# SoyeonHH/MMDA

Hardware: AMD Instinct MI355X
Metric: training samples/sec on MOSEI-shaped synthetic batch (higher is better)
Workload: dtype bf16; 1 GPU; MISA train step, MOSEI shapes B=32/GPU T=50 (d_t,d_v,d_a)=(300,35,74) hidden=128 V=20000, bf16 MFMA operands fp32 accumulate, dropout on, full lengths; global_batch=32, seq_len=50, parallelism=single, use_confidNet=False, rnncell=lstm, dp_global_stats=False

## Files before the change

### mmda_amd/csrc/fused_rows.h

```cpp
#pragma once
#include "../../include/mmda_hip.h"
#include "loss_terms.h"
#include <stdint.h>

struct FusedBwdC {
  int B, hs, ncls, nb;
  const float* tcp; const float* scores; const float* d_tcp; const float* d_scores; float* d_logits;
  float p_cls; uint64_t seed; int site_cls;
  const float* head_w;
  float* d_hfused;
  mmda_ln_bwd_args ln2;
  float* pg_parts;
  const float* d_recon; const float* rec_wT; float* rec_part;
};

struct FusedBwdA {
  int B, hs, nhead, nb;
  mmda_ln_bwd_args ln1;
  const float* ffn_parts; int n_parts; float* d_x1;
  const float* d_attn_out; const float* out_wT; float* d_ctx;
  const float* qkv; const float* probs; float* d_qkv; float p_tf; uint64_t seed; int site_attn;
  const float* in_wT;
  const float* d_recon;
  const float* rec_part;
  const float* rec_wT;
  const float* x6;
  float* d_x6;
  const float* priv_wT;
  const float* sh_wT;
  float* d_orig;
  mmda_ln_bwd_args lnp[3];
  float* pg_parts;
  unsigned long long* dbg;
  const unsigned* wait_flag; unsigned wait_value; unsigned* wait_err;
};

struct FusedFwdA {
  int B, hs, nhead, nb;
  const float* x6;
  const float* rec_w; const float* rec_b; float* recon;
  const float* in_w; const float* in_b; float* qkv;
  float* ctx; float* probs; float p_tf; uint64_t seed; int site_attn;
  const float* out_w; const float* out_b; float* attn_out;
  mmda_ln_args ln1;
  const float* orig; float* d_recon; float* d_orig; float recon_inv_n, recon_scale;
  int split_recon;
};
struct FusedFwdC {
  int B, hs, ncls, nb;
  mmda_ln_args ln2;
  const float* ffn_parts; int n_parts; const float* b2; float* f2;
  const float* hfused; const float* head_w; const float* head_b; float* logits;
  float threshold; float* tcp; float* scores; float* labels; float p_cls; uint64_t seed; int site_cls;
  const float* emo; float* d_scores;
  ClsTerm cls;
};
struct FusedFfnFwd {
  int M, hs, F, S;
  const float* x1; const float* w1; const float* b1; float* f1;
  float p; uint64_t seed; int site;
  const float* w2;
  float* parts;
};
struct FusedFfnBwd {
  int M, hs, F, S;
  const float* d_f2; const float* f1; float gate_scale;
  const float* l2_wT;
  float* d_f1;
  const float* l1_wT;
  float* parts;
};
int mmda_fused_ffn_fwd(const FusedFfnFwd* a, void* stream);
int mmda_fused_ffn_bwd(const FusedFfnBwd* a, void* stream);
int mmda_fused_fwd_a(const FusedFwdA* a, void* stream);
int mmda_fused_fwd_c(const FusedFwdC* a, void* stream);
int mmda_fused_bwd_c(const FusedBwdC* a, void* stream);
int mmda_fused_bwd_a(const FusedBwdA* a, void* stream);
constexpr int FUSED_PG_SLOTS = 5;
int mmda_fused_pg_finish(const float* pg_parts, int B, int hs, float* const* dgamma, float* const* dbeta, void* stream);
extern "C" int mmda_debug_set_fused_stamps(void* device_buffer);
```

### mmda_amd/csrc/fused_rows.hip

```cpp
#include "common.h"
#include "internal.h"
#include "rowlocal.h"
#include "fused_rows.h"

namespace {

typedef __attribute__((ext_vector_type(4))) float f4;
constexpr int FR_THREADS = 512;

struct MacRound { f4 a[8], b[8]; };
constexpr int WL_LD = 128 + 4;
struct WRows { f4 g[8]; };
__device__ __forceinline__ void wrows_load(WRows& W, const float* __restrict__ bblk, int ldb, int lane) {
#pragma unroll
  for (int j = 0; j < 8; ++j) W.g[j] = *reinterpret_cast<const f4*>(bblk + (int64_t)(2 * j + (lane >> 5)) * ldb + 4 * (lane & 31));
}
__device__ __forceinline__ void wrows_to_lds(const WRows& W, float* wl, int lane) {
#pragma unroll
  for (int j = 0; j < 8; ++j) *reinterpret_cast<f4*>(wl + (2 * j + (lane >> 5)) * WL_LD + 4 * (lane & 31)) = W.g[j];
}
__device__ __forceinline__ void mac_frags(MacRound& R, const float* arow , const float* wl, int lane) {
  const int r16 = lane & 15, g = lane >> 4;
  const f4 z = {0.f, 0.f, 0.f, 0.f};
#pragma unroll
  for (int c = 0; c < 8; ++c) {
    R.a[c] = arow ? *reinterpret_cast<const f4*>(arow + 16 * c + 4 * g) : z;
    R.b[c] = *reinterpret_cast<const f4*>(wl + r16 * WL_LD + 16 * c + 4 * g);
  }
}
__device__ __forceinline__ void mac_run(f32x4& acc, const MacRound& R) {
#pragma unroll
  for (int c = 0; c < 8; ++c)
#pragma unroll
    for (int s = 0; s < 4; ++s) acc = __builtin_amdgcn_mfma_f32_16x16x4f32(R.a[c][s], R.b[c][s], acc, 0, 0, 0);
}
template <int NR>
__device__ __forceinline__ void tile_mac_chain(f32x4& acc, const float* const (&ar)[NR], const float* const (&bblk)[NR], const int (&ldb)[NR],
                                               int lane, float* wl ) {
  WRows W;
  MacRound R;
  wrows_load(W, bblk[0], ldb[0], lane);
#pragma unroll
  for (int r = 0; r < NR; ++r) {
    wrows_to_lds(W, wl, lane);
    if (r + 1 < NR) wrows_load(W, bblk[r + 1], ldb[r + 1], lane);
    mac_frags(R, ar[r], wl, lane);
    mac_run(acc, R);
  }
}

__device__ __forceinline__ float sum_parts(const float* __restrict__ p, int n, int64_t stride) {
  float acc = 0.f;
  int q = 0;
  for (; q + 16 <= n; q += 16) {
    float v[16];
#pragma unroll
    for (int u = 0; u < 16; ++u) v[u] = p[(q + u) * stride];
#pragma unroll
    for (int u = 0; u < 16; ++u) acc += v[u];
  }
  for (; q < n; ++q) acc += p[q * stride];
  return acc;
}

template <typename RowOff, typename Finish>
__device__ __forceinline__ void sum_parts_rows(const float* __restrict__ parts, int n, int64_t stride, int groups, RowOff row_off, f4* lds,
                                               Finish finish) {
  const int n0 = (n + 1) >> 1;
  for (int it = threadIdx.x; it < 2 * groups; it += FR_THREADS) {
    const int gi = it % groups, half = it / groups;
    const float* p = parts + row_off(gi) + (int64_t)(half ? n0 : 0) * stride;
    const int cnt = half ? n - n0 : n0;
    f4 acc = {0.f, 0.f, 0.f, 0.f};
    int q = 0;
    for (; q + 16 <= cnt; q += 16) {
      f4 v[16];
#pragma unroll
      for (int u = 0; u < 16; ++u) v[u] = *reinterpret_cast<const f4*>(p + (q + u) * stride);
#pragma unroll
      for (int u = 0; u < 16; ++u) acc += v[u];
    }
    for (; q < cnt; ++q) acc += *reinterpret_cast<const f4*>(p + q * stride);
    lds[half * groups + gi] = acc;
  }
  __syncthreads();
  for (int gi = threadIdx.x; gi < groups; gi += FR_THREADS) finish(gi, lds[gi] + lds[groups + gi]);
  __syncthreads();
}

__device__ __forceinline__ void stage_sync() {
  __threadfence_block();
  __syncthreads();
}

constexpr int LDS_A_FLOATS = 12 * (384 + 4) + 18 * (128 + 4);
template <typename SrcOf>
__device__ __forceinline__ void stage_rows(float* lds, int nrows, int K, SrcOf src_of) {
  const int per_row = K >> 2;
  for (int e = threadIdx.x; e < nrows * per_row; e += FR_THREADS) {
    const int r = e / per_row, c = e % per_row;
    const float* src = src_of(r);
    const f4 z = {0.f, 0.f, 0.f, 0.f};
    *reinterpret_cast<f4*>(lds + r * (K + 4) + 4 * c) = src ? *reinterpret_cast<const f4*>(src + 4 * c) : z;
  }
  __syncthreads();
}

template <typename RowOf>
__device__ __forceinline__ void ln_bwd_rows(const mmda_ln_bwd_args& a, int nrows, RowOf row_of, float* red ,
                                            float* part) {
  const int lane = threadIdx.x & 63, wave = threadIdx.x >> 6;
  float dg[2] = {0.f, 0.f}, db[2] = {0.f, 0.f};
  for (int i = wave; i < nrows; i += FR_THREADS / 64) ln_bwd_row<2>(a, row_of(i), lane, dg, db);
  if (part == nullptr) return;
#pragma unroll
  for (int q = 0; q < 2; ++q) { red[(0 * 8 + wave) * 128 + q * 64 + lane] = dg[q]; red[(1 * 8 + wave) * 128 + q * 64 + lane] = db[q]; }
  __syncthreads();
  for (int i = threadIdx.x; i < 128; i += FR_THREADS) {
    float gsum = 0.f, bsum = 0.f;
#pragma unroll
    for (int w = 0; w < 8; ++w) { gsum += red[(0 * 8 + w) * 128 + i]; bsum += red[(1 * 8 + w) * 128 + i]; }
    part[i] = i < a.n ? gsum : 0.f;
    part[128 + i] = i < a.n ? bsum : 0.f;
  }
  __syncthreads();
}
__device__ __forceinline__ float* pg_slot(float* parts, int b, int k) { return parts ? parts + ((int64_t)b * FUSED_PG_SLOTS + k) * 256 : nullptr; }
__device__ __forceinline__ void pg_zero_rest(float* parts, int b0, int nb, int k) {
  if (!parts) return;
  for (int e = threadIdx.x; e < (nb - 1) * 256; e += FR_THREADS) pg_slot(parts, b0 + 1 + e / 256, k)[e % 256] = 0.f;
}

__device__ __forceinline__ void rec_part_rows(const FusedBwdC& P, int b0, int nb, float* lds_a, float* lds_w) {
  const int B = P.B, hs = P.hs;
  const int lane = threadIdx.x & 63, wave = threadIdx.x >> 6;
  const int r16 = lane & 15, g = lane >> 4;
  const int nmod = 3 * nb;
  const bool mok = r16 < nmod;
  const int mi = mok ? r16 / nb : 0;
  const int col = wave * 16 + r16;
  stage_rows(lds_a, nmod, hs, [&](int r) { return P.d_recon + ((int64_t)(r / nb) * B + b0 + (r % nb)) * hs; });
  f32x4 acc = {0.f, 0.f, 0.f, 0.f};
  const float* row = mok ? lds_a + r16 * (hs + 4) : nullptr;
  const float* const ar[3] = {(mok && mi == 0) ? row : nullptr, (mok && mi == 1) ? row : nullptr, (mok && mi == 2) ? row : nullptr};
  const float* rw = P.rec_wT + (int64_t)wave * 16 * hs;
  const float* const bb[3] = {rw, rw + (int64_t)hs * hs, rw + (int64_t)2 * hs * hs};
  const int ld[3] = {hs, hs, hs};
  tile_mac_chain<3>(acc, ar, bb, ld, lane, lds_w + wave * 16 * WL_LD);
#pragma unroll
  for (int i = 0; i < 4; ++i) {
    const int r = 4 * g + i;
    if (r < nmod) P.rec_part[((int64_t)(r / nb) * B + b0 + (r % nb)) * hs + col] = acc[i];
  }
}

__global__ __launch_bounds__(FR_THREADS) void fused_bwd_c_kernel(FusedBwdC P) {
  __shared__ float red[2 * 8 * 128];
  __shared__ __attribute__((aligned(16))) float lds_a[6 * (128 + 4)];
  __shared__ __attribute__((aligned(16))) float lds_w[8 * 16 * WL_LD];
  const int nblk = (P.B + P.nb - 1) / P.nb;
  if ((int)blockIdx.x >= nblk) {
    const int rb0 = ((int)blockIdx.x - nblk) * P.nb;
    rec_part_rows(P, rb0, min(P.nb, P.B - rb0), lds_a, lds_w);
    return;
  }
  const int b0 = (int)blockIdx.x * P.nb;
  const int nb = min(P.nb, P.B - b0);
  const int NC = 6 + P.ncls, B = P.B, hs = P.hs;
  for (int e = threadIdx.x; e < nb * NC; e += FR_THREADS) {
    const int b = b0 + e / NC, c = e % NC;
    P.d_logits[b * NC + c] = head_bwd_one(b, c, P.ncls, P.tcp, P.scores, P.d_tcp, P.d_scores, P.p_cls, P.seed, P.site_cls);
  }
  stage_sync();
  const int W6 = 6 * hs;
  for (int e = threadIdx.x; e < nb * W6; e += FR_THREADS) {
    const int b = b0 + e / W6, n = e % W6;
    float acc = 0.f;
    for (int c = 0; c < NC; ++c) acc += P.d_logits[b * NC + c] * P.head_w[(int64_t)c * W6 + n];
    P.d_hfused[(int64_t)b * W6 + n] = acc;
  }
  stage_sync();
  ln_bwd_rows(P.ln2, S6K * nb, [&](int i) { return (i / nb) * B + b0 + (i % nb); }, red, pg_slot(P.pg_parts, b0, 0));
  pg_zero_rest(P.pg_parts, b0, nb, 0);
}

__global__ __launch_bounds__(FR_THREADS) void fused_bwd_a_kernel(FusedBwdA P) {
  __shared__ float red[2 * 8 * 128];
  __shared__ __attribute__((aligned(16))) float lds_a[LDS_A_FLOATS];
  __shared__ __attribute__((aligned(16))) float lds_w[8 * 16 * WL_LD];
  const int b0 = (int)blockIdx.x * P.nb;
  const int nb = min(P.nb, P.B - b0);
  const int B = P.B, hs = P.hs;
  const int lane = threadIdx.x & 63, wave = threadIdx.x >> 6;
  const int r16 = lane & 15, g = lane >> 4;
  const int64_t BH = (int64_t)B * hs;
  int stamp_i = 0;
  auto stamp = [&]() { if (P.dbg && blockIdx.x == 0 && threadIdx.x == 0) P.dbg[stamp_i] = __builtin_readcyclecounter(); ++stamp_i; };
  stamp();
  flag_wait(P.wait_flag, P.wait_value, P.wait_err);
  if (P.ffn_parts) {
    const int64_t MH = (int64_t)S6K * B * hs;
    auto off = [&](int gi) { const int i = gi / (hs / 4); return ((int64_t)(i / nb) * B + b0 + (i % nb)) * hs + 4 * (gi % (hs / 4)); };
    sum_parts_rows(P.ffn_parts, P.n_parts, MH, S6K * nb * (hs / 4), off, reinterpret_cast<f4*>(lds_a), [&](int gi, f4 t) {
      f4* d = reinterpret_cast<f4*>(P.d_x1 + off(gi));
      *d = *d + t;
    });
    stage_sync();
  }
  ln_bwd_rows(P.ln1, S6K * nb, [&](int i) { return (i / nb) * B + b0 + (i % nb); }, red, pg_slot(P.pg_parts, b0, 1));
  pg_zero_rest(P.pg_parts, b0, nb, 1);
  stage_sync();
  stamp();
  const int ntok = S6K * nb;
  const bool rok = r16 < ntok;
  const int tj = rok ? r16 / nb : 0;
  const int col = wave * 16 + r16;
  {
    f32x4 acc = {0.f, 0.f, 0.f, 0.f};
    stage_rows(lds_a, ntok, hs, [&](int r) { return P.d_attn_out + ((int64_t)(r / nb) * B + b0 + (r % nb)) * hs; });
    const float* const ar[1] = {rok ? lds_a + r16 * (hs + 4) : nullptr};
    const float* const bb[1] = {P.out_wT + (int64_t)wave * 16 * hs};
    const int ld[1] = {hs};
    tile_mac_chain<1>(acc, ar, bb, ld, lane, lds_w + wave * 16 * WL_LD);
#pragma unroll
    for (int i = 0; i < 4; ++i) {
      const int r = 4 * g + i;
      if (r < ntok) P.d_ctx[((int64_t)(r / nb) * B + b0 + (r % nb)) * hs + col] = acc[i];
    }
  }
  stage_sync();
  stamp();
  for (int pr = wave; pr < nb * P.nhead; pr += FR_THREADS / 64)
    attn_bwd_hd64_one(P.qkv, P.probs, P.d_ctx, B, P.d_qkv, P.p_tf, P.seed, P.site_attn, P.nhead, (b0 + pr / P.nhead) * P.nhead + pr % P.nhead, lane);
  stage_sync();
  stamp();
  {
    f32x4 acc = {0.f, 0.f, 0.f, 0.f};
    float* lds_r = lds_a + 12 * (3 * hs + 4);
    stage_rows(lds_a, ntok, 3 * hs, [&](int r) { return P.d_qkv + ((int64_t)(r / nb) * B + b0 + (r % nb)) * 3 * hs; });
    const float* qrow = rok ? lds_a + r16 * (3 * hs + 4) : nullptr;
    const float* wrow = P.in_wT + (int64_t)wave * 16 * 3 * hs;
    if (P.rec_part) {
      const float* const ar[3] = {qrow, qrow ? qrow + 128 : nullptr, qrow ? qrow + 256 : nullptr};
      const float* const bb[3] = {wrow, wrow + 128, wrow + 256};
      const int ld[3] = {3 * hs, 3 * hs, 3 * hs};
      tile_mac_chain<3>(acc, ar, bb, ld, lane, lds_w + wave * 16 * WL_LD);
    } else {
      stage_rows(lds_r, ntok, hs, [&](int r) { return P.d_recon + ((int64_t)((r / nb) % 3) * B + b0 + (r % nb)) * hs; });
      const float* rec_row = rok ? lds_r + r16 * (hs + 4) : nullptr;
      const float* const ar[6] = {qrow, qrow ? qrow + 128 : nullptr, qrow ? qrow + 256 : nullptr, (rok && tj % 3 == 0) ? rec_row : nullptr,
                                  (rok && tj % 3 == 1) ? rec_row : nullptr, (rok && tj % 3 == 2) ? rec_row : nullptr};
      const float* recw = P.rec_wT + (int64_t)wave * 16 * hs;
      const float* const bb[6] = {wrow, wrow + 128, wrow + 256, recw, recw + (int64_t)hs * hs, recw + (int64_t)2 * hs * hs};
      const int ld[6] = {3 * hs, 3 * hs, 3 * hs, hs, hs, hs};
      tile_mac_chain<6>(acc, ar, bb, ld, lane, lds_w + wave * 16 * WL_LD);
    }
#pragma unroll
    for (int i = 0; i < 4; ++i) {
      const int r = 4 * g + i;
      if (r < ntok) {
        const int64_t o = ((int64_t)(r / nb) * B + b0 + (r % nb)) * hs + col;
        const float s = P.x6[o];
        float t = acc[i];
        if (P.rec_part) t += P.rec_part[((int64_t)((r / nb) % 3) * B + b0 + (r % nb)) * hs + col];
        P.d_x6[o] = (P.d_x6[o] + t) * (s * (1.f - s));
      }
    }
  }
  stage_sync();
  stamp();
  const int nmod = 3 * nb;
  const bool mok = r16 < nmod;
  const int mi = mok ? r16 / nb : 0;
  {
    f32x4 acc = {0.f, 0.f, 0.f, 0.f};
    stage_rows(lds_a, 2 * nmod, hs, [&](int r) { return P.d_x6 + ((int64_t)((r / nmod) * 3 + (r % nmod) / nb) * B + b0 + (r % nb)) * hs; });
    const float* prow = mok ? lds_a + r16 * (hs + 4) : nullptr;
    const float* const ar[4] = {mok ? lds_a + (nmod + r16) * (hs + 4) : nullptr, (mok && mi == 0) ? prow : nullptr,
                                (mok && mi == 1) ? prow : nullptr, (mok && mi == 2) ? prow : nullptr};
    const float* pw = P.priv_wT + (int64_t)wave * 16 * hs;
    const float* const bb[4] = {P.sh_wT + (int64_t)wave * 16 * hs, pw, pw + (int64_t)hs * hs, pw + (int64_t)2 * hs * hs};
    const int ld[4] = {hs, hs, hs, hs};
    tile_mac_chain<4>(acc, ar, bb, ld, lane, lds_w + wave * 16 * WL_LD);
#pragma unroll
    for (int i = 0; i < 4; ++i) {
      const int r = 4 * g + i;
      if (r < nmod) {
        const int64_t o = ((int64_t)(r / nb) * B + b0 + (r % nb)) * hs + col;
        P.d_orig[o] += acc[i];
      }
    }
  }
  stage_sync();
  stamp();
  for (int i = wave; i < 3 * nb; i += FR_THREADS / 64) {
    const mmda_ln_bwd_args& a = P.lnp[i / nb];
    float dg[2] = {0.f, 0.f}, db[2] = {0.f, 0.f};
    ln_bwd_row<2>(a, b0 + i % nb, lane, dg, db);
    float* part = pg_slot(P.pg_parts, b0 + i % nb, 2 + i / nb);
    if (part) {
#pragma unroll
      for (int q = 0; q < 2; ++q) {
        const int c = q * 64 + lane;
        part[c] = c < a.n ? dg[q] : 0.f;
        part[128 + c] = c < a.n ? db[q] : 0.f;
      }
    }
  }
  (void)BH;
  stamp();
}

__global__ __launch_bounds__(FR_THREADS) void fused_fwd_a_kernel(FusedFwdA P) {
  __shared__ __attribute__((aligned(16))) float lds_a[LDS_A_FLOATS];
  __shared__ __attribute__((aligned(16))) float lds_w[8 * 16 * WL_LD];
  const int nblk = (P.B + P.nb - 1) / P.nb;
  const bool do_recon = !P.split_recon || (int)blockIdx.x >= nblk;
  const bool do_chain = !P.split_recon || (int)blockIdx.x < nblk;
  const int b0 = ((int)blockIdx.x % nblk) * P.nb;
  const int nb = min(P.nb, P.B - b0);
  const int B = P.B, hs = P.hs;
  const int lane = threadIdx.x & 63, wave = threadIdx.x >> 6;
  const int r16 = lane & 15, g = lane >> 4;
  const int ntok = S6K * nb, nmod = 3 * nb;
  const bool rok = r16 < ntok;
  const bool mok = r16 < nmod;
  const int mi = mok ? r16 / nb : 0;
  const int col = wave * 16 + r16;
  stage_rows(lds_a, ntok, hs, [&](int r) { return P.x6 + ((int64_t)(r / nb) * B + b0 + (r % nb)) * hs; });
  if (do_recon) {
  for (int e = threadIdx.x; e < nmod * (hs / 4); e += FR_THREADS) {
    const int r = e / (hs / 4), c = e % (hs / 4);
    const f4 a = *reinterpret_cast<const f4*>(lds_a + r * (hs + 4) + 4 * c), b2 = *reinterpret_cast<const f4*>(lds_a + (nmod + r) * (hs + 4) + 4 * c);
    *reinterpret_cast<f4*>(lds_a + (12 + r) * (hs + 4) + 4 * c) = a + b2;
  }
  __syncthreads();
  {
    f32x4 acc = {0.f, 0.f, 0.f, 0.f};
    const float* srow = mok ? lds_a + (12 + r16) * (hs + 4) : nullptr;
    const float* const ar[3] = {(mok && mi == 0) ? srow : nullptr, (mok && mi == 1) ? srow : nullptr, (mok && mi == 2) ? srow : nullptr};
    const float* rw = P.rec_w + (int64_t)wave * 16 * hs;
    const float* const bb[3] = {rw, rw + (int64_t)hs * hs, rw + (int64_t)2 * hs * hs};
    const int ld[3] = {hs, hs, hs};
    tile_mac_chain<3>(acc, ar, bb, ld, lane, lds_w + wave * 16 * WL_LD);
#pragma unroll
    for (int i = 0; i < 4; ++i) {
      const int r = 4 * g + i;
      if (r < nmod) {
        const int64_t o = ((int64_t)(r / nb) * B + b0 + (r % nb)) * hs + col;
        const float rv = acc[i] + P.rec_b[(r / nb) * hs + col];
        P.recon[o] = rv;
        if (P.d_recon) {
          const float gr = recon_seed(rv - P.orig[o], P.recon_inv_n, P.recon_scale);
          P.d_recon[o] = gr;
          P.d_orig[o] = 0.f - gr;
        }
      }
    }
  }
  }
  if (!do_chain) return;
#pragma unroll 1
  for (int pass = 0; pass < 3; ++pass) {
    const int n = pass * 128 + col;
    f32x4 acc = {0.f, 0.f, 0.f, 0.f};
    const float* const ar[1] = {rok ? lds_a + r16 * (hs + 4) : nullptr};
    const float* const bb[1] = {P.in_w + (int64_t)(pass * 128 + wave * 16) * hs};
    const int ld[1] = {hs};
    tile_mac_chain<1>(acc, ar, bb, ld, lane, lds_w + wave * 16 * WL_LD);
    const float bias = P.in_b[n];
#pragma unroll
    for (int i = 0; i < 4; ++i) {
      const int r = 4 * g + i;
      if (r < ntok) P.qkv[((int64_t)(r / nb) * B + b0 + (r % nb)) * 3 * hs + n] = acc[i] + bias;
    }
  }
  stage_sync();
  for (int pr = wave; pr < nb * P.nhead; pr += FR_THREADS / 64)
    attn_fwd_hd64_one(P.qkv, B, P.ctx, P.probs, P.p_tf, P.seed, P.site_attn, P.nhead, (b0 + pr / P.nhead) * P.nhead + pr % P.nhead, lane);
  stage_sync();
  {
    f32x4 acc = {0.f, 0.f, 0.f, 0.f};
    stage_rows(lds_a, ntok, hs, [&](int r) { return P.ctx + ((int64_t)(r / nb) * B + b0 + (r % nb)) * hs; });
    const float* const ar[1] = {rok ? lds_a + r16 * (hs + 4) : nullptr};
    const float* const bb[1] = {P.out_w + (int64_t)wave * 16 * hs};
    const int ld[1] = {hs};
    tile_mac_chain<1>(acc, ar, bb, ld, lane, lds_w + wave * 16 * WL_LD);
    const float bias = P.out_b[col];
#pragma unroll
    for (int i = 0; i < 4; ++i) {
      const int r = 4 * g + i;
      if (r < ntok) P.attn_out[((int64_t)(r / nb) * B + b0 + (r % nb)) * hs + col] = acc[i] + bias;
    }
  }
  stage_sync();
  for (int i = wave; i < ntok; i += FR_THREADS / 64) ln_fwd_row<2>(P.ln1, (i / nb) * B + b0 + (i % nb), lane);
}

template <bool CLS_OPTS>
__global__ __launch_bounds__(FR_THREADS) void fused_fwd_c_kernel(FusedFwdC P) {
  __shared__ f4 sp[2 * 12 * 32];
  const int b0 = (int)blockIdx.x * P.nb;
  const int nb = min(P.nb, P.B - b0);
  const int B = P.B, hs = P.hs, NC = 6 + P.ncls, W6 = 6 * hs;
  const int lane = threadIdx.x & 63, wave = threadIdx.x >> 6;
  if (P.ffn_parts) {
    const int64_t MH = (int64_t)S6K * B * hs;
    auto off = [&](int gi) { const int i = gi / (hs / 4); return ((int64_t)(i / nb) * B + b0 + (i % nb)) * hs + 4 * (gi % (hs / 4)); };
    sum_parts_rows(P.ffn_parts, P.n_parts, MH, S6K * nb * (hs / 4), off, sp, [&](int gi, f4 t) {
      const float* b = P.b2 + 4 * (gi % (hs / 4));
      *reinterpret_cast<f4*>(P.f2 + off(gi)) = t + f4{b[0], b[1], b[2], b[3]};
    });
    stage_sync();
  }
  for (int i = wave; i < S6K * nb; i += FR_THREADS / 64) ln_fwd_row<2>(P.ln2, (i / nb) * B + b0 + (i % nb), lane);
  stage_sync();
  for (int e = wave; e < nb * NC; e += FR_THREADS / 64) {
    const int b = b0 + e / NC, c = e % NC;
    const float* x = P.hfused + (int64_t)b * W6;
    const float* w = P.head_w + (int64_t)c * W6;
    float acc = 0.f;
    for (int k = lane * 4; k < W6; k += 256) {
      const f4 xv = *reinterpret_cast<const f4*>(x + k), wv = *reinterpret_cast<const f4*>(w + k);
      acc += xv[0] * wv[0] + xv[1] * wv[1] + xv[2] * wv[2] + xv[3] * wv[3];
    }
    acc = wave_sum(acc);
    if (lane == 0) {
      const float z = acc + P.head_b[c];
      P.logits[b * NC + c] = z;
      head_fwd_one(z, b, c, P, [&](int k, float sc) {
        if (P.d_scores) {
          const float yv = P.emo[b * P.ncls + k];
          float v, d;
          if constexpr (CLS_OPTS) cls_term(P.cls, sc, yv, k, v, d);
          else bce_plain(sc, yv, 1.f, v, d);
          P.d_scores[b * P.ncls + k] = d / B;
        }
      });
    }
  }
}

constexpr int FFN_RB = 48, FFN_S = 32;
constexpr int FFN_LDS_X = FFN_RB * (128 + 4), FFN_LDS_H = FFN_RB * (FFN_S + 4);

struct FfnGeom { int rb0, nrows, j; };

template <typename Epi1, typename Store2>
__device__ __forceinline__ void ffn_two_products(const float* xs, float* hs_, const float* __restrict__ b1rows ,
                                                 int ldb1, const float* __restrict__ b2rows , int ldb2,
                                                 Epi1 epi1, Store2 store2) {
  const int lane = threadIdx.x & 63, wave = threadIdx.x >> 6;
  const int r16 = lane & 15, g = lane >> 4;
  {
    const int ct = wave >> 2;
    f4 bw[8];
    const float* brow = b1rows + (int64_t)(ct * 16 + r16) * ldb1;
#pragma unroll
    for (int c = 0; c < 8; ++c) bw[c] = *reinterpret_cast<const f4*>(brow + 16 * c + 4 * g);
#pragma unroll
    for (int q = 0; q < (FFN_RB / 16 + 3) / 4; ++q) {
      const int rt = (wave & 3) + 4 * q;
      if (rt >= FFN_RB / 16) break;
      const float* arow = xs + (rt * 16 + r16) * (128 + 4);
      f32x4 acc = {0.f, 0.f, 0.f, 0.f};
#pragma unroll
      for (int c = 0; c < 8; ++c) {
        const f4 a = *reinterpret_cast<const f4*>(arow + 16 * c + 4 * g);
#pragma unroll
        for (int s = 0; s < 4; ++s) acc = __builtin_amdgcn_mfma_f32_16x16x4f32(a[s], bw[c][s], acc, 0, 0, 0);
      }
#pragma unroll
      for (int i = 0; i < 4; ++i) {
        const int row = rt * 16 + 4 * g + i, unit = ct * 16 + r16;
        hs_[row * (FFN_S + 4) + unit] = epi1(row, unit, acc[i]);
      }
    }
  }
  __syncthreads();
  {
    f4 bw[2];
    const float* brow = b2rows + (int64_t)(wave * 16 + r16) * ldb2;
#pragma unroll
    for (int c = 0; c < 2; ++c) bw[c] = *reinterpret_cast<const f4*>(brow + 16 * c + 4 * g);
#pragma unroll
    for (int rt = 0; rt < FFN_RB / 16; ++rt) {
      const float* arow = hs_ + (rt * 16 + r16) * (FFN_S + 4);
      f32x4 acc = {0.f, 0.f, 0.f, 0.f};
#pragma unroll
      for (int c = 0; c < 2; ++c) {
        const f4 a = *reinterpret_cast<const f4*>(arow + 16 * c + 4 * g);
#pragma unroll
        for (int s = 0; s < 4; ++s) acc = __builtin_amdgcn_mfma_f32_16x16x4f32(a[s], bw[c][s], acc, 0, 0, 0);
      }
#pragma unroll
      for (int i = 0; i < 4; ++i) store2(rt * 16 + 4 * g + i, wave * 16 + r16, acc[i]);
    }
  }
}

__device__ __forceinline__ void ffn_stage_x(float* xs, const float* __restrict__ X, int rb0, int M) {
  constexpr int PER = FFN_RB * 32 / FR_THREADS;
  f4 v[PER];
#pragma unroll
  for (int u = 0; u < PER; ++u) {
    const int e = threadIdx.x + u * FR_THREADS, r = e >> 5, c = e & 31;
    v[u] = *reinterpret_cast<const f4*>(X + (int64_t)min(rb0 + r, M - 1) * 128 + 4 * c);
  }
#pragma unroll
  for (int u = 0; u < PER; ++u) {
    const int e = threadIdx.x + u * FR_THREADS, r = e >> 5, c = e & 31;
    const f4 z = {0.f, 0.f, 0.f, 0.f};
    *reinterpret_cast<f4*>(xs + r * (128 + 4) + 4 * c) = (rb0 + r < M) ? v[u] : z;
  }
  __syncthreads();
}

__global__ __launch_bounds__(FR_THREADS) void fused_ffn_fwd_kernel(FusedFfnFwd P) {
  extern __shared__ __attribute__((aligned(16))) float ffn_lds[];
  float* xs = ffn_lds; float* hs_ = ffn_lds + FFN_LDS_X;
  const int nsl = P.F / FFN_S;
  const int j = (int)blockIdx.x % nsl, rb0 = ((int)blockIdx.x / nsl) * FFN_RB;
  ffn_stage_x(xs, P.x1, rb0, P.M);
  float* part = P.parts + (int64_t)j * P.M * P.hs;
  ffn_two_products(xs, hs_, P.w1 + (int64_t)j * FFN_S * P.hs, P.hs, P.w2 + (int64_t)j * FFN_S, P.F,
    [&](int row, int unit, float v) {
      const int m = rb0 + row, n = j * FFN_S + unit;
      v += P.b1[n];
      v = fmaxf(v, 0.f);
      if (P.p > 0.f) v *= drop_mul(P.p, P.seed, P.site, (uint64_t)m * P.F + n);
      if (m < P.M) P.f1[(int64_t)m * P.F + n] = v; else v = 0.f;
      return v;
    },
    [&](int row, int col, float v) { if (rb0 + row < P.M) part[(int64_t)(rb0 + row) * P.hs + col] = v; });
}

__global__ __launch_bounds__(FR_THREADS) void fused_ffn_bwd_kernel(FusedFfnBwd P) {
  extern __shared__ __attribute__((aligned(16))) float ffn_lds[];
  float* xs = ffn_lds; float* hs_ = ffn_lds + FFN_LDS_X;
  const int nsl = P.F / FFN_S;
  const int j = (int)blockIdx.x % nsl, rb0 = ((int)blockIdx.x / nsl) * FFN_RB;
  ffn_stage_x(xs, P.d_f2, rb0, P.M);
  float* part = P.parts + (int64_t)j * P.M * P.hs;
  ffn_two_products(xs, hs_, P.l2_wT + (int64_t)j * FFN_S * P.hs, P.hs, P.l1_wT + (int64_t)j * FFN_S, P.F,
    [&](int row, int unit, float v) {
      const int m = rb0 + row, n = j * FFN_S + unit;
      if (m >= P.M) return 0.f;
      v *= (P.f1[(int64_t)m * P.F + n] > 0.f) ? P.gate_scale : 0.f;
      P.d_f1[(int64_t)m * P.F + n] = v;
      return v;
    },
    [&](int row, int col, float v) { if (rb0 + row < P.M) part[(int64_t)(rb0 + row) * P.hs + col] = v; });
}

}

int mmda_fused_ffn_fwd(const FusedFfnFwd* a, void* stream) {
  if (!a || a->M <= 0 || a->hs != 128 || a->S != FFN_S || a->F <= 0 || (a->F % FFN_S)) return MMDA_EINVAL;
  const int lds = (FFN_LDS_X + FFN_LDS_H) * 4;
  static bool attr = false;
  if (!attr) { (void)hipFuncSetAttribute(reinterpret_cast<const void*>(fused_ffn_fwd_kernel), hipFuncAttributeMaxDynamicSharedMemorySize, lds); attr = true; }
  hipLaunchKernelGGL(fused_ffn_fwd_kernel, dim3((a->F / FFN_S) * ceil_div(a->M, FFN_RB)), dim3(FR_THREADS), lds, (hipStream_t)stream, *a);
  MMDA_CHECK_LAUNCH("mmda_fused_ffn_fwd");
  return MMDA_OK;
}

int mmda_fused_ffn_bwd(const FusedFfnBwd* a, void* stream) {
  if (!a || a->M <= 0 || a->hs != 128 || a->S != FFN_S || a->F <= 0 || (a->F % FFN_S)) return MMDA_EINVAL;
  const int lds = (FFN_LDS_X + FFN_LDS_H) * 4;
  static bool attr = false;
  if (!attr) { (void)hipFuncSetAttribute(reinterpret_cast<const void*>(fused_ffn_bwd_kernel), hipFuncAttributeMaxDynamicSharedMemorySize, lds); attr = true; }
  hipLaunchKernelGGL(fused_ffn_bwd_kernel, dim3((a->F / FFN_S) * ceil_div(a->M, FFN_RB)), dim3(FR_THREADS), lds, (hipStream_t)stream, *a);
  MMDA_CHECK_LAUNCH("mmda_fused_ffn_bwd");
  return MMDA_OK;
}

int mmda_fused_fwd_a(const FusedFwdA* a, void* stream) {
  if (!a || a->B <= 0 || a->nb <= 0 || a->nb > 2 || a->hs != 128 || a->nhead != 2 || a->ln1.n != 128) return MMDA_EINVAL;
  if (a->d_recon && (!a->orig || !a->d_orig)) return MMDA_EINVAL;
  static const int split_on = mmda_env_int("MMDA_FUSED_SPLIT", 1);
  FusedFwdA f = *a;
  const int nblk = ceil_div(a->B, a->nb);
  f.split_recon = (split_on && nblk <= 64) ? 1 : 0;
  hipLaunchKernelGGL(fused_fwd_a_kernel, dim3(f.split_recon ? 2 * nblk : nblk), dim3(FR_THREADS), 0, (hipStream_t)stream, f);
  MMDA_CHECK_LAUNCH("mmda_fused_fwd_a");
  return MMDA_OK;
}

int mmda_fused_fwd_c(const FusedFwdC* a, void* stream) {
  if (!a || a->B <= 0 || a->nb <= 0 || a->nb > 2 || a->hs != 128 || a->ln2.n != 128 || (a->d_scores && !a->emo)) return MMDA_EINVAL;
  const bool opts = a->d_scores && !cls_plain(a->cls);
  hipLaunchKernelGGL(opts ? fused_fwd_c_kernel<true> : fused_fwd_c_kernel<false>, dim3(ceil_div(a->B, a->nb)), dim3(FR_THREADS), 0,
                     (hipStream_t)stream, *a);
  MMDA_CHECK_LAUNCH("mmda_fused_fwd_c");
  return MMDA_OK;
}

struct FusedPgOut { float* dgamma[FUSED_PG_SLOTS]; float* dbeta[FUSED_PG_SLOTS]; };
__global__ __launch_bounds__(256) void fused_pg_finish_kernel(const float* __restrict__ parts, int B, int hs, FusedPgOut out) {
  __shared__ float sub[256];
  const int e = blockIdx.x * 16 + (threadIdx.x >> 4);
  const int j = threadIdx.x & 15;
  const bool ok = e < FUSED_PG_SLOTS * 256;
  const int k = ok ? e / 256 : 0, which = (e % 256) / 128, c = e % 128;
  const float* p = parts + (int64_t)k * 256 + which * 128 + c;
  float acc = 0.f;
  if (ok) {
    const int64_t st = (int64_t)FUSED_PG_SLOTS * 256;
    int b = j;
    for (; b + 7 * 16 < B; b += 8 * 16) {
      float v[8];
#pragma unroll
      for (int u = 0; u < 8; ++u) v[u] = p[(b + 16 * u) * st];
#pragma unroll
      for (int u = 0; u < 8; ++u) acc += v[u];
    }
    for (; b < B; b += 16) acc += p[b * st];
  }
  sub[threadIdx.x] = acc;
  __syncthreads();
  float* dst = which ? out.dbeta[k] : out.dgamma[k];
  if (ok && j == 0 && dst && c < hs) {
    float t = 0.f;
#pragma unroll
    for (int u = 0; u < 16; ++u) t += sub[(threadIdx.x & ~15) + u];
    dst[c] += t;
  }
}

int mmda_fused_pg_finish(const float* pg_parts, int B, int hs, float* const* dgamma, float* const* dbeta, void* stream) {
  if (!pg_parts || B <= 0 || hs != 128 || !dgamma || !dbeta) return MMDA_EINVAL;
  FusedPgOut out;
  for (int k = 0; k < FUSED_PG_SLOTS; ++k) { out.dgamma[k] = dgamma[k]; out.dbeta[k] = dbeta[k]; }
  hipLaunchKernelGGL(fused_pg_finish_kernel, dim3(FUSED_PG_SLOTS * 256 / 16), dim3(256), 0, (hipStream_t)stream, pg_parts, B, hs, out);
  MMDA_CHECK_LAUNCH("mmda_fused_pg_finish");
  return MMDA_OK;
}

int mmda_fused_bwd_c(const FusedBwdC* a, void* stream) {
  if (!a || a->B <= 0 || a->nb <= 0 || a->hs != 128 || a->ln2.n != 128) return MMDA_EINVAL;
  if ((a->ln2.dgamma || a->ln2.dbeta) && !a->pg_parts) return MMDA_EINVAL;
  if (a->rec_part && (!a->d_recon || !a->rec_wT || a->nb > 2)) return MMDA_EINVAL;
  hipLaunchKernelGGL(fused_bwd_c_kernel, dim3(ceil_div(a->B, a->nb) * (a->rec_part ? 2 : 1)), dim3(FR_THREADS), 0, (hipStream_t)stream, *a);
  MMDA_CHECK_LAUNCH("mmda_fused_bwd_c");
  return MMDA_OK;
}

static unsigned long long* g_fr_dbg = nullptr;
extern "C" int mmda_debug_set_fused_stamps(void* device_buffer) { g_fr_dbg = (unsigned long long*)device_buffer; return MMDA_OK; }

int mmda_fused_bwd_a(const FusedBwdA* a, void* stream) {
  if (!a || a->B <= 0 || a->nb <= 0 || a->nb > 2 || a->hs != 128 || a->nhead != 2) return MMDA_EINVAL;
  if ((a->ln1.dgamma || a->ln1.dbeta || a->lnp[0].dgamma || a->lnp[0].dbeta) && !a->pg_parts) return MMDA_EINVAL;
  FusedBwdA P = *a;
  P.dbg = g_fr_dbg;
  hipLaunchKernelGGL(fused_bwd_a_kernel, dim3(ceil_div(a->B, a->nb)), dim3(FR_THREADS), 0, (hipStream_t)stream, P);
  MMDA_CHECK_LAUNCH("mmda_fused_bwd_a");
  return MMDA_OK;
}
```

### mmda_amd/csrc/misa.hip

```cpp
#include "common.h"
#include "fused_rows.h"
#include "internal.h"
#include <algorithm>

#include <cstring>
#include <map>
#include <string>
#include <vector>

namespace {

struct ParamInfo { std::string name; int64_t off; int rows, cols; };

struct RnnP {
  int D, H;
  int64_t w_ih, w_hh[2], b_ih, b_hh;
  int ldD, ldG, ldH;
};
struct ModP {
  int D, H;
  RnnP rnn[2];
  int64_t ln_w, ln_b;
  int64_t pw, pb, plw, plb;
};
struct ParamTable {
  std::vector<ParamInfo> params;
  std::map<std::string, int> index;
  int64_t dense = 0, flat = 0;
  int64_t rnn2_begin = 0, rnn1_begin = 0;
  ModP mod[3];
  int64_t priv_w, priv_b, sh_w, sh_b, rec_w, rec_b, d1_w = -1, d1_b = -1, d2_w = -1, d2_b = -1, sp_w, sp_b;
  int64_t head_w, head_b, embed;
  int64_t in_w, in_b, out_w, out_b, l1_w, l1_b, l2_w, l2_b, n1_w, n1_b, n2_w, n2_b;
  int64_t prelu_a = -1;
};

struct RnnW {
  int64_t pack_f[2], pack_b[2], pack_c[2];
  int64_t wb, wbT;
  int64_t xb, xbT;
  int64_t dgb, dgbT;
  int64_t hbT;
  int64_t hbp[2];
  int64_t pw_ih = -1, pw_hh[2] = {-1, -1}, pb_ih = -1, pb_hh = -1, gw_ih = -1, gw_hh[2] = {-1, -1}, gb = -1;
};
struct ModW {
  RnnW rnn[2];
  int64_t x, gates[2], c[2], hseq[2], normed, ln_mean, ln_rstd, utt, d_utt, d_hseq1, d_normed, d_x, xchg, xchg_floats;
};
struct Workspace {
  int B = 0, T = 0, ldR = 0;
  int64_t floats = 0;
  ModW mod[3];
  int64_t pub_begin = 0, pub_end = 0;
  int64_t zero_begin = 0, zero_end = 0;
  int64_t zero_cls = 0, zero_recon = 0;
  int64_t gpad_begin = 0, gpad_end = 0;
  int64_t z, pmean, prstd, orig, x6, rsum, recon, dom_z, dom_h, dom, qkv, probs, ctx, attn_out, ln1_mean, ln1_rstd, x1, f1, f2,
      ln2_mean, ln2_rstd, hfused, logits, tcp, scores, labels, losses, diff_work, ffn_parts, pg_parts, ln_parts;
  int64_t x1q, x1s, w1q, w1s, f1q, f1s, w2q, w2s;
  int64_t head_wT, l2_wT, l1_wT, out_wT, in_wT, rec_wT, priv_wT, sh_wT, d1_wT = -1, d2_wT = -1, pwT[3];
  int64_t d_scores, d_tcp, d_x6, d_orig, d_recon, d_dom, d_logits, d_hfused, d_x1, d_f2, d_f1, d_attn_out, d_ctx, d_qkv, d_z,
      d_dom_h, d_dom_z;
  int64_t gnorm = -1, gnorm_parts = -1;
  int64_t esort = -1;
  int64_t rec_part = -1;
};

struct StepPlan {
  bool inf = false;
  bool enc_cut = false;
  bool enc_nostash = false;
  bool enc_cached = false;
  bool bfg = false;
  int gm = 0;
  bool kdg = false;
  bool tn_wgrad = false;
  bool want_b = false, want_c = false;
  bool want_wT = false, wT_merge = false;
  bool skinny = false;
  bool row_fuse = false;
  bool ffn_fuse_fwd = false, ffn_fuse_bwd = false;
  bool seed_recon = false, seed_cls = false;
  bool fj_on = false, fj_fwd = false, fj_device = false;
  bool zg_here = false;
  bool rec_hoisted = false;
  bool sort_early = false;
  int embed_update = 0;
  bool embed_deferred = false;
  bool embed_bg = false, embed_bg_late = false; int embed_bg_wgs = 0, embed_bg_lds = 0;
};

enum { EU_DENSE = 0, EU_SPARSE = 1, EU_FROZEN = 2 };

enum { SITE_ATTN = 1, SITE_DROP1 = 2, SITE_FFN = 3, SITE_DROP2 = 4, SITE_CLS = 5, SITE_DISC = 6,
       SITE_RRELU = 7 , SITE_RRELU_DISC = 10 };
constexpr int FFN = 2048, NHEAD = 2, S6 = 6;

struct OptStep { float lr, clip, grad_scale; int step; const float* acc; bool norm; };
struct PendingRows {
  const int64_t* ids = nullptr; const int32_t* lengths = nullptr; bool on = false;
  void set(const int64_t* i, const int32_t* l) { ids = i; lengths = l; on = true; }
  PendingRows take() { const PendingRows r = *this; *this = PendingRows{}; return r; }
};
struct RowList { int64_t* ids; float* rows; int64_t used, capacity; };

int64_t add_param(ParamTable& t, const std::string& name, int rows, int cols) {
  ParamInfo p{name, t.flat, rows, cols};
  t.index[name] = (int)t.params.size();
  t.params.push_back(p);
  t.flat += (int64_t)rows * (cols > 0 ? cols : 1);
  return p.off;
}

ParamTable build_params(const mmda_misa_config& c) {
  ParamTable t{};
  const int dims[3] = {c.d_t, c.d_v, c.d_a};
  const char* mn[3] = {"t", "v", "a"};
  const int hs = c.hidden;
  for (int i = 0; i < 3; ++i) { ModP& md = t.mod[i]; md.D = md.H = dims[i]; }
  for (int i = 0; i < 3; ++i) {
    ModP& md = t.mod[i];
    std::string p = std::string("project_") + mn[i] + ".project_" + mn[i];
    md.pw = add_param(t, p + ".weight", hs, 4 * md.H);
    md.pb = add_param(t, p + ".bias", hs, 0);
    md.plw = add_param(t, p + "_layer_norm.weight", hs, 0);
    md.plb = add_param(t, p + "_layer_norm.bias", hs, 0);
  }
  t.priv_w = add_param(t, "private_t.private_t_1.weight", hs, hs);
  add_param(t, "private_v.private_v_1.weight", hs, hs);
  add_param(t, "private_a.private_a_3.weight", hs, hs);
  t.priv_b = add_param(t, "private_t.private_t_1.bias", hs, 0);
  add_param(t, "private_v.private_v_1.bias", hs, 0);
  add_param(t, "private_a.private_a_3.bias", hs, 0);
  t.sh_w = add_param(t, "shared.shared_1.weight", hs, hs);
  t.sh_b = add_param(t, "shared.shared_1.bias", hs, 0);
  t.rec_w = add_param(t, "recon_t.recon_t_1.weight", hs, hs);
  add_param(t, "recon_v.recon_v_1.weight", hs, hs);
  add_param(t, "recon_a.recon_a_1.weight", hs, hs);
  t.rec_b = add_param(t, "recon_t.recon_t_1.bias", hs, 0);
  add_param(t, "recon_v.recon_v_1.bias", hs, 0);
  add_param(t, "recon_a.recon_a_1.bias", hs, 0);
  if (!c.use_cmd_sim) {
    t.d1_w = add_param(t, "discriminator.discriminator_layer_1.weight", hs, hs);
    t.d1_b = add_param(t, "discriminator.discriminator_layer_1.bias", hs, 0);
    t.d2_w = add_param(t, "discriminator.discriminator_layer_2.weight", 3, hs);
    t.d2_b = add_param(t, "discriminator.discriminator_layer_2.bias", 3, 0);
  }
  t.sp_w = add_param(t, "sp_discriminator.sp_discriminator_layer_1.weight", 4, hs);
  t.sp_b = add_param(t, "sp_discriminator.sp_discriminator_layer_1.bias", 4, 0);
  t.head_w = add_param(t, "confidence.confidence_layer_1.weight", 6, 6 * hs);
  add_param(t, "classifier.classifier_layer.weight", c.ncls, 6 * hs);
  t.head_b = add_param(t, "confidence.confidence_layer_1.bias", 6, 0);
  add_param(t, "classifier.classifier_layer.bias", c.ncls, 0);
  for (int i = 0; i < 3; ++i) {
    t.mod[i].ln_w = add_param(t, std::string(mn[i]) + "layer_norm.weight", 2 * t.mod[i].H, 0);
    t.mod[i].ln_b = add_param(t, std::string(mn[i]) + "layer_norm.bias", 2 * t.mod[i].H, 0);
  }
  const std::string te = "transformer_encoder.layers.0.";
  t.in_w = add_param(t, te + "self_attn.in_proj_weight", 3 * hs, hs);
  t.in_b = add_param(t, te + "self_attn.in_proj_bias", 3 * hs, 0);
  t.out_w = add_param(t, te + "self_attn.out_proj.weight", hs, hs);
  t.out_b = add_param(t, te + "self_attn.out_proj.bias", hs, 0);
  t.l1_w = add_param(t, te + "linear1.weight", FFN, hs);
  t.l1_b = add_param(t, te + "linear1.bias", FFN, 0);
  t.l2_w = add_param(t, te + "linear2.weight", hs, FFN);
  t.l2_b = add_param(t, te + "linear2.bias", hs, 0);
  t.n1_w = add_param(t, te + "norm1.weight", hs, 0);
  t.n1_b = add_param(t, te + "norm1.bias", hs, 0);
  t.n2_w = add_param(t, te + "norm2.weight", hs, 0);
  t.n2_b = add_param(t, te + "norm2.bias", hs, 0);
  if (c.act == MMDA_ACT_PRELU) t.prelu_a = add_param(t, "activation.weight", 1, 0);
  for (int l = 1; l >= 0; --l) {
    t.flat = (t.flat + 3) & ~(int64_t)3;
    (l == 1 ? t.rnn2_begin : t.rnn1_begin) = t.flat;
    for (int i = 0; i < 3; ++i) {
      ModP& md = t.mod[i];
      RnnP& r = md.rnn[l];
      r.H = md.H; r.D = l == 0 ? md.D : 2 * md.H;
      r.ldD = round_up(r.D, 8); r.ldG = round_up(8 * r.H, 8); r.ldH = round_up(r.H, 8);
      const int ng = c.rnncell == MMDA_CELL_GRU ? 3 : 4;
      std::string pre = std::string(mn[i]) + "rnn" + (l == 0 ? "1" : "2") + ".";
      r.w_ih = add_param(t, pre + "weight_ih_l0", ng * r.H, r.D);
      add_param(t, pre + "weight_ih_l0_reverse", ng * r.H, r.D);
      r.w_hh[0] = add_param(t, pre + "weight_hh_l0", ng * r.H, r.H);
      r.w_hh[1] = add_param(t, pre + "weight_hh_l0_reverse", ng * r.H, r.H);
      r.b_ih = add_param(t, pre + "bias_ih_l0", ng * r.H, 0);
      add_param(t, pre + "bias_ih_l0_reverse", ng * r.H, 0);
      r.b_hh = add_param(t, pre + "bias_hh_l0", ng * r.H, 0);
      add_param(t, pre + "bias_hh_l0_reverse", ng * r.H, 0);
    }
  }
  t.flat = (t.flat + 3) & ~(int64_t)3;
  t.dense = t.flat;
  t.embed = add_param(t, "embed.weight", c.vocab, c.d_t);
  t.flat = (t.flat + 3) & ~(int64_t)3;
  return t;
}

Workspace carve(const mmda_misa_config& c, const ParamTable& par, int B, int T) {
  const int hs = c.hidden, NC = 6 + c.ncls;
  const int64_t R = (int64_t)T * B;
  int64_t cur = 0;
  auto take = [&cur](int64_t n) { int64_t o = cur; cur += (n + 3) & ~(int64_t)3; return o; };
  Workspace w{};
  w.B = B; w.T = T; w.ldR = round_up(B * T, 8);
  for (int i = 0; i < 3; ++i) {
    const ModP& md = par.mod[i]; ModW& mw = w.mod[i];
    mw.xchg_floats = (mmda_lstm_xchg_bytes(md.H, B) + 3) / 4;
    mw.xchg = mw.xchg_floats > 0 ? take(mw.xchg_floats) : -1;
  }
  for (int i = 0; i < 3; ++i) {
    const ModP& md = par.mod[i]; ModW& mw = w.mod[i];
    for (int l = 0; l < 2; ++l) {
      const RnnP& r = md.rnn[l]; RnnW& rw = mw.rnn[l];
      for (int d = 0; d < 2; ++d) {
        rw.pack_f[d] = take(mmda_lstm_packed_bytes(MMDA_F32, r.H, 0) / 4);
        rw.pack_b[d] = take(mmda_lstm_packed_bytes(MMDA_F32, r.H, 1) / 4);
        rw.pack_c[d] = take(mmda_lstm_packed_bytes(MMDA_BF16, r.H, 2) / 4);
      }
    }
    for (int l = 0; l < 2; ++l) {
      const RnnP& r = md.rnn[l]; RnnW& rw = mw.rnn[l];
      rw.wb = take((int64_t)8 * r.H * r.ldD / 2); rw.wbT = take((int64_t)r.D * r.ldG / 2);
      rw.xb = take(R * r.ldD / 2); rw.xbT = take((int64_t)r.D * w.ldR / 2);
      rw.dgb = take(R * r.ldG / 2); rw.dgbT = take((int64_t)8 * r.H * w.ldR / 2);
      rw.hbT = take((int64_t)2 * r.H * w.ldR / 2);
      for (int d = 0; d < 2; ++d) rw.hbp[d] = take(R * r.ldH / 2);
    }
    if (c.rnncell == MMDA_CELL_GRU) {
      for (int l = 0; l < 2; ++l) {
        const RnnP& r = md.rnn[l]; RnnW& rw = mw.rnn[l];
        rw.pw_ih = take((int64_t)8 * r.H * r.D); rw.pw_hh[0] = take((int64_t)4 * r.H * r.H); rw.pw_hh[1] = take((int64_t)4 * r.H * r.H);
        rw.pb_ih = take(8 * r.H); rw.pb_hh = take(8 * r.H);
      }
    }
    mw.x = (i == 0) ? take(R * md.D) : -1;
    for (int l = 0; l < 2; ++l) {
      mw.gates[l] = take(R * 8 * md.H);
      mw.c[l] = take((int64_t)T * round_up(B, 4) * 2 * md.H);
      mw.hseq[l] = take(R * 2 * md.H);
    }
    mw.normed = take(R * 2 * md.H);
    mw.ln_mean = take(R);
    mw.ln_rstd = take(R);
    mw.utt = take((int64_t)B * 4 * md.H);
    mw.d_utt = take((int64_t)B * 4 * md.H);
    mw.d_hseq1 = take(R * 2 * md.H);
    mw.d_normed = take(R * 2 * md.H);
    mw.d_x = (i == 0) ? take(R * md.D) : -1;
  }
  const int64_t BH = (int64_t)B * hs;
  w.z = take(3 * BH); w.pmean = take(3 * B); w.prstd = take(3 * B);
  w.pub_begin = cur;
  w.orig = take(3 * BH); w.x6 = take(6 * BH); w.recon = take(3 * BH); w.dom = take((int64_t)3 * B * 3);
  w.tcp = take((int64_t)B * 6); w.scores = take((int64_t)B * c.ncls); w.labels = take((int64_t)B * c.ncls);
  w.pub_end = cur;
  w.rsum = take(3 * BH); w.dom_z = take(3 * BH); w.dom_h = take(3 * BH);
  w.qkv = take(6 * BH * 3); w.probs = take((int64_t)B * NHEAD * S6 * S6); w.ctx = take(6 * BH);
  w.attn_out = take(6 * BH); w.ln1_mean = take(6 * B); w.ln1_rstd = take(6 * B); w.x1 = take(6 * BH);
  w.f1 = take((int64_t)6 * B * FFN); w.f2 = take(6 * BH); w.ln2_mean = take(6 * B); w.ln2_rstd = take(6 * B);
  w.hfused = take(6 * BH); w.logits = take((int64_t)B * NC);
  w.x1q = take(6 * BH / 4); w.x1s = take(6 * BH / 128 + 4); w.w1q = take((int64_t)FFN * hs / 4); w.w1s = take((int64_t)FFN * hs / 128 + 4);
  w.f1q = take((int64_t)6 * B * FFN / 4); w.f1s = take((int64_t)6 * B * FFN / 128 + 4);
  w.w2q = take((int64_t)hs * FFN / 4); w.w2s = take((int64_t)hs * FFN / 128 + 4);
  w.diff_work = take(mmda_loss_diff_work_floats(B, hs));
  w.ffn_parts = take((int64_t)(FFN / 32) * 6 * BH);
  w.ln_parts = take((int64_t)512 * 2 * 2 * (par.mod[0].H + par.mod[1].H + par.mod[2].H));
  w.rec_part = take(3 * BH);
  w.esort = take(2 * (int64_t)B * T + 64);
  w.pg_parts = take((int64_t)B * FUSED_PG_SLOTS * 2 * 128);
  w.head_wT = take((int64_t)6 * hs * NC); w.l2_wT = take((int64_t)FFN * hs); w.l1_wT = take((int64_t)hs * FFN);
  w.out_wT = take((int64_t)hs * hs); w.in_wT = take((int64_t)hs * 3 * hs); w.rec_wT = take((int64_t)3 * hs * hs);
  w.priv_wT = take((int64_t)3 * hs * hs); w.sh_wT = take((int64_t)hs * hs);
  if (!c.use_cmd_sim) { w.d1_wT = take((int64_t)hs * hs); w.d2_wT = take((int64_t)hs * 3); }
  for (int i = 0; i < 3; ++i) w.pwT[i] = take((int64_t)4 * par.mod[i].H * hs);
  w.gpad_begin = cur;
  if (c.rnncell == MMDA_CELL_GRU) {
    for (int i = 0; i < 3; ++i)
      for (int l = 0; l < 2; ++l) {
        const RnnP& r = par.mod[i].rnn[l]; RnnW& rw = w.mod[i].rnn[l];
        rw.gw_ih = take((int64_t)8 * r.H * r.D); rw.gw_hh[0] = take((int64_t)4 * r.H * r.H); rw.gw_hh[1] = take((int64_t)4 * r.H * r.H);
        rw.gb = take(8 * r.H);
      }
  }
  w.gpad_end = cur;
  w.zero_begin = cur;
  w.losses = take(8);
  w.d_tcp = take((int64_t)B * 6); w.d_x6 = take(6 * BH); w.d_dom = take((int64_t)3 * B * 3);
  w.zero_cls = cur;
  w.d_scores = take((int64_t)B * c.ncls);
  w.zero_recon = cur;
  w.d_orig = take(3 * BH); w.d_recon = take(3 * BH);
  w.zero_end = cur;
  w.d_logits = take((int64_t)B * NC); w.d_hfused = take(6 * BH); w.d_x1 = take(6 * BH); w.d_f2 = take(6 * BH);
  w.d_f1 = take((int64_t)6 * B * FFN); w.d_attn_out = take(6 * BH); w.d_ctx = take(6 * BH);
  w.d_qkv = take(6 * BH * 3); w.d_z = take(3 * BH); w.d_dom_h = take(3 * BH); w.d_dom_z = take(3 * BH);
  w.gnorm = take(4); w.gnorm_parts = take(2 * mmda_grad_norm_partials(INT64_MAX));
  w.floats = cur;
  return w;
}

struct TensorName { const char* name; int64_t (*off)(const Workspace&); };
#define TENSOR(name, expr) {name, [](const Workspace& w) -> int64_t { return w.expr; }}
const TensorName kTensorNames[] = {
    TENSOR("scores", scores), TENSOR("labels", labels), TENSOR("tcp", tcp), TENSOR("logits", logits), TENSOR("hfused", hfused),
    TENSOR("x6", x6), TENSOR("orig", orig), TENSOR("recon", recon), TENSOR("dom", dom), TENSOR("losses", losses),
    TENSOR("grad_norm", gnorm), TENSOR("utt_t", mod[0].utt), TENSOR("utt_v", mod[1].utt), TENSOR("utt_a", mod[2].utt),
    TENSOR("d_scores", d_scores), TENSOR("d_tcp", d_tcp), TENSOR("d_x6", d_x6), TENSOR("d_orig", d_orig), TENSOR("d_recon", d_recon),
    TENSOR("d_dom", d_dom), TENSOR("pub_begin", pub_begin), TENSOR("pub_end", pub_end), TENSOR("zero_begin", zero_begin),
    TENSOR("zero_end", zero_end), TENSOR("hseq1_t", mod[0].hseq[0]), TENSOR("hseq1_v", mod[1].hseq[0]), TENSOR("hseq1_a", mod[2].hseq[0]),
    TENSOR("d_x_t", mod[0].d_x),
    TENSOR("xchg_t", mod[0].xchg), TENSOR("xchg_v", mod[1].xchg), TENSOR("xchg_a", mod[2].xchg)};
#undef TENSOR

}

struct mmda_misa {
  explicit mmda_misa(const mmda_misa_config& c) : cfg(c), par(build_params(c)) {}
  mmda_misa(const mmda_misa&) = delete;
  mmda_misa_config cfg;
  const ParamTable par;
  const Workspace& lay = lay_;
  void rebind(const Workspace& v) { lay_ = v; }
  float *P = nullptr, *G = nullptr, *M1 = nullptr, *V1 = nullptr;
  float* ws = nullptr;
  float* xchg_ws = nullptr; int xchg_B = 0; int abort_sticky = 0;
  mmda_adam_opts adam = {0.9f, 0.999f, 1e-8f, 0.f, 0, nullptr};
  float clip_norm = 0.f;
  mmda_cls_opts cls_opts = {}; int cls_on = 0;
  const mmda_cls_opts* cls() const { return cls_on ? &cls_opts : nullptr; }
  int fusion_fp8 = 0;
  int embed_update = EU_DENSE;
  std::vector<mmda_run> runs;
  int prefix_frozen = 0;
  int embed_flag = 1;
  int enc_frozen = 0;
  int cut_keep_stash = 0;
  int32_t* df_row_step = nullptr; float* df_ring = nullptr; int df_window = 0;
  int use_side = 1;
  int use_cluster = 1;
  int use_bf16_gemm = 1;
  int inference = 0;
  int ext_batch_losses = 0;
  int ev_stride = 1;
  int ev_rotate = 0;
  hipStream_t side = nullptr;
  hipEvent_t ev_fork = nullptr, ev_join = nullptr, ev_pack = nullptr;
  hipEvent_t ev_early = nullptr;
  hipStream_t bg = nullptr; hipEvent_t ev_bg_fork = nullptr, ev_bg_done = nullptr;
  unsigned* row_stamp = nullptr; unsigned bg_epoch = 0u;
  int bg_on = -1, bg_wgs = 0;
  const OptStep* bg_step = nullptr;
  int bg_pending = 0, bg_active = 0;
  unsigned* jflags = nullptr;
  mmda_run* runs_dev = nullptr; int runs_dev_cap = 0; int runs_dirty = 1;
  std::vector<hipEvent_t> ev;
  StepPlan plan;
  int64_t early_floats = 0; int early_valid = 0;
  int64_t adam_early_done = 0;
  int wT_valid = 0;
  int wT_pending = 0;
  int enc_cached = 0;
  PendingRows eu;
  int df_seq = 0, df_flushed = 0;
  int training = 0; uint64_t seed = 0;
  unsigned epoch = 1;
  int side_pending = 0;
  int zero_grad_pending = 0;
  int eager_losses = 0, eager_done = 0;
  const float* emo_eager = nullptr;
  const float* misc_deferred = nullptr;
  unsigned jval[2] = {0u, 0u};
  int esort_valid = 0; unsigned esort_val = 0u;
  int fj1 = 0, fj2 = 0, fj1_armed = 0;
  int ev_steps = 0, ev_fwd = 0, ev_bwd = 0;
  int ev_seen_f = 0, ev_seen_b = 0;
  std::vector<char> ev_done;

 private:
  Workspace lay_{};
};

namespace {

struct Ctx {
  mmda_misa* m; void* s; int rc = 0;
  bool grouping = false; std::vector<mmda_gemm_args> pending;
  bool absent_next = false; std::vector<mmda_gemm_args> absent;
  bool deferring = false; std::vector<mmda_gemm_args> deferred;
};

void group_begin(Ctx& c) { c.grouping = true; c.pending.clear(); c.absent.clear(); }
void group_end(Ctx& c) {
  c.grouping = false;
  if (!c.rc && !c.pending.empty())
    c.rc = mmda_gemm_grouped_sized(c.pending.data(), (int)c.pending.size(), c.absent.data(), (int)c.absent.size(), c.s);
  c.pending.clear(); c.absent.clear();
}

void gemm(Ctx& c, int mode, int tA, int tB, int M, int N, int K, const float* A, int lda, const float* Bp, int ldb, float* C,
          int ldc, const float* bias = nullptr, const float* bias2 = nullptr, int acc = 0, int act = 0, int batch = 1,
          int64_t sA = 0, int64_t sB = 0, int64_t sC = 0, int64_t sBias = 0, mmda_gemm_args* extra = nullptr) {
  if (c.rc) return;
  mmda_gemm_args g = {};
  if (extra) g = *extra;
  g.mode = mode; g.transA = tA; g.transB = tB; g.M = M; g.N = N; g.K = K; g.batch = batch;
  g.A = A; g.lda = lda; g.strideA = sA; g.B = Bp; g.ldb = ldb; g.strideB = sB; g.C = C; g.ldc = ldc; g.strideC = sC;
  g.bias = bias; g.bias2 = bias2; g.strideBias = sBias; g.accumulate = acc; g.act = act;
  if (c.absent_next) { c.absent_next = false; if (c.grouping) c.absent.push_back(g); return; }
  if (c.deferring && tA && acc) c.deferred.push_back(g);
  else if (c.grouping) c.pending.push_back(g);
  else c.rc = mmda_gemm(&g, c.s);
}

int side_fork(mmda_misa* m, void* main_stream, void** out);
int side_launch(mmda_misa* m, std::vector<mmda_gemm_args>& list, void* main_stream);
int side_join(mmda_misa* m, void* main_stream);
void lin_fwd(Ctx& c, int mode, int M, int N, int K, const float* x, const float* W, const float* b, float* y, int act = 0) {
  gemm(c, mode, 0, 1, M, N, K, x, K, W, K, y, N, b, nullptr, 0, act);
}
void lin_dx(Ctx& c, int mode, int M, int N, int K, const float* dy, const float* W, float* dx, int acc) {
  gemm(c, mode, 0, 0, M, K, N, dy, N, W, K, dx, K, nullptr, nullptr, acc);
}
void lin_dw(Ctx& c, int mode, int M, int N, int K, const float* dy, const float* x, float* dW, float* db) {
  mmda_gemm_args e = {};
  e.bias_grad = db;
  gemm(c, mode, 1, 0, N, K, M, dy, N, x, K, dW, K, nullptr, nullptr, 1, 0, 1, 0, 0, 0, 0, &e);
}

constexpr int SKINNY_MAX_B = 256;
mmda_skinny_args sk_nt(int M, int N, int K, const float* x, int ldx, const float* W, const float* b, float* y, int ldy, int act = 0) {
  mmda_skinny_args g = {};
  g.M = M; g.N = N; g.K = K; g.transB = 1; g.A = x; g.lda = ldx; g.B = W; g.ldb = K; g.C = y; g.ldc = ldy; g.bias = b; g.act = act;
  return g;
}
mmda_skinny_args sk_nn(int M, int N, int K, const float* dy, int lddy, const float* W, float* dx, int lddx, int acc) {
  mmda_skinny_args g = {};
  g.M = M; g.N = K; g.K = N; g.transB = 0; g.A = dy; g.lda = lddy; g.B = W; g.ldb = K; g.C = dx; g.ldc = lddx; g.accumulate = acc;
  return g;
}
mmda_skinny_args sk_dx(int M, int N, int K, const float* dy, int lddy, const float* WT, float* dx, int lddx, int acc) {
  mmda_skinny_args g = {};
  g.M = M; g.N = K; g.K = N; g.transB = 1; g.A = dy; g.lda = lddy; g.B = WT; g.ldb = N; g.C = dx; g.ldc = lddx; g.accumulate = acc;
  return g;
}
mmda_skinny_args sk_dxw(bool wt, int M, int N, int K, const float* dy, int lddy, const float* WT, const float* W, float* dx, int lddx,
                        int acc) {
  return wt ? sk_dx(M, N, K, dy, lddy, WT, dx, lddx, acc) : sk_nn(M, N, K, dy, lddy, W, dx, lddx, acc);
}
void sk_launch(Ctx& c, const mmda_skinny_args* p, int n) {
  if (!c.rc) c.rc = mmda_gemm_skinny(p, n, c.s);
}


void ev_rec(mmda_misa* m, int step, int slot, int which, void* stream) {
  if (m->ev.empty() || step >= m->ev_steps) return;
  if ((slot < 2 ? m->ev_seen_f : m->ev_seen_b) % m->ev_stride) return;
  if (m->ev_rotate && slot != (step & 3)) return;
  (void)hipEventRecord(m->ev[(step * 4 + slot) * 2 + which], (hipStream_t)stream);
  if (which == 1 && (size_t)(step * 4 + slot) < m->ev_done.size()) m->ev_done[step * 4 + slot] = 1;
}

unsigned fork_event_flags() {
  static const int sysfence = mmda_env_int("MMDA_EVENT_SYSFENCE", 0);
  return hipEventDisableTiming | (sysfence ? 0u : hipEventDisableSystemFence);
}
int side_fork(mmda_misa* m, void* main_stream, void** out) {
  *out = main_stream;
  if (!m->use_side) return MMDA_OK;
  if (!m->side) {
    if (hipStreamCreateWithFlags(&m->side, hipStreamNonBlocking) != hipSuccess) return MMDA_ELAUNCH;
    const unsigned evf = fork_event_flags();
    if (hipEventCreateWithFlags(&m->ev_fork, evf) != hipSuccess) return MMDA_ELAUNCH;
    if (hipEventCreateWithFlags(&m->ev_join, evf) != hipSuccess) return MMDA_ELAUNCH;
    if (hipEventCreateWithFlags(&m->ev_pack, evf) != hipSuccess) return MMDA_ELAUNCH;
    if (hipMalloc(reinterpret_cast<void**>(&m->jflags), 64) != hipSuccess) { m->jflags = nullptr; return MMDA_ELAUNCH; }
    if (hipMemset(m->jflags, 0, 64) != hipSuccess) return MMDA_ELAUNCH;
  }
  if (hipEventRecord(m->ev_fork, (hipStream_t)main_stream) != hipSuccess) return MMDA_ELAUNCH;
  if (hipStreamWaitEvent(m->side, m->ev_fork, 0) != hipSuccess) return MMDA_ELAUNCH;
  m->side_pending = 1;
  *out = m->side;
  return MMDA_OK;
}
int side_launch(mmda_misa* m, std::vector<mmda_gemm_args>& list, void* main_stream) {
  if (list.empty()) return MMDA_OK;
  void* ss = nullptr;
  int rc = side_fork(m, main_stream, &ss);
  if (!rc) rc = mmda_gemm_grouped(list.data(), (int)list.size(), ss);
  list.clear();
  return rc;
}
__global__ void flag_wait_kernel(const unsigned* flag, unsigned value, unsigned* err) { flag_wait(flag, value, err); }
__global__ void flag_set_kernel(unsigned* flag, unsigned value) {
  __hip_atomic_store(flag, value, __ATOMIC_RELEASE, __HIP_MEMORY_SCOPE_AGENT);
}
int side_flag_signal(mmda_misa* m, int idx, bool by_kernel = false) {
  if (!m->side || !m->jflags) return MMDA_EINVAL;
  ++m->jval[idx];
  if (!by_kernel) {
    hipLaunchKernelGGL(flag_set_kernel, dim3(1), dim3(1), 0, m->side, m->jflags + idx, m->jval[idx]);
    MMDA_CHECK_LAUNCH("side_flag_signal");
  }
  if (hipEventRecord(m->ev_join, m->side) != hipSuccess) return MMDA_ELAUNCH;
  m->side_pending = 0;
  return MMDA_OK;
}
int flag_join_fallback(mmda_misa* m, void* main_stream) {
  if (hipStreamWaitEvent((hipStream_t)main_stream, m->ev_join, 0) != hipSuccess) return MMDA_ELAUNCH;
  return MMDA_OK;
}
int side_join(mmda_misa* m, void* main_stream) {
  if (!m->side_pending) return MMDA_OK;
  if (hipEventRecord(m->ev_join, m->side) != hipSuccess) return MMDA_ELAUNCH;
  if (hipStreamWaitEvent((hipStream_t)main_stream, m->ev_join, 0) != hipSuccess) return MMDA_ELAUNCH;
  m->side_pending = 0;
  return MMDA_OK;
}

int bg_begin(mmda_misa* m, const int64_t* ids, int n, void* main_stream, RowStamp* st) {
  const size_t bytes = sizeof(unsigned) * (size_t)m->cfg.vocab;
  if (!m->bg) {
    int least = 0, greatest = 0;
    if (hipDeviceGetStreamPriorityRange(&least, &greatest) != hipSuccess) return MMDA_ELAUNCH;
    if (hipStreamCreateWithPriority(&m->bg, hipStreamNonBlocking, least) != hipSuccess) { m->bg = nullptr; return MMDA_ELAUNCH; }
    if (hipEventCreateWithFlags(&m->ev_bg_fork, fork_event_flags()) != hipSuccess) return MMDA_ELAUNCH;
    if (hipEventCreateWithFlags(&m->ev_bg_done, fork_event_flags()) != hipSuccess) return MMDA_ELAUNCH;
  }
  if (!m->row_stamp) {
    if (hipMalloc(reinterpret_cast<void**>(&m->row_stamp), bytes) != hipSuccess) { m->row_stamp = nullptr; return MMDA_ELAUNCH; }
    if (hipMemset(m->row_stamp, 0, bytes) != hipSuccess) return MMDA_ELAUNCH;
    m->bg_epoch = 0u;
  }
  if (!m->ev_bg_fork || !m->ev_bg_done) return MMDA_ELAUNCH;
  if (++m->bg_epoch == 0u) {
    if (hipMemsetAsync(m->row_stamp, 0, bytes, (hipStream_t)main_stream) != hipSuccess) return MMDA_ELAUNCH;
    m->bg_epoch = 1u;
  }
  *st = RowStamp{m->row_stamp, m->bg_epoch, m->cfg.vocab, ids, n};
  return MMDA_OK;
}
TableRows bg_table(const mmda_misa* m) { return TableRows{m->row_stamp, m->bg_epoch, m->cfg.vocab, m->cfg.d_t}; }
AdamHyper bg_hyper(const mmda_misa* m, const OptStep& o) {
  return AdamHyper{o.lr, m->adam.beta1, m->adam.beta2, m->adam.eps, o.clip, o.grad_scale, o.step, m->adam.weight_decay, m->adam.decoupled, nullptr};
}
int bg_launch(mmda_misa* m, void* main_stream) {
  if (!m->bg_step || !m->bg || !m->row_stamp) return MMDA_EINVAL;
  if (hipEventRecord(m->ev_bg_fork, (hipStream_t)main_stream) != hipSuccess) return MMDA_ELAUNCH;
  if (hipStreamWaitEvent(m->bg, m->ev_bg_fork, 0) != hipSuccess) return MMDA_ELAUNCH;
  const int64_t e = m->par.embed;
  const int rc = mmda_adam_background_launch(m->P + e, m->M1 + e, m->V1 + e, bg_table(m), bg_hyper(m, *m->bg_step), m->plan.embed_bg_wgs,
                                             m->plan.embed_bg_lds, m->bg);
  if (rc) return rc;
  m->bg_pending = 1; m->bg_active = 1;
  if (hipEventRecord(m->ev_bg_done, m->bg) != hipSuccess) return MMDA_ELAUNCH;
  return MMDA_OK;
}
int bg_join(mmda_misa* m, void* stream) {
  if (!m->bg_pending) return MMDA_OK;
  if (hipStreamWaitEvent((hipStream_t)stream, m->ev_bg_done, 0) != hipSuccess) return MMDA_ELAUNCH;
  m->bg_pending = 0;
  return MMDA_OK;
}

#define WS(off) (m->ws + (off))
#define PP(off) (m->P + (off))
#define GG(off) (m->G + (off))

inline bool is_gru(const mmda_misa* m) { return m->cfg.rnncell == MMDA_CELL_GRU; }
inline float* rW_ih(mmda_misa* m, int i, int l) { return is_gru(m) ? WS(m->lay.mod[i].rnn[l].pw_ih) : PP(m->par.mod[i].rnn[l].w_ih); }
inline float* rW_hh(mmda_misa* m, int i, int l, int d) { return is_gru(m) ? WS(m->lay.mod[i].rnn[l].pw_hh[d]) : PP(m->par.mod[i].rnn[l].w_hh[d]); }
inline float* rB_ih(mmda_misa* m, int i, int l) { return is_gru(m) ? WS(m->lay.mod[i].rnn[l].pb_ih) : PP(m->par.mod[i].rnn[l].b_ih); }
inline float* rB_hh(mmda_misa* m, int i, int l) { return is_gru(m) ? WS(m->lay.mod[i].rnn[l].pb_hh) : PP(m->par.mod[i].rnn[l].b_hh); }
inline float* gW_ih(mmda_misa* m, int i, int l) { return is_gru(m) ? WS(m->lay.mod[i].rnn[l].gw_ih) : GG(m->par.mod[i].rnn[l].w_ih); }
inline float* gW_hh(mmda_misa* m, int i, int l, int d) { return is_gru(m) ? WS(m->lay.mod[i].rnn[l].gw_hh[d]) : GG(m->par.mod[i].rnn[l].w_hh[d]); }
inline float* gB_ih(mmda_misa* m, int i, int l) { return is_gru(m) ? WS(m->lay.mod[i].rnn[l].gb) : GG(m->par.mod[i].rnn[l].b_ih); }
inline float* gB_hh(mmda_misa* m, int i, int l) { return is_gru(m) ? nullptr : GG(m->par.mod[i].rnn[l].b_hh); }

int gru_jobs(mmda_misa* m, float* base, bool grads, mmda_gru_pad_job* j) {
  int n = 0;
  for (int i = 0; i < 3; ++i)
    for (int l = 0; l < 2; ++l, ++n) {
      const RnnP& r = m->par.mod[i].rnn[l]; const RnnW& rw = m->lay.mod[i].rnn[l];
      j[n] = mmda_gru_pad_job{};
      j[n].H = r.H; j[n].D = r.D;
      for (int d = 0; d < 2; ++d) {
        j[n].w_ih[d] = base + r.w_ih + (int64_t)d * 3 * r.H * r.D; j[n].w_hh[d] = base + r.w_hh[d];
        j[n].b_ih[d] = base + r.b_ih + (int64_t)d * 3 * r.H; j[n].b_hh[d] = base + r.b_hh + (int64_t)d * 3 * r.H;
        j[n].pw_hh[d] = grads ? WS(rw.gw_hh[d]) : WS(rw.pw_hh[d]);
      }
      j[n].pw_ih = grads ? WS(rw.gw_ih) : WS(rw.pw_ih);
      j[n].pb_ih = grads ? WS(rw.gb) : WS(rw.pb_ih);
      j[n].pb_hh = grads ? nullptr : WS(rw.pb_hh);
    }
  return n;
}

mmda_act_params act_params(mmda_misa* m, int training, uint64_t seed, int site, bool grads) {
  mmda_act_params p = {};
  if (m->cfg.act == MMDA_ACT_PRELU) { p.slope = m->P + m->par.prelu_a; p.dslope = grads ? m->G + m->par.prelu_a : nullptr; }
  if (m->cfg.act == MMDA_ACT_RRELU) { p.lo = 1.0f / 8.0f; p.hi = 1.0f / 3.0f; p.rand = training ? 1 : 0; p.seed = seed; p.site = site; }
  return p;
}

int check_ready(const mmda_misa* m) {
  if (!m || !m->P || !m->ws) return MMDA_EINVAL;
  return MMDA_OK;
}

mmda_lstm_desc lstm_desc(mmda_misa* m, int i, int l, bool bwd, int gate_minor, bool with_c) {
  const ModW& mw = m->lay.mod[i]; const RnnW& rw = mw.rnn[l];
  const int64_t* wp = bwd ? rw.pack_b : rw.pack_f;
  mmda_lstm_desc d = {};
  d.H = m->par.mod[i].rnn[l].H; d.gates = WS(mw.gates[l]); d.cstash = WS(mw.c[l]); d.hseq = WS(mw.hseq[l]);
  d.wpack[0] = WS(wp[0]); d.wpack[1] = WS(wp[1]);
  if (with_c) { d.wpack_c[0] = WS(rw.pack_c[0]); d.wpack_c[1] = WS(rw.pack_c[1]); }
  d.utt = WS(bwd ? mw.d_utt : mw.utt); d.layer = l; d.d_hseq = bwd && l == 0 ? WS(mw.d_hseq1) : nullptr;
  d.xchg = (m->use_cluster && mw.xchg >= 0) ? (void*)WS(mw.xchg) : nullptr; d.epoch_base = m->epoch;
  d.gate_minor = gate_minor; d.cell = m->cfg.rnncell;
  return d;
}

int64_t grad_floats(const mmda_misa* m) { return m->embed_update == EU_DENSE && !m->df_row_step ? m->par.flat : m->par.embed; }

bool masked(const mmda_misa* m) { return m->prefix_frozen || (!m->embed_flag && grad_floats(m) == m->par.flat); }
bool encoder_cut(const mmda_misa* m) {
  return m->enc_frozen && (m->embed_update == EU_FROZEN || (m->embed_update == EU_DENSE && !m->df_row_step && !m->embed_flag));
}
void runs_slice(const mmda_misa* m, int64_t lo, int64_t hi, int* r0, int* n, int64_t* items) {
  const int nr = (int)m->runs.size() - 1;
  int a = 0;
  while (a < nr && m->runs[a].begin < lo) ++a;
  int b = a;
  while (b < nr && m->runs[b].begin < hi) ++b;
  *r0 = a; *n = b - a; *items = m->runs[b].first - m->runs[a].first;
}
int runs_ready(mmda_misa* m, void* stream) {
  if (!m->runs_dirty && m->runs_dev) return MMDA_OK;
  const int need = (int)m->runs.size();
  if (hipStreamSynchronize((hipStream_t)stream) != hipSuccess) return MMDA_ELAUNCH;
  if (m->side && hipStreamSynchronize(m->side) != hipSuccess) return MMDA_ELAUNCH;
  if (need > m->runs_dev_cap) {
    if (m->runs_dev) (void)hipFree(m->runs_dev);
    m->runs_dev = nullptr; m->runs_dev_cap = 0;
    const int cap = (int)m->par.params.size() + 1;
    if (hipMalloc(reinterpret_cast<void**>(&m->runs_dev), sizeof(mmda_run) * cap) != hipSuccess) { m->runs_dev = nullptr; return MMDA_ELAUNCH; }
    m->runs_dev_cap = cap;
  }
  if (hipMemcpy(m->runs_dev, m->runs.data(), sizeof(mmda_run) * need, hipMemcpyHostToDevice) != hipSuccess) return MMDA_ELAUNCH;
  m->runs_dirty = 0;
  return MMDA_OK;
}
constexpr mmda_adam_opts kAdamDefaults = {0.9f, 0.999f, 1e-8f, 0.f, 0, nullptr};
int bucket_adam(mmda_misa* m, int64_t lo, int64_t hi, const float* acc, float lr, float clip, float grad_scale, int step, const FlagWait& w,
                void* stream, const float* scale_dev = nullptr) {
  const AdamHyper h{lr, m->adam.beta1, m->adam.beta2, m->adam.eps, clip, grad_scale, step, m->adam.weight_decay, m->adam.decoupled, scale_dev};
  if (!masked(m)) return mmda_adam_launch(m->P + lo, acc ? acc + lo : nullptr, m->G + lo, m->M1 + lo, m->V1 + lo, hi - lo, nullptr, h, w, stream);
  int r0 = 0, n = 0; int64_t items = 0;
  runs_slice(m, lo, hi, &r0, &n, &items);
  if (n > 0 && (m->runs_dirty || !m->runs_dev)) return MMDA_EINVAL;
  const RunTable t{n > 0 ? m->runs_dev + r0 : nullptr, n, items};
  return mmda_adam_launch(m->P, acc, m->G, m->M1, m->V1, 0, &t, h, w, stream);
}
int bucket_norm(mmda_misa* m, const float* acc, float grad_scale, void* stream) {
  if (!m->ws || m->lay.gnorm < 0) return MMDA_EINVAL;
  double* parts = reinterpret_cast<double*>(m->ws + m->lay.gnorm_parts);
  const int64_t cap = mmda_grad_norm_partials(INT64_MAX);
  const int64_t hi = grad_floats(m);
  if (!masked(m)) return mmda_grad_norm_launch(m->G, acc, hi, nullptr, m->clip_norm, grad_scale, parts, cap, m->ws + m->lay.gnorm, stream);
  int r0 = 0, n = 0; int64_t items = 0;
  runs_slice(m, 0, hi, &r0, &n, &items);
  if (n > 0 && (m->runs_dirty || !m->runs_dev)) return MMDA_EINVAL;
  const RunTable t{n > 0 ? m->runs_dev + r0 : nullptr, n, items};
  return mmda_grad_norm_launch(m->G, acc, 0, &t, m->clip_norm, grad_scale, parts, cap, m->ws + m->lay.gnorm, stream);
}
bool adam_settings_refused(const mmda_misa* m) {
  if (m->adam.weight_decay > 0.f && m->df_row_step) return true;
  if (m->clip_norm > 0.f && (m->embed_update == EU_SPARSE || m->df_row_step)) return true;
  return false;
}
int apply_trainable(mmda_misa* m, const unsigned char* flags) {
  const int np = (int)m->par.params.size();
  std::vector<int64_t> begin, len;
  int prefix_frozen = 0, embed_flag = 1, enc_frozen = 1;
  for (int i = 0; i < np; ++i) {
    const ParamInfo& p = m->par.params[i];
    const bool on = !flags || flags[i] != 0;
    const std::string top = p.name.substr(0, p.name.find('.'));
    if (p.off == m->par.embed) embed_flag = on ? 1 : 0;
    else if (!on) prefix_frozen = 1;
    if (on && ((p.off >= m->par.rnn2_begin && p.off < m->par.embed) || top == "tlayer_norm" || top == "vlayer_norm" || top == "alayer_norm")) enc_frozen = 0;
    if (!on) continue;
    begin.push_back(p.off);
    len.push_back((i + 1 < np ? m->par.params[i + 1].off : m->par.flat) - p.off);
  }
  const int64_t cuts[3] = {m->par.rnn2_begin, m->par.rnn1_begin, m->par.embed};
  std::vector<mmda_run> runs(begin.size() + 1);
  int n = 0;
  const int64_t items = mmda_runs_build_cut(begin.data(), len.data(), (int)begin.size(), m->par.flat, cuts, 3, runs.data(), &n);
  if (items < 0) return MMDA_EINVAL;
  runs.resize(n + 1);
  runs[n] = mmda_run{m->par.flat, 0, items};
  m->runs.swap(runs);
  m->prefix_frozen = prefix_frozen; m->embed_flag = embed_flag; m->enc_frozen = enc_frozen;
  m->runs_dirty = 1;
  return MMDA_OK;
}

constexpr int FJ_DEVICE_MAX_B = 64;
constexpr int kEmbedBgDefault = 1, kEmbedBgWorkgroups = 32, kEmbedBgLds = 1024, kEmbedBgMaxB = 32;

StepPlan plan_step(mmda_misa* m) {
  static const int tn_on = mmda_env_int("MMDA_GEMM_TN", 1);
  static const int wt_merge = mmda_env_int("MMDA_WT_MERGE", 1);
  static const int row_fuse_on = mmda_env_int("MMDA_ROW_FUSE", 1);
  static const int ffn_fuse_on = mmda_env_int("MMDA_FFN_FUSE", 1);
  static const int loss_seeds_on = mmda_env_int("MMDA_LOSS_SEEDS", 1);
  static const int flag_join_on = mmda_env_int("MMDA_FLAG_JOIN", 1);
  static const int zg_side = mmda_env_int("MMDA_ZERO_GRAD_SIDE", -1);
  static const int fsplit = mmda_env_int("MMDA_FUSED_SPLIT", 1);
  static const int sort_early = mmda_env_int("MMDA_SORT_EARLY", 1);
  static const int bg_on = mmda_env_int("MMDA_EMBED_BG", kEmbedBgDefault);
  static const int bg_wgs = mmda_env_int("MMDA_EMBED_BG_WGS", 0);
  static const int bg_late = mmda_env_int("MMDA_EMBED_BG_LATE", 0);
  static const int bg_lds = mmda_env_int("MMDA_EMBED_BG_LDS", kEmbedBgLds);
  const mmda_misa_config& c = m->cfg;
  const int B = m->lay.B, T = m->lay.T, mode = c.mode;
  StepPlan P;
  auto probe_resident = [&](int gate_minor, int backward) -> bool {
    if (T <= 0 || mode != MMDA_BF16) return false;
    mmda_lstm_desc probe[3];
    for (int i = 0; i < 3; ++i) probe[i] = lstm_desc(m, i, 0, false, gate_minor, true);
    if (backward == 2) return mmda_lstm_bwd_emits_dg_bf16(mode, 3, probe, B, T) != 0;
    return mmda_lstm_resident_applicable(mode, 3, probe, B, T, backward) != 0;
  };
  P.inf = m->inference != 0;
  P.enc_cut = !P.inf && encoder_cut(m);
  P.enc_nostash = P.inf || (P.enc_cut && !m->cut_keep_stash);
  P.enc_cached = m->enc_cached != 0;
  P.bfg = mode == MMDA_BF16 && m->use_bf16_gemm;
  if (P.bfg && (B % 8) == 0 && T > 0) P.gm = probe_resident(1, 0) && probe_resident(1, 1);
  P.kdg = !P.enc_nostash && P.bfg && P.gm && probe_resident(1, 2);
  P.tn_wgrad = P.kdg && tn_on;
  P.want_c = !P.enc_nostash && m->use_cluster && mode == MMDA_BF16;
  P.want_b = !P.enc_nostash && !(P.want_c && probe_resident(0, 1));
  P.skinny = B <= SKINNY_MAX_B;
  P.want_wT = P.skinny && !P.inf;
  P.wT_merge = P.bfg && P.want_wT && wt_merge;
  P.row_fuse = P.skinny && row_fuse_on && c.use_cmd_sim && c.hidden == 128 && NHEAD == 2;
  P.ffn_fuse_fwd = P.row_fuse && ffn_fuse_on && !m->fusion_fp8 && (FFN % 32) == 0;
  P.ffn_fuse_bwd = P.row_fuse && ffn_fuse_on && (FFN % 32) == 0;
  P.seed_recon = loss_seeds_on && P.row_fuse && m->eager_losses && m->emo_eager;
  P.seed_cls = P.seed_recon && !c.use_confidNet;
  P.fj_on = flag_join_on && m->use_side && m->eager_losses;
  P.fj_fwd = P.fj_on && P.seed_recon && P.seed_cls;
  P.fj_device = P.fj_fwd && B <= FJ_DEVICE_MAX_B;
  P.zg_here = zg_side >= 0 ? zg_side != 0 : P.fj_device;
  P.rec_hoisted = fsplit && m->lay.rec_part >= 0 && B <= 64;
  P.embed_update = m->embed_update;
  P.embed_deferred = m->embed_update == EU_DENSE && m->df_row_step != nullptr;
  P.sort_early = sort_early && T > 0 && m->lay.esort >= 0 && mmda_embed_scatter_sorts(T * B) && P.embed_update != EU_FROZEN && !P.enc_cut;
  const int bg_switch = m->bg_on >= 0 ? (m->bg_on ? 2 : 0) : bg_on;
  const int64_t tab = (int64_t)c.vocab * c.d_t;
  P.embed_bg = bg_switch != 0 && (bg_switch >= 2 || B <= kEmbedBgMaxB) && m->bg_step && !P.enc_cached && !P.enc_cut && P.embed_update == EU_DENSE &&
               !P.embed_deferred && !masked(m) && T > 0 && m->M1 && m->V1 && tab > 0 && (tab & 3) == 0 && tab < ((int64_t)1 << 31);
  P.embed_bg_late = bg_late != 0;
  P.embed_bg_lds = std::max(0, std::min(65536, bg_lds));
  P.embed_bg_wgs = std::min(4096, m->bg_wgs > 0 ? m->bg_wgs : bg_wgs > 0 ? bg_wgs : kEmbedBgWorkgroups);
  return P;
}

}

extern "C" int mmda_misa_create(const mmda_misa_config* cfg, mmda_misa** out) {
  if (!cfg || !out) return MMDA_EINVAL;
  if (cfg->vocab <= 0 || cfg->d_t <= 0 || cfg->d_v <= 0 || cfg->d_a <= 0 || cfg->hidden <= 0 || cfg->ncls <= 0) return MMDA_EINVAL;
  if (cfg->d_t > 512 || cfg->d_v > 512 || cfg->d_a > 512 || cfg->hidden % NHEAD || cfg->hidden > 1024) return MMDA_EINVAL;
  if (cfg->mode != MMDA_F32 && cfg->mode != MMDA_BF16) return MMDA_EINVAL;
  if (cfg->rnncell != MMDA_CELL_LSTM && cfg->rnncell != MMDA_CELL_GRU) return MMDA_EINVAL;
  mmda_misa* m = new mmda_misa(*cfg);
  if (apply_trainable(m, nullptr)) { delete m; return MMDA_EINVAL; }
  *out = m;
  return MMDA_OK;
}
extern "C" void mmda_misa_destroy(mmda_misa* m) {
  if (!m) return;
  if (m->ev_fork) (void)hipEventDestroy(m->ev_fork);
  if (m->ev_join) (void)hipEventDestroy(m->ev_join);
  if (m->ev_pack) (void)hipEventDestroy(m->ev_pack);
  if (m->ev_early) (void)hipEventDestroy(m->ev_early);
  if (m->bg) { (void)hipStreamSynchronize(m->bg); (void)hipStreamDestroy(m->bg); }
  if (m->ev_bg_fork) (void)hipEventDestroy(m->ev_bg_fork);
  if (m->ev_bg_done) (void)hipEventDestroy(m->ev_bg_done);
  if (m->row_stamp) (void)hipFree(m->row_stamp);
  if (m->side) (void)hipStreamDestroy(m->side);
  if (m->jflags) (void)hipFree(m->jflags);
  if (m->runs_dev) (void)hipFree(m->runs_dev);
  for (hipEvent_t e : m->ev) (void)hipEventDestroy(e);
  delete m;
}
extern "C" int mmda_misa_num_params(const mmda_misa* m) { return m ? (int)m->par.params.size() : MMDA_EINVAL; }
extern "C" int mmda_misa_param_info(const mmda_misa* m, int i, const char** name, int64_t* offset, int* rows, int* cols) {
  if (!m || i < 0 || i >= (int)m->par.params.size()) return MMDA_EINVAL;
  const ParamInfo& p = m->par.params[i];
  if (name) *name = p.name.c_str();
  if (offset) *offset = p.off;
  if (rows) *rows = p.rows;
  if (cols) *cols = p.cols;
  return MMDA_OK;
}
extern "C" int64_t mmda_misa_flat_floats(const mmda_misa* m) { return m ? m->par.flat : MMDA_EINVAL; }
extern "C" int64_t mmda_misa_dense_floats(const mmda_misa* m) { return m ? m->par.dense : MMDA_EINVAL; }
extern "C" int mmda_misa_bind(mmda_misa* m, float* params, float* grads, float* adam_m, float* adam_v) {
  if (!m || !params) return MMDA_EINVAL;
  if (((uintptr_t)params | (uintptr_t)grads | (uintptr_t)adam_m | (uintptr_t)adam_v) & 15) return MMDA_EINVAL;
  m->P = params; m->G = grads; m->M1 = adam_m; m->V1 = adam_v;
  return MMDA_OK;
}
extern "C" int64_t mmda_misa_workspace_floats(const mmda_misa* m, int B, int T) {
  if (!m || B <= 0 || T <= 0) return MMDA_EINVAL;
  return carve(m->cfg, m->par, B, T).floats;
}
namespace {
int harvest_abort(mmda_misa* m) {
  if (!m->ws || !m->xchg_ws || m->xchg_ws != m->ws) return MMDA_OK;
  for (int i = 0; i < 3; ++i) {
    if (m->lay.mod[i].xchg < 0) continue;
    unsigned w = 0;
    if (hipMemcpy(&w, m->ws + m->lay.mod[i].xchg, sizeof(w), hipMemcpyDeviceToHost) != hipSuccess) return MMDA_ELAUNCH;
    if (w) m->abort_sticky = 1;
  }
  return MMDA_OK;
}
}

extern "C" int mmda_misa_set_workspace_async(mmda_misa* m, float* ws, int64_t floats, int B, int T, void* stream) {
  if (!m || !ws || B <= 0 || T <= 0 || ((uintptr_t)ws & 15)) return MMDA_EINVAL;
  const Workspace w = carve(m->cfg, m->par, B, T);
  if (floats < w.floats) return MMDA_EINVAL;
  const bool keep = m->xchg_ws == ws && m->xchg_B == B;
  if (!keep && m->xchg_ws == ws) { int rc = harvest_abort(m); if (rc) return rc; }
  m->rebind(w);
  m->ws = ws;
  hipStream_t s = (hipStream_t)stream;
  if (!keep) {
    for (int i = 0; i < 3; ++i)
      if (w.mod[i].xchg >= 0 && hipMemsetAsync(ws + w.mod[i].xchg, 0, sizeof(float) * w.mod[i].xchg_floats, s) != hipSuccess) return MMDA_ELAUNCH;
    m->xchg_ws = ws; m->xchg_B = B;
  }
  if (w.gpad_end > w.gpad_begin && hipMemsetAsync(ws + w.gpad_begin, 0, sizeof(float) * (w.gpad_end - w.gpad_begin), s) != hipSuccess)
    return MMDA_ELAUNCH;
  return MMDA_OK;
}
extern "C" int mmda_misa_set_workspace(mmda_misa* m, float* ws, int64_t floats, int B, int T) {
  return mmda_misa_set_workspace_async(m, ws, floats, B, T, nullptr);
}
extern "C" int64_t mmda_misa_tensor_offset(const mmda_misa* m, const char* name) {
  if (!m || !name || !m->ws) return -1;
  for (const TensorName& t : kTensorNames)
    if (!strcmp(t.name, name)) return t.off(m->lay);
  return -1;
}
extern "C" int mmda_misa_set_mode(mmda_misa* m, int mode) {
  if (!m || (mode != MMDA_F32 && mode != MMDA_BF16)) return MMDA_EINVAL;
  m->cfg.mode = mode;
  return MMDA_OK;
}
extern "C" int mmda_misa_set_overlap(mmda_misa* m, int side_stream) {
  if (!m) return MMDA_EINVAL;
  m->use_side = side_stream ? 1 : 0;
  return MMDA_OK;
}
extern "C" int mmda_misa_set_recurrence(mmda_misa* m, int resident_weights) {
  if (!m) return MMDA_EINVAL;
  m->use_cluster = resident_weights ? 1 : 0;
  return MMDA_OK;
}
extern "C" int mmda_misa_set_gemm_operands(mmda_misa* m, int bf16_copies) {
  if (!m) return MMDA_EINVAL;
  m->use_bf16_gemm = bf16_copies ? 1 : 0;
  return MMDA_OK;
}
extern "C" int64_t mmda_misa_early_grad_floats(const mmda_misa* m) {
  return (m && m->early_valid) ? m->early_floats : 0;
}
extern "C" int mmda_misa_wait_early_grads(mmda_misa* m, void* stream) {
  if (!m || !m->early_valid || !m->ev_early) return MMDA_EINVAL;
  if (hipStreamWaitEvent((hipStream_t)stream, m->ev_early, 0) != hipSuccess) return MMDA_ELAUNCH;
  return MMDA_OK;
}
extern "C" int mmda_misa_set_external_batch_losses(mmda_misa* m, int on) {
  if (!m) return MMDA_EINVAL;
  m->ext_batch_losses = on ? 1 : 0;
  return MMDA_OK;
}
extern "C" int mmda_misa_set_inference(mmda_misa* m, int forward_only) {
  if (!m) return MMDA_EINVAL;
  m->inference = forward_only ? 1 : 0;
  return MMDA_OK;
}
extern "C" int mmda_misa_cluster_status(const mmda_misa* m, int* aborted_host) {
  if (!m || !m->ws || !aborted_host) return MMDA_EINVAL;
  *aborted_host = m->abort_sticky;
  if (m->jflags) {
    unsigned w = 0;
    if (hipMemcpy(&w, m->jflags + 2, sizeof(w), hipMemcpyDeviceToHost) != hipSuccess) return MMDA_ELAUNCH;
    if (w) *aborted_host |= 2;
  }
  for (int i = 0; i < 3; ++i) {
    if (m->lay.mod[i].xchg < 0) continue;
    unsigned w = 0;
    if (hipMemcpy(&w, m->ws + m->lay.mod[i].xchg, sizeof(w), hipMemcpyDeviceToHost) != hipSuccess) return MMDA_ELAUNCH;
    if (w) *aborted_host = 1;
  }
  return MMDA_OK;
}

namespace {
void weight_transpose_jobs(mmda_misa* m, std::vector<mmda_transpose_job>& tj) {
  const mmda_misa_config& c = m->cfg;
  const ParamTable& p = m->par; const Workspace& w = m->lay;
  const int hs_ = c.hidden, NC_ = 6 + c.ncls;
  auto T_ = [&](int64_t src, int rows, int cols, int64_t dst) { tj.push_back(mmda_transpose_job{PP(src), rows, cols, cols, WS(dst), rows}); };
  T_(p.head_w, NC_, 6 * hs_, w.head_wT); T_(p.l2_w, hs_, FFN, w.l2_wT); T_(p.l1_w, FFN, hs_, w.l1_wT);
  T_(p.out_w, hs_, hs_, w.out_wT); T_(p.in_w, 3 * hs_, hs_, w.in_wT); T_(p.sh_w, hs_, hs_, w.sh_wT);
  for (int i = 0; i < 3; ++i) {
    T_(p.rec_w + (int64_t)i * hs_ * hs_, hs_, hs_, w.rec_wT + (int64_t)i * hs_ * hs_);
    T_(p.priv_w + (int64_t)i * hs_ * hs_, hs_, hs_, w.priv_wT + (int64_t)i * hs_ * hs_);
    T_(p.mod[i].pw, hs_, 4 * p.mod[i].H, w.pwT[i]);
  }
  if (!c.use_cmd_sim) { T_(p.d1_w, hs_, hs_, w.d1_wT); T_(p.d2_w, 3, hs_, w.d2_wT); }
}
int weight_transposes(mmda_misa* m, void* ss) {
  std::vector<mmda_transpose_job> tj;
  weight_transpose_jobs(m, tj);
  const int rc = mmda_transpose_f32(tj.data(), (int)tj.size(), ss);
  m->wT_valid = rc ? 0 : 1;
  m->wT_pending = 0;
  return rc;
}

int backward_only_jobs(mmda_misa* m, mmda_convert_job* cj) {
  const ParamTable& p = m->par; const Workspace& w = m->lay;
  const int R = w.B * w.T;
  int n = 0;
  for (int i = 0; i < 3; ++i) {
    const ModP& md = p.mod[i]; const ModW& mw = w.mod[i];
    for (int l = 0; l < 2; ++l) {
      const RnnP& r = md.rnn[l]; const RnnW& rw = mw.rnn[l];
      if (m->plan.tn_wgrad) {
        for (int d = 0; d < 2; ++d)
          cj[n++] = mmda_convert_job{WS(mw.hseq[l]) + d * md.H, 2 * md.H, R, md.H, nullptr, WS(rw.hbp[d]), r.ldH, nullptr, 0};
      } else {
        cj[n++] = mmda_convert_job{WS(mw.hseq[l]), 2 * md.H, R, 2 * md.H, nullptr, nullptr, 0, WS(rw.hbT), w.ldR};
      }
    }
    if (!m->plan.tn_wgrad) cj[n++] = mmda_convert_job{WS(mw.normed), 2 * md.H, R, 2 * md.H, nullptr, nullptr, 0, WS(mw.rnn[1].xbT), w.ldR};
  }
  return n;
}

int eager_side_losses(mmda_misa* m, void* stream) {
  if (!m->eager_losses) return MMDA_OK;
  const mmda_misa_config& c = m->cfg; const Workspace& w = m->lay;
  const int B = w.B, hs = c.hidden;
  const int64_t BH = (int64_t)B * hs;
  void* ss = nullptr;
  int rc = side_fork(m, stream, &ss);
  if (!rc && m->wT_pending) rc = weight_transposes(m, B >= 128 ? stream : ss);
  const StepPlan& P = m->plan;
  const int64_t zend = P.seed_cls ? w.zero_cls : P.seed_recon ? w.zero_recon : w.zero_end;
  if (!rc && P.zg_here && m->zero_grad_pending) {
    rc = mmda_zero2(WS(w.zero_begin), zend - w.zero_begin, m->G, grad_floats(m), ss);
    m->zero_grad_pending = 0;
  } else if (!rc) {
    if (hipMemsetAsync(WS(w.zero_begin), 0, sizeof(float) * (zend - w.zero_begin), (hipStream_t)ss) != hipSuccess) rc = MMDA_ELAUNCH;
  }
  float* L = WS(w.losses);
  if (!rc) rc = mmda_loss_diff(WS(w.x6), BH, B, hs, c.diff_weight, L + 1, WS(w.d_x6), WS(w.diff_work), ss);
  m->fj1_armed = (!rc && c.use_cmd_sim && P.fj_fwd && m->jflags && mmda_loss_cmd_sets_flag(B, hs)) ? 1 : 0;
  if (!rc && c.use_cmd_sim) {
    static const int sim_pairs[6] = {0, 1, 0, 2, 2, 1};
    rc = mmda_loss_cmd_pairs_tail(WS(w.x6 + 3 * BH), BH, 3, 3, sim_pairs, 5, B, hs, c.sim_weight, 1.0f / 3.0f, L + 2, WS(w.d_x6 + 3 * BH), ss,
                                  m->fj1_armed ? m->jflags + 0 : nullptr, m->jval[0] + 1);
  }
  if (!rc && m->zero_grad_pending) { rc = mmda_misa_zero_grad(m, stream); m->zero_grad_pending = 0; }
  m->eager_done = 1;
  return rc;
}
}

namespace {
int ffn_fp8(mmda_misa* m, float p_tf, uint64_t seed, void* stream) {
  const mmda_misa_config& c = m->cfg; const ParamTable& p = m->par; const Workspace& w = m->lay;
  const int hs = c.hidden, R6 = 6 * w.B;
  if ((hs % 128) != 0) return MMDA_EINVAL;
  auto U8 = [&](int64_t off) { return reinterpret_cast<unsigned char*>(m->ws + off); };
  mmda_mx8_quant_job q[3] = {
      {m->ws + w.x1, hs, R6, hs, U8(w.x1q), U8(w.x1s)},
      {m->P + p.l1_w, hs, FFN, hs, U8(w.w1q), U8(w.w1s)},
      {m->P + p.l2_w, FFN, hs, FFN, U8(w.w2q), U8(w.w2s)}};
  int rc = mmda_mx8_quant(q, 3, stream);
  if (rc) return rc;
  mmda_mx8_args g = {};
  g.M = R6; g.N = FFN; g.K = hs; g.Aq = U8(w.x1q); g.As = U8(w.x1s); g.Bq = U8(w.w1q); g.Bs = U8(w.w1s);
  g.C = m->ws + w.f1; g.ldc = FFN; g.bias = m->P + p.l1_b; g.act = MMDA_ACT_RELU; g.drop_p = p_tf; g.drop_seed = seed; g.drop_site = SITE_FFN;
  rc = mmda_gemm_mx8(&g, stream);
  if (rc) return rc;
  mmda_mx8_quant_job qf = {m->ws + w.f1, FFN, R6, FFN, U8(w.f1q), U8(w.f1s)};
  rc = mmda_mx8_quant(&qf, 1, stream);
  if (rc) return rc;
  mmda_mx8_args h = {};
  h.M = R6; h.N = hs; h.K = FFN; h.Aq = U8(w.f1q); h.As = U8(w.f1s); h.Bq = U8(w.w2q); h.Bs = U8(w.w2s);
  h.C = m->ws + w.f2; h.ldc = hs; h.bias = m->P + p.l2_b;
  return mmda_gemm_mx8(&h, stream);
}
}

extern "C" int mmda_misa_set_adam(mmda_misa* m, const mmda_adam_opts* opts, float clip_norm) {
  if (!m || !(clip_norm >= 0.f)) return MMDA_EINVAL;
  const mmda_adam_opts o = opts ? *opts : kAdamDefaults;
  if (!mmda_adam_opts_valid(&o)) return MMDA_EINVAL;
  const bool moved = o.beta1 != m->adam.beta1 || o.beta2 != m->adam.beta2 || o.eps != m->adam.eps;
  if (moved && m->df_row_step && m->df_flushed != m->df_seq) return MMDA_EINVAL;
  m->adam = o; m->adam.scale_dev = nullptr;
  m->clip_norm = clip_norm;
  return MMDA_OK;
}

extern "C" int mmda_misa_set_cls_loss(mmda_misa* m, const mmda_cls_opts* opts) {
  if (!m || !mmda_cls_opts_valid(opts, m->cfg.ncls)) return MMDA_EINVAL;
  m->cls_on = opts && !(opts->n_weights == 0 && opts->focal_gamma == 0.f);
  m->cls_opts = m->cls_on ? *opts : mmda_cls_opts{};
  return MMDA_OK;
}

extern "C" int mmda_misa_set_embed_update(mmda_misa* m, int mode) {
  if (!m) return MMDA_EINVAL;
  if (mode != EU_DENSE && mode != EU_SPARSE && mode != EU_FROZEN) return MMDA_EINVAL;
  if (mode != EU_DENSE) { m->df_row_step = nullptr; m->df_ring = nullptr; m->df_window = 0; }
  m->embed_update = mode;
  m->eu.take();
  return MMDA_OK;
}

extern "C" int mmda_misa_set_embed_deferred(mmda_misa* m, int32_t* row_step, float* step_scalars, int window, void* stream) {
  if (!m) return MMDA_EINVAL;
  if (!row_step && !step_scalars) {
    m->df_row_step = nullptr; m->df_ring = nullptr; m->df_window = 0; m->eu.take();
    return MMDA_OK;
  }
  if (!row_step || !step_scalars || window < 1 || m->embed_update != EU_DENSE) return MMDA_EINVAL;
  const int rc = mmda_embed_deferred_reset(row_step, m->cfg.vocab, stream);
  if (rc) return rc;
  m->df_row_step = row_step; m->df_ring = step_scalars; m->df_window = window; m->eu.take();
  m->df_seq = m->df_flushed = 0;
  return MMDA_OK;
}

extern "C" int mmda_misa_set_embed_background(mmda_misa* m, int on, int workgroups) {
  if (!m || (on != 0 && on != 1) || workgroups < 0 || workgroups > 4096) return MMDA_EINVAL;
  m->bg_on = on; m->bg_wgs = workgroups;
  return MMDA_OK;
}
extern "C" int mmda_misa_embed_background_active(const mmda_misa* m) { return m ? m->bg_active : MMDA_EINVAL; }

extern "C" int mmda_misa_embed_flush(mmda_misa* m, void* stream) {
  if (!m) return MMDA_EINVAL;
  if (!m->df_row_step) return MMDA_OK;
  if (!m->P || !m->M1 || !m->V1) return MMDA_EINVAL;
  if (m->df_flushed == m->df_seq) return MMDA_OK;
  const int rc = mmda_embed_rows_flush(PP(m->par.embed), m->M1 + m->par.embed, m->V1 + m->par.embed, m->df_row_step, m->df_ring, m->df_window,
                                       m->cfg.d_t, m->cfg.vocab, m->adam.beta1, m->adam.beta2, m->adam.eps, m->df_seq, stream);
  if (!rc) m->df_flushed = m->df_seq;
  return rc;
}

namespace {
int deferred_apply(mmda_misa* m, const int64_t* ids, const unsigned* sorted, const int32_t* lengths, float lr, float beta1, float beta2,
                   float eps, float clip, float grad_scale, int step, bool catch_up, void* stream) {
  if (!m->df_row_step || !m->P || !m->M1 || !m->V1 || !m->ws || m->lay.T <= 0 || !ids) return MMDA_EINVAL;
  if (m->df_seq == INT32_MAX) return MMDA_EINVAL;
  const int seq = m->df_seq + 1;
  const int rc = mmda_embed_dense_adam_apply(PP(m->par.embed), m->M1 + m->par.embed, m->V1 + m->par.embed, m->df_row_step, m->df_ring, m->df_window, ids,
                                             sorted, m->lay.B * m->lay.T, m->cfg.d_t, WS(m->lay.mod[0].d_x), lengths, m->lay.B, m->cfg.vocab, lr, beta1,
                                             beta2, eps, clip, grad_scale, seq, step, catch_up, stream);
  if (rc) return rc;
  if (seq % m->df_window == 0) m->df_flushed = seq - 1;
  m->df_seq = seq;
  return MMDA_OK;
}
}

extern "C" int mmda_misa_embed_deferred_step(mmda_misa* m, float lr, float beta1, float beta2, float eps, float clip, float grad_scale,
                                             int step, void* stream) {
  if (!m || !m->df_row_step || m->embed_update != EU_DENSE || !m->eu.on || step < 1) return MMDA_EINVAL;
  const PendingRows r = m->eu.take();
  return deferred_apply(m, r.ids, nullptr, r.lengths, lr, beta1, beta2, eps, clip, grad_scale, step, true, stream);
}

extern "C" int mmda_misa_set_fusion_fp8(mmda_misa* m, int on) {
  if (!m) return MMDA_EINVAL;
  if (on && (m->cfg.hidden % 128) != 0) return MMDA_EINVAL;
  m->fusion_fp8 = on ? 1 : 0;
  return MMDA_OK;
}

extern "C" int mmda_misa_set_trainable(mmda_misa* m, const unsigned char* flags, int n_params) {
  if (!m || !flags || n_params != (int)m->par.params.size()) return MMDA_EINVAL;
  return apply_trainable(m, flags);
}
extern "C" int mmda_misa_trainable_info(const mmda_misa* m, mmda_run* runs, int capacity, int* n_runs, int64_t* trainable_floats,
                                        int* encoder_cut_on) {
  if (!m || capacity < 0 || (capacity > 0 && !runs)) return MMDA_EINVAL;
  int n = 0; int64_t floats = 0, end = -1, items = 0;
  mmda_run last = {0, 0, 0};
  for (size_t i = 0; i + 1 < m->runs.size(); ++i) {
    const mmda_run& r = m->runs[i];
    floats += r.len;
    if (n > 0 && r.begin == end) {
      last.len += r.len;
    } else {
      if (n > 0) items += ((last.begin + last.len - 1) >> 2) - (last.begin >> 2) + 1;
      last = mmda_run{r.begin, r.len, items};
      ++n;
    }
    if (n <= capacity) runs[n - 1] = last;
    end = r.begin + r.len;
  }
  if (n_runs) *n_runs = n;
  if (trainable_floats) *trainable_floats = floats;
  if (encoder_cut_on) *encoder_cut_on = encoder_cut(m) ? 1 : 0;
  return MMDA_OK;
}
extern "C" int mmda_misa_set_cut_forward(mmda_misa* m, int keep_stash) {
  if (!m) return MMDA_EINVAL;
  m->cut_keep_stash = keep_stash ? 1 : 0;
  return MMDA_OK;
}

namespace {
struct Pass : Ctx {
  const StepPlan& P;
  const mmda_misa_config& c;
  const ParamTable& p; const Workspace& w;
  const int B, T, R, hs, NC, mode;
  static constexpr int fmode = MMDA_F32;
  const int64_t BH; const float p_tf, p_cls; const uint64_t seed;
  const OptStep* early = nullptr;
  Pass(mmda_misa* m_, void* s_)
      : Ctx{m_, s_}, P(m_->plan), c(m_->cfg), p(m_->par), w(m_->lay), B(w.B), T(w.T), R(w.T * w.B), hs(c.hidden), NC(6 + c.ncls), mode(c.mode),
        BH((int64_t)B * hs), p_tf(m_->training ? c.fusion_dropout : 0.f), p_cls(m_->training ? c.dropout : 0.f), seed(m_->seed) {}
  mmda_ln_args proj_ln_fwd(int i), norm1_fwd(), norm2_fwd();
  mmda_ln_bwd_args proj_ln_bwd(int i), norm1_bwd(), norm2_bwd();
  void fwd_operands(const int64_t* t_ids, const float* const* xin);
  void fwd_encoder_layer(int l, const float* const* xin, const int32_t* lengths);
  void fwd_fusion_skinny(), fwd_fusion_tiled();
  void bwd_fusion_fused(), bwd_fusion_skinny(), bwd_fusion_tiled(), skinny_ffn_dx(bool wt), skinny_proj_dx(bool wt);
  void fusion_wgrads(), bwd_side_chain(bool pg_pending, const int64_t* t_ids, const int32_t* lengths);
  void bwd_encoder_layer(int l, const float* const* xin, const int64_t* t_ids, const int32_t* lengths);
  void bwd_text_rows(const int64_t* t_ids, const int32_t* lengths);
  const unsigned* take_sorted();
};

mmda_ln_args Pass::proj_ln_fwd(int i) {
  mmda_ln_args ln = {};
  ln.rows = B; ln.n = hs; ln.x = WS(w.z + i * BH); ln.gamma = PP(p.mod[i].plw); ln.beta = PP(p.mod[i].plb);
  ln.y = WS(w.orig + i * BH); ln.mean = WS(w.pmean + i * B); ln.rstd = WS(w.prstd + i * B); ln.act = c.act;
  ln.eps = 1e-5f; ln.actp = act_params(m, m->training, seed, SITE_RRELU + i, false);
  return ln;
}
mmda_ln_args Pass::norm1_fwd() {
  mmda_ln_args ln = {};
  ln.rows = 6 * B; ln.n = hs; ln.x = WS(w.x6); ln.res = WS(w.attn_out); ln.gamma = PP(p.n1_w); ln.beta = PP(p.n1_b);
  ln.y = WS(w.x1); ln.mean = WS(w.ln1_mean); ln.rstd = WS(w.ln1_rstd); ln.drop_p = p_tf; ln.drop_seed = seed;
  ln.drop_site = SITE_DROP1; ln.eps = 1e-5f;
  return ln;
}
mmda_ln_args Pass::norm2_fwd() {
  mmda_ln_args ln = {};
  ln.rows = 6 * B; ln.n = hs; ln.x = WS(w.x1); ln.res = WS(w.f2); ln.gamma = PP(p.n2_w); ln.beta = PP(p.n2_b);
  ln.y = WS(w.hfused); ln.mean = WS(w.ln2_mean); ln.rstd = WS(w.ln2_rstd); ln.drop_p = p_tf; ln.drop_seed = seed;
  ln.drop_site = SITE_DROP2; ln.permute_S = S6; ln.permute_B = B; ln.eps = 1e-5f;
  return ln;
}
mmda_ln_bwd_args Pass::proj_ln_bwd(int i) {
  mmda_ln_bwd_args l = {};
  l.rows = B; l.n = hs; l.dy = WS(w.d_orig + i * BH); l.x = WS(w.z + i * BH); l.gamma = PP(p.mod[i].plw);
  l.mean = WS(w.pmean + i * B); l.rstd = WS(w.prstd + i * B); l.d_x = WS(w.d_z + i * BH);
  l.dgamma = GG(p.mod[i].plw); l.dbeta = GG(p.mod[i].plb); l.act = c.act;
  l.actp = act_params(m, m->training, seed, SITE_RRELU + i, true);
  return l;
}
mmda_ln_bwd_args Pass::norm1_bwd() {
  mmda_ln_bwd_args l = {};
  l.rows = 6 * B; l.n = hs; l.dy = WS(w.d_x1); l.x = WS(w.x6); l.res = WS(w.attn_out); l.gamma = PP(p.n1_w);
  l.mean = WS(w.ln1_mean); l.rstd = WS(w.ln1_rstd); l.d_x = WS(w.d_x6); l.accumulate_dx = 1; l.d_res = WS(w.d_attn_out);
  l.dgamma = GG(p.n1_w); l.dbeta = GG(p.n1_b); l.drop_p = p_tf; l.drop_seed = seed; l.drop_site = SITE_DROP1;
  return l;
}
mmda_ln_bwd_args Pass::norm2_bwd() {
  mmda_ln_bwd_args l = {};
  l.rows = 6 * B; l.n = hs; l.dy = WS(w.d_hfused); l.x = WS(w.x1); l.res = WS(w.f2); l.gamma = PP(p.n2_w);
  l.mean = WS(w.ln2_mean); l.rstd = WS(w.ln2_rstd); l.d_x = WS(w.d_x1); l.d_res = WS(w.d_f2);
  l.dgamma = GG(p.n2_w); l.dbeta = GG(p.n2_b); l.drop_p = p_tf; l.drop_seed = seed; l.drop_site = SITE_DROP2;
  l.permute_S = S6; l.permute_B = B;
  return l;
}

void Pass::fwd_operands(const int64_t* t_ids, const float* const* xin) {
  auto first_jobs = [&](bool transposed, mmda_convert_job* cj) -> int {
    int n = 0;
    for (int i = 0; i < 3; ++i) {
      for (int l = 0; l < 2; ++l) {
        const RnnP& r = p.mod[i].rnn[l]; const RnnW& rw = w.mod[i].rnn[l];
        cj[n++] = mmda_convert_job{rW_ih(m, i, l), r.D, 8 * r.H, r.D, nullptr, WS(rw.wb), r.ldD,
                                   transposed ? WS(rw.wbT) : nullptr, transposed ? r.ldG : 0, P.gm ? r.H : 0};
      }
      const RnnP& r0 = p.mod[i].rnn[0]; const RnnW& rw0 = w.mod[i].rnn[0];
      const float* src = i == 0 ? PP(p.embed) : xin[i];
      const bool xt = transposed && !P.tn_wgrad;
      cj[n++] = mmda_convert_job{src, r0.D, R, r0.D, i == 0 ? t_ids : nullptr, WS(rw0.xb), r0.ldD, xt ? WS(rw0.xbT) : nullptr, xt ? w.ldR : 0};
    }
    return n;
  };
  m->wT_pending = 0;
  int Hs[12]; const float* Wp[12]; void* Fp[12]; void* Bp[12]; void* Cp[12];
  int k = 0;
  for (int i = 0; i < 3; ++i)
    for (int l = 0; l < 2; ++l)
      for (int d = 0; d < 2; ++d, ++k) {
        const RnnP& r = p.mod[i].rnn[l]; const RnnW& rw = w.mod[i].rnn[l];
        Hs[k] = r.H; Wp[k] = rW_hh(m, i, l, d); Fp[k] = WS(rw.pack_f[d]); Bp[k] = P.want_b ? WS(rw.pack_b[d]) : nullptr; Cp[k] = WS(rw.pack_c[d]);
      }
  m->wT_valid = 0;
  if (P.bfg) {
    mmda_convert_job cj[9];
    const int nj = first_jobs(!P.enc_nostash, cj);
    std::vector<mmda_transpose_job> tj;
    if (P.wT_merge) weight_transpose_jobs(m, tj);
    if (tj.size() > 20) tj.clear();
    RowStamp st;
    if (P.embed_bg) rc = bg_begin(m, t_ids, R, s, &st);
    if (!rc) rc = mmda_lstm_pack_convert_transpose_stamped(12, Hs, Wp, Fp, Bp, P.want_c ? Cp : nullptr, cj, nj, tj.data(), (int)tj.size(),
                                                           P.embed_bg ? &st : nullptr, s);
    m->wT_pending = (P.want_wT && tj.empty()) ? 1 : 0;
    if (!tj.empty()) m->wT_valid = rc ? 0 : 1;
  } else {
    void* ss = nullptr;
    rc = side_fork(m, s, &ss);
    if (!rc) rc = mmda_lstm_pack_whh_multi(mode, 12, Hs, Wp, Fp, Bp, P.want_c ? Cp : nullptr, ss);
    if (!rc && ss != s && hipEventRecord(m->ev_pack, (hipStream_t)ss) != hipSuccess) rc = MMDA_ELAUNCH;
    if (!rc && P.want_wT) rc = weight_transposes(m, ss);
    RowStamp st;
    if (!rc && P.embed_bg) rc = bg_begin(m, t_ids, R, s, &st);
    if (!rc) rc = mmda_embed_gather_stamped(PP(p.embed), t_ids, R, m->cfg.d_t, WS(w.mod[0].x), P.embed_bg ? &st : nullptr, s);
  }
  if (!rc && P.embed_bg && !P.embed_bg_late) rc = bg_launch(m, s);
}

void Pass::fwd_encoder_layer(int l, const float* const* xin, const int32_t* lengths) {
  mmda_lstm_desc desc[3];
  mmda_gemm_bf16_args bg[3];
  group_begin(*this);
  for (int i = 0; i < 3; ++i) {
    const RnnP& r = p.mod[i].rnn[l]; const ModW& mw = w.mod[i]; const RnnW& rw = mw.rnn[l];
    const float* in = l == 0 ? xin[i] : WS(mw.normed);
    if (P.bfg) {
      bg[i] = mmda_gemm_bf16_args{};
      bg[i].M = R; bg[i].N = 8 * r.H; bg[i].K = r.D; bg[i].A = WS(rw.xb); bg[i].lda = r.ldD; bg[i].B = WS(rw.wb); bg[i].ldb = r.ldD;
      bg[i].C = WS(mw.gates[l]); bg[i].ldc = 8 * r.H; bg[i].bias = rB_ih(m, i, l); bg[i].bias2 = rB_hh(m, i, l);
      bg[i].perm_n_H = P.gm ? r.H : 0;
    } else {
      gemm(*this, mode, 0, 1, R, 8 * r.H, r.D, in, r.D, rW_ih(m, i, l), r.D, WS(mw.gates[l]), 8 * r.H, rB_ih(m, i, l), rB_hh(m, i, l));
    }
    desc[i] = lstm_desc(m, i, l, false, P.gm, false);
    desc[i].forward_only = P.enc_nostash;
  }
  if (P.bfg && !rc) rc = mmda_gemm_bf16_grouped(bg, 3, s);
  m->epoch += (unsigned)T + 2u;
  group_end(*this);
  if (!rc && l == 0 && m->side_pending && m->use_side) {
    if (hipStreamWaitEvent((hipStream_t)s, m->ev_pack, 0) != hipSuccess) rc = MMDA_ELAUNCH;
  }
  if (rc) return;
  ev_rec(m, m->ev_fwd, l, 0, s);
  rc = mmda_lstm_fwd(mode, 3, desc, B, T, lengths, s);
  ev_rec(m, m->ev_fwd, l, 1, s);
  if (rc) return;
  if (l == 0 && P.embed_bg && P.embed_bg_late) { rc = bg_launch(m, s); if (rc) return; }
  if (l == 0) {
    mmda_ln_args ln[3];
    for (int i = 0; i < 3; ++i) {
      const ModP& md = p.mod[i]; const ModW& mw = w.mod[i];
      ln[i] = mmda_ln_args{};
      ln[i].rows = R; ln[i].n = 2 * md.H; ln[i].x = WS(mw.hseq[0]); ln[i].gamma = PP(md.ln_w); ln[i].beta = PP(md.ln_b);
      ln[i].y = WS(mw.normed); ln[i].mean = WS(mw.ln_mean); ln[i].rstd = WS(mw.ln_rstd); ln[i].eps = 1e-5f;
    }
    if (P.bfg)
      for (int i = 0; i < 3; ++i) { ln[i].y_bf16 = WS(w.mod[i].rnn[1].xb); ln[i].ld_bf16 = p.mod[i].rnn[1].ldD; }
    if (P.bfg && (P.enc_nostash || P.tn_wgrad))
      for (int i = 0; i < 3; ++i) ln[i].y = nullptr;
    rc = mmda_layernorm_fwd_multi(ln, 3, s);
  } else if (!m->eager_losses && ((P.bfg && !P.enc_nostash) || m->zero_grad_pending || m->wT_pending)) {
    void* ss = nullptr;
    rc = side_fork(m, s, &ss);
    if (!rc && m->wT_pending) rc = weight_transposes(m, ss);
    if (!rc && m->zero_grad_pending && !m->eager_losses) { rc = mmda_misa_zero_grad(m, ss); m->zero_grad_pending = 0; }
  }
}

void Pass::fwd_fusion_skinny() {
  mmda_skinny_args g[8];
  mmda_ln_args ln[3];
  for (int i = 0; i < 3; ++i) {
    const ModP& md = p.mod[i]; const ModW& mw = w.mod[i];
    g[i] = sk_nt(B, hs, 4 * md.H, WS(mw.utt), 4 * md.H, PP(md.pw), PP(md.pb), WS(w.z + i * BH), hs);
    ln[i] = proj_ln_fwd(i);
  }
  sk_launch(*this, g, 3);
  if (!rc) rc = mmda_layernorm_fwd_multi(ln, 3, s);
  for (int i = 0; i < 3; ++i)
    g[i] = sk_nt(B, hs, hs, WS(w.orig + i * BH), hs, PP(p.priv_w + (int64_t)i * hs * hs), PP(p.priv_b + i * hs), WS(w.x6 + i * BH), hs,
                 MMDA_ACT_SIGMOID);
  g[3] = sk_nt(3 * B, hs, hs, WS(w.orig), hs, PP(p.sh_w), PP(p.sh_b), WS(w.x6 + 3 * BH), hs, MMDA_ACT_SIGMOID);
  sk_launch(*this, g, 4);
  if (!rc) rc = eager_side_losses(m, s);
  const mmda_ln_args l1 = norm1_fwd();
  if (P.row_fuse) {
    if (!rc) {
      FusedFwdA f = {};
      f.B = B; f.hs = hs; f.nhead = NHEAD; f.nb = 1; f.x6 = WS(w.x6);
      f.rec_w = PP(p.rec_w); f.rec_b = PP(p.rec_b); f.recon = WS(w.recon);
      f.in_w = PP(p.in_w); f.in_b = PP(p.in_b); f.qkv = WS(w.qkv);
      f.ctx = WS(w.ctx); f.probs = WS(w.probs); f.p_tf = p_tf; f.seed = seed; f.site_attn = SITE_ATTN;
      f.out_w = PP(p.out_w); f.out_b = PP(p.out_b); f.attn_out = WS(w.attn_out); f.ln1 = l1;
      if (P.seed_recon) {
        f.orig = WS(w.orig); f.d_recon = WS(w.d_recon); f.d_orig = WS(w.d_orig);
        f.recon_inv_n = 1.0f / (float)(3 * BH); f.recon_scale = c.recon_weight;
      }
      rc = mmda_fused_fwd_a(&f, s);
    }
  } else {
    int n = 0;
    for (int i = 0; i < 3; ++i) {
      g[n] = sk_nt(B, hs, hs, WS(w.x6 + i * BH), hs, PP(p.rec_w + (int64_t)i * hs * hs), PP(p.rec_b + i * hs), WS(w.recon + i * BH), hs);
      g[n++].A2 = WS(w.x6 + (3 + i) * BH);
    }
    g[n++] = sk_nt(6 * B, 3 * hs, hs, WS(w.x6), hs, PP(p.in_w), PP(p.in_b), WS(w.qkv), 3 * hs);
    if (!c.use_cmd_sim) g[n++] = sk_nt(3 * B, hs, hs, WS(w.x6 + 3 * BH), hs, PP(p.d1_w), PP(p.d1_b), WS(w.dom_z), hs);
    sk_launch(*this, g, n);
    if (!c.use_cmd_sim && !rc) {
      const mmda_act_params ap = act_params(m, m->training, seed, SITE_RRELU_DISC, false);
      rc = mmda_act_dropout_fwd_p(WS(w.dom_z), WS(w.dom_h), 3 * BH, c.act, &ap, p_cls, seed, SITE_DISC, s);
    }
    if (!rc) rc = mmda_attn_fwd(WS(w.qkv), S6, B, hs, NHEAD, WS(w.ctx), WS(w.probs), p_tf, seed, SITE_ATTN, s);
    n = 0;
    g[n++] = sk_nt(6 * B, hs, hs, WS(w.ctx), hs, PP(p.out_w), PP(p.out_b), WS(w.attn_out), hs);
    if (!c.use_cmd_sim) g[n++] = sk_nt(3 * B, 3, hs, WS(w.dom_h), hs, PP(p.d2_w), PP(p.d2_b), WS(w.dom), 3);
    sk_launch(*this, g, n);
    if (!rc) rc = mmda_layernorm_fwd(&l1, s);
  }
  if (m->fusion_fp8) {
    if (!rc) rc = ffn_fp8(m, p_tf, seed, s);
  } else if (P.ffn_fuse_fwd) {
    if (!rc) {
      FusedFfnFwd f = {};
      f.M = 6 * B; f.hs = hs; f.F = FFN; f.S = 32; f.x1 = WS(w.x1); f.w1 = PP(p.l1_w); f.b1 = PP(p.l1_b); f.f1 = WS(w.f1);
      f.p = p_tf; f.seed = seed; f.site = SITE_FFN; f.w2 = PP(p.l2_w); f.parts = WS(w.ffn_parts);
      rc = mmda_fused_ffn_fwd(&f, s);
    }
  } else {
    g[0] = sk_nt(6 * B, FFN, hs, WS(w.x1), hs, PP(p.l1_w), PP(p.l1_b), WS(w.f1), FFN, MMDA_ACT_RELU);
    g[0].drop_p = p_tf; g[0].drop_seed = seed; g[0].drop_site = SITE_FFN;
    sk_launch(*this, g, 1);
    g[0] = sk_nt(6 * B, hs, FFN, WS(w.f1), FFN, PP(p.l2_w), PP(p.l2_b), WS(w.f2), hs);
    sk_launch(*this, g, 1);
  }
  const mmda_ln_args l2 = norm2_fwd();
  if (P.row_fuse) {
    if (!rc) {
      FusedFwdC f = {};
      f.B = B; f.hs = hs; f.ncls = c.ncls; f.nb = 1; f.ln2 = l2;
      if (P.ffn_fuse_fwd) { f.ffn_parts = WS(w.ffn_parts); f.n_parts = FFN / 32; f.b2 = PP(p.l2_b); f.f2 = WS(w.f2); }
      f.hfused = WS(w.hfused); f.head_w = PP(p.head_w); f.head_b = PP(p.head_b); f.logits = WS(w.logits);
      f.threshold = c.threshold; f.tcp = WS(w.tcp); f.scores = WS(w.scores); f.labels = WS(w.labels);
      f.p_cls = p_cls; f.seed = seed; f.site_cls = SITE_CLS;
      if (P.seed_cls) { f.emo = m->emo_eager; f.d_scores = WS(w.d_scores); f.cls = cls_term_of(m->cls()); }
      rc = mmda_fused_fwd_c(&f, s);
    }
  } else {
    if (!rc) rc = mmda_layernorm_fwd(&l2, s);
    g[0] = sk_nt(B, NC, 6 * hs, WS(w.hfused), 6 * hs, PP(p.head_w), PP(p.head_b), WS(w.logits), NC);
    sk_launch(*this, g, 1);
    if (!rc)
      rc = mmda_heads_fwd(WS(w.logits), B, c.ncls, c.threshold, WS(w.tcp), WS(w.scores), WS(w.labels), p_cls, seed, SITE_CLS,
                            s);
  }
}

void Pass::fwd_fusion_tiled() {
  for (int i = 0; i < 3 && !rc; ++i) {
    const ModP& md = p.mod[i]; const ModW& mw = w.mod[i];
    lin_fwd(*this, fmode, B, hs, 4 * md.H, WS(mw.utt), PP(md.pw), PP(md.pb), WS(w.z + i * BH));
    if (rc) break;
    const mmda_ln_args ln = proj_ln_fwd(i);
    rc = mmda_layernorm_fwd(&ln, s);
  }
  gemm(*this, fmode, 0, 1, B, hs, hs, WS(w.orig), hs, PP(p.priv_w), hs, WS(w.x6), hs, PP(p.priv_b), nullptr, 0, MMDA_ACT_SIGMOID, 3,
       BH, (int64_t)hs * hs, BH, hs);
  gemm(*this, fmode, 0, 1, 3 * B, hs, hs, WS(w.orig), hs, PP(p.sh_w), hs, WS(w.x6 + 3 * BH), hs, PP(p.sh_b), nullptr, 0,
       MMDA_ACT_SIGMOID);
  if (!rc) rc = eager_side_losses(m, s);
  if (!rc) rc = mmda_add(WS(w.x6), WS(w.x6 + 3 * BH), WS(w.rsum), 3 * BH, s);
  gemm(*this, fmode, 0, 1, B, hs, hs, WS(w.rsum), hs, PP(p.rec_w), hs, WS(w.recon), hs, PP(p.rec_b), nullptr, 0, 0, 3, BH,
       (int64_t)hs * hs, BH, hs);
  if (!c.use_cmd_sim) {
    lin_fwd(*this, fmode, 3 * B, hs, hs, WS(w.x6 + 3 * BH), PP(p.d1_w), PP(p.d1_b), WS(w.dom_z));
    if (!rc) {
      const mmda_act_params ap = act_params(m, m->training, seed, SITE_RRELU_DISC, false);
      rc = mmda_act_dropout_fwd_p(WS(w.dom_z), WS(w.dom_h), 3 * BH, c.act, &ap, p_cls, seed, SITE_DISC, s);
    }
    lin_fwd(*this, fmode, 3 * B, 3, hs, WS(w.dom_h), PP(p.d2_w), PP(p.d2_b), WS(w.dom));
  }
  lin_fwd(*this, fmode, 6 * B, 3 * hs, hs, WS(w.x6), PP(p.in_w), PP(p.in_b), WS(w.qkv));
  if (!rc) rc = mmda_attn_fwd(WS(w.qkv), S6, B, hs, NHEAD, WS(w.ctx), WS(w.probs), p_tf, seed, SITE_ATTN, s);
  lin_fwd(*this, fmode, 6 * B, hs, hs, WS(w.ctx), PP(p.out_w), PP(p.out_b), WS(w.attn_out));
  const mmda_ln_args l1 = norm1_fwd(), l2 = norm2_fwd();
  if (!rc) rc = mmda_layernorm_fwd(&l1, s);
  if (m->fusion_fp8) {
    if (!rc) rc = ffn_fp8(m, p_tf, seed, s);
  } else {
    mmda_gemm_args e = {};
    e.drop_p = p_tf; e.drop_seed = seed; e.drop_site = SITE_FFN;
    gemm(*this, fmode, 0, 1, 6 * B, FFN, hs, WS(w.x1), hs, PP(p.l1_w), hs, WS(w.f1), FFN, PP(p.l1_b), nullptr, 0, MMDA_ACT_RELU, 1, 0,
         0, 0, 0, &e);
    lin_fwd(*this, fmode, 6 * B, hs, FFN, WS(w.f1), PP(p.l2_w), PP(p.l2_b), WS(w.f2));
  }
  if (!rc) rc = mmda_layernorm_fwd(&l2, s);
  lin_fwd(*this, fmode, B, NC, 6 * hs, WS(w.hfused), PP(p.head_w), PP(p.head_b), WS(w.logits));
  if (!rc)
    rc = mmda_heads_fwd(WS(w.logits), B, c.ncls, c.threshold, WS(w.tcp), WS(w.scores), WS(w.labels), p_cls, seed, SITE_CLS,
                          s);
}
}

namespace {
int forward_from_projections(Pass& x, void* stream) {
  mmda_misa* m = x.m;
  if (m->plan.skinny) x.fwd_fusion_skinny();
  else x.fwd_fusion_tiled();
  if (!x.rc && m->wT_pending) {
    void* ss = nullptr;
    x.rc = side_fork(m, stream, &ss);
    if (!x.rc) x.rc = weight_transposes(m, ss);
  }
  if (!x.rc && m->plan.fj_fwd && m->side_pending && m->jflags) {
    x.rc = side_flag_signal(m, 0, m->fj1_armed != 0);
    m->fj1 = x.rc ? 0 : 1; m->fj1_armed = 0;
    return x.rc;
  }
  if (m->fj1_armed) return MMDA_ELAUNCH;
  if (!x.rc) x.rc = side_join(m, stream);
  return x.rc;
}

bool encoded_batch_ok(const mmda_misa* m, const mmda_encoded_batch* eb) {
  return eb && eb->tab_t && eb->tab_v && eb->tab_a && eb->rows && eb->B > 0 && eb->B == m->lay.B;
}

int forward_encoded(mmda_misa* m, const mmda_encoded_batch* eb, float* emo_out, int training, uint64_t seed, void* stream) {
  m->training = training; m->seed = seed;
  m->enc_cached = 1;
  m->plan = plan_step(m);
  Pass x(m, stream);
  m->wT_valid = 0;
  m->wT_pending = m->plan.want_wT ? 1 : 0;
  x.rc = mmda_encoded_gather(eb->tab_t, eb->tab_v, eb->tab_a, 4 * m->par.mod[0].H, 4 * m->par.mod[1].H, 4 * m->par.mod[2].H,
                             emo_out ? eb->tab_emo : nullptr, m->cfg.ncls, eb->rows, m->lay.B, WS(m->lay.mod[0].utt), WS(m->lay.mod[1].utt),
                             WS(m->lay.mod[2].utt), emo_out, stream);
  if (x.rc) return x.rc;
  return forward_from_projections(x, stream);
}
}

extern "C" int mmda_misa_forward_encoded(mmda_misa* m, const mmda_encoded_batch* eb, int training, uint64_t seed, void* stream) {
  if (check_ready(m) || !encoded_batch_ok(m, eb)) return MMDA_EINVAL;
  if (!m->inference && !encoder_cut(m)) return MMDA_EINVAL;
  return forward_encoded(m, eb, nullptr, training, seed, stream);
}

extern "C" int mmda_misa_forward(mmda_misa* m, const int64_t* t_ids, const float* v, const float* a, const int32_t* lengths,
                                 int training, uint64_t seed, void* stream) {
  if (check_ready(m) || !t_ids || !v || !a || !lengths) return MMDA_EINVAL;
  m->enc_cached = 0;
  m->training = training; m->seed = seed;
  m->plan = plan_step(m);
  Pass x(m, stream);
  if (is_gru(m)) {
    mmda_gru_pad_job gj[MMDA_GRU_PAD_MAX];
    int n = gru_jobs(m, m->P, false, gj);
    x.rc = mmda_gru_pad_params(gj, n, stream);
    if (x.rc) return x.rc;
  }
  if (m->plan.embed_deferred) {
    if (!m->M1 || !m->V1) return MMDA_EINVAL;
    x.rc = mmda_embed_rows_catch_up(PP(m->par.embed), m->M1 + m->par.embed, m->V1 + m->par.embed, m->df_row_step, m->df_ring, m->df_window, t_ids,
                                    m->lay.B * m->lay.T, m->cfg.d_t, lengths, m->lay.B, m->cfg.vocab, m->adam.beta1, m->adam.beta2, m->adam.eps, m->df_seq, stream);
    if (x.rc) return x.rc;
  }
  const float* xin[3] = {WS(m->lay.mod[0].x), v, a};
  x.fwd_operands(t_ids, xin);
  for (int l = 0; l < 2 && !x.rc; ++l) x.fwd_encoder_layer(l, xin, lengths);
  if (x.rc) return x.rc;
  if (!m->ev.empty()) { if (m->ev_seen_f % m->ev_stride == 0) m->ev_fwd++; m->ev_seen_f++; }
  return forward_from_projections(x, stream);
}

extern "C" int mmda_misa_zero_act_grads(mmda_misa* m, void* stream) {
  if (check_ready(m)) return MMDA_EINVAL;
  if (hipMemsetAsync(WS(m->lay.zero_begin), 0, sizeof(float) * (m->lay.zero_end - m->lay.zero_begin), (hipStream_t)stream) != hipSuccess)
    return MMDA_ELAUNCH;
  return MMDA_OK;
}

extern "C" int mmda_misa_losses(mmda_misa* m, const float* emo, int with_grads, void* stream) {
  if (check_ready(m) || !emo) return MMDA_EINVAL;
  const mmda_misa_config& c = m->cfg; const Workspace& w = m->lay;
  const int B = w.B, hs = c.hidden;
  const int64_t BH = (int64_t)B * hs;
  hipStream_t s = (hipStream_t)stream;
  int rc = MMDA_OK;
  float* L = WS(w.losses);
  const bool ext = m->ext_batch_losses && with_grads && c.use_cmd_sim;
  const bool eager = (m->eager_done || ext) && with_grads;
  const bool s_recon = m->eager_done && with_grads && m->plan.seed_recon, s_cls = m->eager_done && with_grads && m->plan.seed_cls;
  m->eager_done = 0;
  if (eager) {
    rc = side_join(m, stream);
    if (rc) return rc;
  } else {
    if (with_grads) { rc = mmda_misa_zero_act_grads(m, stream); if (rc) return rc; }
    else if (hipMemsetAsync(WS(w.losses), 0, sizeof(float) * 8, s) != hipSuccess) return MMDA_ELAUNCH;
    rc = mmda_loss_diff(WS(w.x6), BH, B, hs, c.diff_weight, L + 1, with_grads ? WS(w.d_x6) : nullptr, WS(w.diff_work), stream);
    if (rc) return rc;
  }
  if (c.use_cmd_sim) {
    if (!eager) rc = mmda_loss_cmd(WS(w.x6 + 3 * BH), BH, B, hs, c.sim_weight, L + 2, with_grads ? WS(w.d_x6 + 3 * BH) : nullptr, stream);
  } else {
    rc = mmda_loss_domain(WS(w.dom), B, c.sim_weight, L + 2, with_grads ? WS(w.d_dom) : nullptr, stream);
  }
  if (rc) return rc;
  if (s_recon && s_cls && c.use_cmd_sim) {
    m->misc_deferred = emo;
    return MMDA_OK;
  }
  return mmda_loss_misc_opts(WS(w.scores), WS(w.tcp), emo, B, c.ncls, (with_grads && !s_cls) ? WS(w.d_scores) : nullptr,
                             (with_grads && !s_cls) ? WS(w.d_tcp) : nullptr, c.ncls == 6 && !ext, with_grads && c.use_confidNet && !ext,
                             c.conf_weight, WS(w.recon), WS(w.orig), 3 * BH, c.recon_weight, (with_grads && !s_recon) ? WS(w.d_recon) : nullptr,
                             (with_grads && !s_recon) ? WS(w.d_orig) : nullptr, L, c.diff_weight, c.sim_weight, c.recon_weight, c.conf_weight,
                             c.use_confidNet, m->cls(), stream);
}

extern "C" int mmda_misa_zero_grad(mmda_misa* m, void* stream) {
  if (!m || !m->G) return MMDA_EINVAL;
  if (hipMemsetAsync(m->G, 0, sizeof(float) * grad_floats(m), (hipStream_t)stream) != hipSuccess) return MMDA_ELAUNCH;
  return MMDA_OK;
}

namespace {
void Pass::skinny_ffn_dx(bool wt) {
  mmda_skinny_args g = sk_dxw(wt, 6 * B, hs, FFN, WS(w.d_f2), hs, WS(w.l2_wT), PP(p.l2_w), WS(w.d_f1), FFN, 0);
  g.gate = WS(w.f1); g.ldgate = FFN; g.gate_scale = p_tf > 0.f ? 1.f / (1.f - p_tf) : 1.f;
  sk_launch(*this, &g, 1);
  g = sk_dxw(wt, 6 * B, FFN, hs, WS(w.d_f1), FFN, WS(w.l1_wT), PP(p.l1_w), WS(w.d_x1), hs, 1);
  sk_launch(*this, &g, 1);
}
void Pass::skinny_proj_dx(bool wt) {
  mmda_skinny_args g[3];
  for (int i = 0; i < 3; ++i) {
    const ModP& md = p.mod[i]; const ModW& mw = w.mod[i];
    g[i] = sk_dxw(wt, B, hs, 4 * md.H, WS(w.d_z + i * BH), hs, WS(w.pwT[i]), PP(md.pw), WS(mw.d_utt), 4 * md.H, 0);
  }
  sk_launch(*this, g, 3);
}

void Pass::bwd_fusion_fused() {
  {
    FusedBwdC f = {};
    f.B = B; f.hs = hs; f.ncls = c.ncls; f.nb = 1;
    f.tcp = WS(w.tcp); f.scores = WS(w.scores); f.d_tcp = WS(w.d_tcp); f.d_scores = WS(w.d_scores); f.d_logits = WS(w.d_logits);
    if (m->fj1) f.d_tcp = nullptr;
    if (P.rec_hoisted) { f.d_recon = WS(w.d_recon); f.rec_wT = WS(w.rec_wT); f.rec_part = WS(w.rec_part); }
    f.p_cls = p_cls; f.seed = seed; f.site_cls = SITE_CLS; f.head_w = PP(p.head_w); f.d_hfused = WS(w.d_hfused); f.ln2 = norm2_bwd();
    f.pg_parts = WS(w.pg_parts);
    rc = mmda_fused_bwd_c(&f, s);
  }
  if (P.ffn_fuse_bwd) {
    if (!rc) {
      FusedFfnBwd f = {};
      f.M = 6 * B; f.hs = hs; f.F = FFN; f.S = 32; f.d_f2 = WS(w.d_f2); f.f1 = WS(w.f1);
      f.gate_scale = p_tf > 0.f ? 1.f / (1.f - p_tf) : 1.f; f.l2_wT = WS(w.l2_wT); f.d_f1 = WS(w.d_f1); f.l1_wT = WS(w.l1_wT);
      f.parts = WS(w.ffn_parts);
      rc = mmda_fused_ffn_bwd(&f, s);
    }
  } else {
    skinny_ffn_dx(true);
  }
  if (rc) return;
  FusedBwdA f = {};
  f.B = B; f.hs = hs; f.nhead = NHEAD; f.nb = 1;
  if (P.ffn_fuse_bwd) { f.ffn_parts = WS(w.ffn_parts); f.n_parts = FFN / 32; f.d_x1 = WS(w.d_x1); }
  f.ln1 = norm1_bwd();
  f.d_attn_out = WS(w.d_attn_out); f.out_wT = WS(w.out_wT); f.d_ctx = WS(w.d_ctx);
  f.qkv = WS(w.qkv); f.probs = WS(w.probs); f.d_qkv = WS(w.d_qkv); f.p_tf = p_tf; f.seed = seed; f.site_attn = SITE_ATTN;
  f.in_wT = WS(w.in_wT); f.d_recon = WS(w.d_recon); f.rec_wT = WS(w.rec_wT); f.x6 = WS(w.x6); f.d_x6 = WS(w.d_x6);
  if (P.rec_hoisted) f.rec_part = WS(w.rec_part);
  f.priv_wT = WS(w.priv_wT); f.sh_wT = WS(w.sh_wT); f.d_orig = WS(w.d_orig);
  for (int i = 0; i < 3; ++i) f.lnp[i] = proj_ln_bwd(i);
  f.pg_parts = WS(w.pg_parts);
  if (m->fj1) {
    if (P.fj_device) { f.wait_flag = m->jflags; f.wait_value = m->jval[0]; f.wait_err = m->jflags + 2; }
    else rc = flag_join_fallback(m, s);
    m->fj1 = 0;
  }
  if (!rc) rc = mmda_fused_bwd_a(&f, s);
  if (!P.enc_cut) skinny_proj_dx(true);
}

void Pass::bwd_fusion_skinny() {
  const bool wt = m->wT_valid != 0;
  mmda_skinny_args g[8];
  rc = mmda_heads_bwd(WS(w.tcp), WS(w.scores), WS(w.d_tcp), WS(w.d_scores), B, c.ncls, WS(w.d_logits), p_cls, seed, SITE_CLS,
                        s);
  g[0] = sk_dxw(wt, B, NC, 6 * hs, WS(w.d_logits), NC, WS(w.head_wT), PP(p.head_w), WS(w.d_hfused), 6 * hs, 0);
  sk_launch(*this, g, 1);
  const mmda_ln_bwd_args l2 = norm2_bwd(), l1 = norm1_bwd();
  if (!rc) rc = mmda_layernorm_bwd(&l2, s);
  skinny_ffn_dx(wt);
  if (!rc) rc = mmda_layernorm_bwd(&l1, s);
  int n = 0;
  g[n++] = sk_dxw(wt, 6 * B, hs, hs, WS(w.d_attn_out), hs, WS(w.out_wT), PP(p.out_w), WS(w.d_ctx), hs, 0);
  if (!c.use_cmd_sim) g[n++] = sk_dxw(wt, 3 * B, 3, hs, WS(w.d_dom), 3, WS(w.d2_wT), PP(p.d2_w), WS(w.d_dom_h), hs, 0);
  sk_launch(*this, g, n);
  if (!rc) rc = mmda_attn_bwd(WS(w.qkv), WS(w.probs), WS(w.d_ctx), S6, B, hs, NHEAD, WS(w.d_qkv), p_tf, seed, SITE_ATTN, s);
  if (!c.use_cmd_sim) {
    if (!rc) {
      const mmda_act_params ap = act_params(m, m->training, seed, SITE_RRELU_DISC, true);
      rc = mmda_act_dropout_bwd_p(WS(w.d_dom_h), WS(w.dom_z), WS(w.d_dom_z), 3 * BH, c.act, &ap, p_cls, seed, SITE_DISC, s);
    }
    g[0] = sk_dxw(wt, 3 * B, hs, hs, WS(w.d_dom_z), hs, WS(w.d1_wT), PP(p.d1_w), WS(w.d_x6 + 3 * BH), hs, 1);
    g[0].alpha = -c.reverse_grad_weight;
    sk_launch(*this, g, 1);
  }
  for (int j = 0; j < 6; ++j) {
    const int i = j % 3;
    g[j] = sk_dxw(wt, B, 3 * hs, hs, WS(w.d_qkv + (int64_t)j * B * 3 * hs), 3 * hs, WS(w.in_wT), PP(p.in_w), WS(w.d_x6 + j * BH), hs, 1);
    g[j].K2 = hs; g[j].A_2nd = WS(w.d_recon + i * BH); g[j].lda_2nd = hs; g[j].ldb_2nd = hs;
    g[j].B_2nd = wt ? WS(w.rec_wT + (int64_t)i * hs * hs) : PP(p.rec_w + (int64_t)i * hs * hs);
    g[j].dsig = WS(w.x6 + j * BH); g[j].lddsig = hs;
  }
  sk_launch(*this, g, 6);
  for (int i = 0; i < 3; ++i) {
    g[i] = sk_dxw(wt, B, hs, hs, WS(w.d_x6 + i * BH), hs, WS(w.priv_wT + (int64_t)i * hs * hs), PP(p.priv_w + (int64_t)i * hs * hs),
                  WS(w.d_orig + i * BH), hs, 1);
    g[i].K2 = hs; g[i].A_2nd = WS(w.d_x6 + (3 + i) * BH); g[i].lda_2nd = hs; g[i].B_2nd = wt ? WS(w.sh_wT) : PP(p.sh_w); g[i].ldb_2nd = hs;
  }
  sk_launch(*this, g, 3);
  if (!rc) {
    mmda_ln_bwd_args l[3];
    for (int i = 0; i < 3; ++i) l[i] = proj_ln_bwd(i);
    rc = mmda_layernorm_bwd_multi(l, 3, s);
  }
  if (!P.enc_cut) skinny_proj_dx(wt);
}

void Pass::bwd_fusion_tiled() {
  rc = mmda_heads_bwd(WS(w.tcp), WS(w.scores), WS(w.d_tcp), WS(w.d_scores), B, c.ncls, WS(w.d_logits), p_cls, seed, SITE_CLS,
                        s);
  lin_dx(*this, fmode, B, NC, 6 * hs, WS(w.d_logits), PP(p.head_w), WS(w.d_hfused), 0);
  const mmda_ln_bwd_args l2 = norm2_bwd(), l1 = norm1_bwd();
  if (!rc) rc = mmda_layernorm_bwd(&l2, s);
  {
    mmda_gemm_args e = {};
    e.gate = WS(w.f1); e.ldgate = FFN; e.gate_scale = p_tf > 0.f ? 1.f / (1.f - p_tf) : 1.f;
    gemm(*this, fmode, 0, 0, 6 * B, FFN, hs, WS(w.d_f2), hs, PP(p.l2_w), FFN, WS(w.d_f1), FFN, nullptr, nullptr, 0, 0, 1, 0, 0, 0, 0, &e);
  }
  lin_dx(*this, fmode, 6 * B, FFN, hs, WS(w.d_f1), PP(p.l1_w), WS(w.d_x1), 1);
  if (!rc) rc = mmda_layernorm_bwd(&l1, s);
  lin_dx(*this, fmode, 6 * B, hs, hs, WS(w.d_attn_out), PP(p.out_w), WS(w.d_ctx), 0);
  if (!rc) rc = mmda_attn_bwd(WS(w.qkv), WS(w.probs), WS(w.d_ctx), S6, B, hs, NHEAD, WS(w.d_qkv), p_tf, seed, SITE_ATTN, s);
  lin_dx(*this, fmode, 6 * B, 3 * hs, hs, WS(w.d_qkv), PP(p.in_w), WS(w.d_x6), 1);
  if (!c.use_cmd_sim) {
    lin_dx(*this, fmode, 3 * B, 3, hs, WS(w.d_dom), PP(p.d2_w), WS(w.d_dom_h), 0);
    if (!rc) {
      const mmda_act_params ap = act_params(m, m->training, seed, SITE_RRELU_DISC, true);
      rc = mmda_act_dropout_bwd_p(WS(w.d_dom_h), WS(w.dom_z), WS(w.d_dom_z), 3 * BH, c.act, &ap, p_cls, seed, SITE_DISC, s);
    }
    mmda_gemm_args e = {};
    e.alpha = -c.reverse_grad_weight;
    gemm(*this, fmode, 0, 0, 3 * B, hs, hs, WS(w.d_dom_z), hs, PP(p.d1_w), hs, WS(w.d_x6 + 3 * BH), hs, nullptr, nullptr, 1, 0, 1, 0, 0, 0, 0, &e);
  }
  gemm(*this, fmode, 0, 0, B, hs, hs, WS(w.d_recon), hs, PP(p.rec_w), hs, WS(w.d_x6), hs, nullptr, nullptr, 1, 0, 3, BH, (int64_t)hs * hs, BH);
  gemm(*this, fmode, 0, 0, B, hs, hs, WS(w.d_recon), hs, PP(p.rec_w), hs, WS(w.d_x6 + 3 * BH), hs, nullptr, nullptr, 1, 0, 3, BH,
       (int64_t)hs * hs, BH);
  if (!rc) rc = mmda_sigmoid_bwd_inplace(WS(w.d_x6), WS(w.x6), 6 * BH, s);
  gemm(*this, fmode, 0, 0, B, hs, hs, WS(w.d_x6), hs, PP(p.priv_w), hs, WS(w.d_orig), hs, nullptr, nullptr, 1, 0, 3, BH, (int64_t)hs * hs, BH);
  lin_dx(*this, fmode, 3 * B, hs, hs, WS(w.d_x6 + 3 * BH), PP(p.sh_w), WS(w.d_orig), 1);
  for (int i = 0; i < 3 && !rc; ++i) {
    const ModP& md = p.mod[i]; const ModW& mw = w.mod[i];
    const mmda_ln_bwd_args l = proj_ln_bwd(i);
    rc = mmda_layernorm_bwd(&l, s);
    if (!P.enc_cut) lin_dx(*this, fmode, B, hs, 4 * md.H, WS(w.d_z + i * BH), PP(md.pw), WS(mw.d_utt), 0);
  }
}

void Pass::fusion_wgrads() {
  deferring = true;
  lin_dw(*this, fmode, B, NC, 6 * hs, WS(w.d_logits), WS(w.hfused), GG(p.head_w), GG(p.head_b));
  lin_dw(*this, fmode, 6 * B, hs, FFN, WS(w.d_f2), WS(w.f1), GG(p.l2_w), GG(p.l2_b));
  lin_dw(*this, fmode, 6 * B, FFN, hs, WS(w.d_f1), WS(w.x1), GG(p.l1_w), GG(p.l1_b));
  lin_dw(*this, fmode, 6 * B, hs, hs, WS(w.d_attn_out), WS(w.ctx), GG(p.out_w), GG(p.out_b));
  lin_dw(*this, fmode, 6 * B, 3 * hs, hs, WS(w.d_qkv), WS(w.x6), GG(p.in_w), GG(p.in_b));
  if (!c.use_cmd_sim) {
    lin_dw(*this, fmode, 3 * B, 3, hs, WS(w.d_dom), WS(w.dom_h), GG(p.d2_w), GG(p.d2_b));
    lin_dw(*this, fmode, 3 * B, hs, hs, WS(w.d_dom_z), WS(w.x6 + 3 * BH), GG(p.d1_w), GG(p.d1_b));
  }
  mmda_gemm_args e = {};
  e.bias_grad = GG(p.rec_b);
  gemm(*this, fmode, 1, 0, hs, hs, B, WS(w.d_recon), hs, WS(w.rsum), hs, GG(p.rec_w), hs, nullptr, nullptr, 1, 0, 3, BH, BH, (int64_t)hs * hs,
       hs, &e);
  e.bias_grad = GG(p.priv_b);
  gemm(*this, fmode, 1, 0, hs, hs, B, WS(w.d_x6), hs, WS(w.orig), hs, GG(p.priv_w), hs, nullptr, nullptr, 1, 0, 3, BH, BH, (int64_t)hs * hs,
       hs, &e);
  lin_dw(*this, fmode, 3 * B, hs, hs, WS(w.d_x6 + 3 * BH), WS(w.orig), GG(p.sh_w), GG(p.sh_b));
  for (int i = 0; i < 3; ++i)
    lin_dw(*this, fmode, B, hs, 4 * p.mod[i].H, WS(w.d_z + i * BH), WS(w.mod[i].utt), GG(p.mod[i].pw), GG(p.mod[i].pb));
  deferring = false;
}

void Pass::bwd_side_chain(bool pg_pending, const int64_t* t_ids, const int32_t* lengths) {
  void* ss = nullptr;
  rc = side_fork(m, s, &ss);
  if (!rc && m->misc_deferred) {
    rc = mmda_loss_misc_opts(WS(w.scores), WS(w.tcp), m->misc_deferred, B, c.ncls, nullptr, nullptr, c.ncls == 6, 0, c.conf_weight,
                             WS(w.recon), WS(w.orig), 3 * BH, c.recon_weight, nullptr, nullptr, WS(w.losses), c.diff_weight,
                             c.sim_weight, c.recon_weight, c.conf_weight, c.use_confidNet, m->cls(), ss);
    m->misc_deferred = nullptr;
  }
  if (!rc && P.skinny) rc = mmda_add(WS(w.x6), WS(w.x6 + 3 * BH), WS(w.rsum), 3 * BH, ss);
  m->esort_valid = 0;
  if (!rc && P.sort_early && !((P.embed_update == EU_SPARSE || P.embed_deferred) && !early)) {
    rc = mmda_embed_sort_ids(t_ids, B * w.T, lengths, B, c.vocab, reinterpret_cast<unsigned*>(WS(w.esort)), ss);
    if (!rc && ss != s) {
      hipLaunchKernelGGL(flag_set_kernel, dim3(1), dim3(1), 0, (hipStream_t)ss, m->jflags + 3, ++m->esort_val);
      if (hipGetLastError() != hipSuccess) rc = MMDA_ELAUNCH;
    }
    m->esort_valid = rc ? 0 : (ss != s ? 2 : 1);
  }
  if (!rc && pg_pending) {
    float* dg[FUSED_PG_SLOTS] = {GG(p.n2_w), GG(p.n1_w), GG(p.mod[0].plw), GG(p.mod[1].plw), GG(p.mod[2].plw)};
    float* db[FUSED_PG_SLOTS] = {GG(p.n2_b), GG(p.n1_b), GG(p.mod[0].plb), GG(p.mod[1].plb), GG(p.mod[2].plb)};
    rc = mmda_fused_pg_finish(WS(w.pg_parts), B, hs, dg, db, ss);
  }
  if (!rc && !deferred.empty()) rc = mmda_gemm_grouped(deferred.data(), (int)deferred.size(), ss);
  deferred.clear();
  if (!rc && P.bfg && w.T > 0 && !P.enc_cut) {
    mmda_convert_job cj[16];
    const int nj = backward_only_jobs(m, cj);
    rc = mmda_convert_bf16(cj, nj, ss);
  }
}

void Pass::bwd_encoder_layer(int l, const float* const* xin, const int64_t* t_ids, const int32_t* lengths) {
  mmda_lstm_desc desc[3];
  for (int i = 0; i < 3; ++i) desc[i] = lstm_desc(m, i, l, true, P.gm, P.want_c);
  if (P.kdg)
    for (int i = 0; i < 3; ++i) { desc[i].dg_bf16 = WS(w.mod[i].rnn[l].dgb); desc[i].dg_bf16_only = 1; }
  m->epoch += (unsigned)T + 2u;
  if (!P.want_b && !mmda_lstm_resident_applicable(mode, 3, desc, B, T, 1)) { rc = MMDA_EINVAL; return; }
  ev_rec(m, m->ev_bwd, l == 1 ? 2 : 3, 0, s);
  rc = mmda_lstm_bwd(mode, 3, desc, B, T, lengths, s);
  ev_rec(m, m->ev_bwd, l == 1 ? 2 : 3, 1, s);
  if (rc) return;
  const bool bfg = P.bfg, bf_hh = bfg && (B % 8) == 0;
  std::vector<mmda_gemm_bf16_args> bmain, bside;
  const bool frozen = P.embed_update == EU_FROZEN;
  mmda_convert_job dgj[3];
  for (int i = 0; i < 3; ++i) {
    const RnnP& r = p.mod[i].rnn[l]; const ModW& mw = w.mod[i]; const RnnW& rw = mw.rnn[l];
    const bool plain = (l == 1 || (i == 0 && !frozen)) && !P.kdg;
    dgj[i] = mmda_convert_job{WS(mw.gates[l]), 8 * r.H, R, 8 * r.H, nullptr, plain ? WS(rw.dgb) : nullptr, plain ? r.ldG : 0, WS(rw.dgbT),
                              w.ldR};
    if (P.kdg) { dgj[i].src = WS(rw.dgb); dgj[i].ld = r.ldG; dgj[i].src_bf16 = 1; }
  }
  const bool tn = P.tn_wgrad;
  const bool dg_on_side = P.kdg && l == 1 && m->use_side && !tn;
  if (bfg && !dg_on_side && !tn) {
    rc = mmda_convert_bf16(dgj, 3, s);
    if (rc) return;
  }
  deferring = (l == 1);
  group_begin(*this);
  for (int i = 0; i < 3; ++i) {
    const RnnP& r = p.mod[i].rnn[l]; const ModW& mw = w.mod[i]; const RnnW& rw = mw.rnn[l];
    const int H = r.H, G8 = 8 * H;
    const float* dG = WS(mw.gates[l]);
    const float* in = l == 0 ? xin[i] : WS(mw.normed);
    std::vector<mmda_gemm_bf16_args>& wq = (l == 1) ? bside : bmain;
    const unsigned short* dgT = reinterpret_cast<const unsigned short*>(WS(rw.dgbT));
    const unsigned short* hT = reinterpret_cast<const unsigned short*>(WS(rw.hbT));
    if (bfg) {
      mmda_gemm_bf16_args g = {};
      g.M = G8; g.N = r.D; g.K = R; g.A = dgT; g.lda = w.ldR; g.B = WS(rw.xbT); g.ldb = w.ldR; g.C = gW_ih(m, i, l); g.ldc = r.D;
      g.accumulate = 1; g.bias_grad = gB_ih(m, i, l); g.bias_grad2 = gB_hh(m, i, l); g.perm_m_H = P.gm ? H : 0;
      if (tn) { g.tn = 1; g.A = WS(rw.dgb); g.lda = r.ldG; g.B = WS(rw.xb); g.ldb = r.ldD; }
      wq.push_back(g);
    } else {
      mmda_gemm_args e = {};
      e.bias_grad = gB_ih(m, i, l); e.bias_grad2 = gB_hh(m, i, l);
      gemm(*this, mode, 1, 0, G8, r.D, R, dG, G8, in, r.D, gW_ih(m, i, l), r.D, nullptr, nullptr, 1, 0, 1, 0, 0, 0, 0, &e);
    }
    if (T > 1) {
      if (bf_hh) {
        mmda_gemm_bf16_args g = {};
        g.M = 4 * H; g.N = H; g.K = (T - 1) * B; g.lda = w.ldR; g.ldb = w.ldR; g.ldc = H; g.accumulate = 1;
        g.perm_m_H = P.gm ? H : 0;
        if (tn) {
          const unsigned short* dg = reinterpret_cast<const unsigned short*>(WS(rw.dgb));
          const unsigned short* h0 = reinterpret_cast<const unsigned short*>(WS(rw.hbp[0]));
          const unsigned short* h1 = reinterpret_cast<const unsigned short*>(WS(rw.hbp[1]));
          g.tn = 1; g.lda = r.ldG; g.ldb = r.ldH;
          g.A = dg + (int64_t)B * r.ldG; g.B = h0; g.C = gW_hh(m, i, l, 0);
          wq.push_back(g);
          g.A = dg + 4 * H; g.B = h1 + (int64_t)B * r.ldH; g.C = gW_hh(m, i, l, 1);
          wq.push_back(g);
        } else {
          g.A = dgT + B; g.B = hT; g.C = gW_hh(m, i, l, 0);
          wq.push_back(g);
          g.A = dgT + (int64_t)4 * H * w.ldR; g.B = hT + (int64_t)H * w.ldR + B; g.C = gW_hh(m, i, l, 1);
          wq.push_back(g);
        }
      } else {
        const float* hs_ = WS(mw.hseq[l]);
        gemm(*this, mode, 1, 0, 4 * H, H, (T - 1) * B, dG + (int64_t)B * G8, G8, hs_, 2 * H, gW_hh(m, i, l, 0), H, nullptr, nullptr, 1);
        gemm(*this, mode, 1, 0, 4 * H, H, (T - 1) * B, dG + 4 * H, G8, hs_ + (int64_t)B * 2 * H + H, 2 * H, gW_hh(m, i, l, 1), H, nullptr,
             nullptr, 1);
      }
    }
    if (l == 1 || i == 0) {
      float* dst = l == 1 ? WS(mw.d_normed) : WS(mw.d_x);
      const bool skip = l == 0 && frozen;
      if (bfg) {
        mmda_gemm_bf16_args g = {};
        g.M = R; g.N = r.D; g.K = G8; g.A = WS(rw.dgb); g.lda = r.ldG; g.B = WS(rw.wbT); g.ldb = r.ldG; g.C = dst; g.ldc = r.D;
        if (!skip) bmain.push_back(g);
      } else {
        absent_next = skip;
        gemm(*this, mode, 0, 0, R, r.D, G8, dG, G8, rW_ih(m, i, l), r.D, dst, r.D);
      }
    }
  }
  group_end(*this);
  deferring = false;
  if (!rc && !bmain.empty()) rc = mmda_gemm_bf16_grouped(bmain.data(), (int)bmain.size(), s);
  if (rc) return;
  if (l == 1) {
    mmda_ln_bwd_args lb[3];
    for (int i = 0; i < 3; ++i) {
      const ModP& md = p.mod[i]; const ModW& mw = w.mod[i];
      lb[i] = mmda_ln_bwd_args{};
      lb[i].rows = R; lb[i].n = 2 * md.H; lb[i].dy = WS(mw.d_normed); lb[i].x = WS(mw.hseq[0]); lb[i].gamma = PP(md.ln_w);
      lb[i].mean = WS(mw.ln_mean); lb[i].rstd = WS(mw.ln_rstd); lb[i].d_x = WS(mw.d_hseq1);
    }
    const bool ln_split = mmda_ln_bwd_parts_applies(lb, 3) &&
                          mmda_ln_parts_floats(lb, 3) <= (int64_t)512 * 2 * 2 * (p.mod[0].H + p.mod[1].H + p.mod[2].H);
    if (ln_split) {
      for (int i = 0; i < 3; ++i) { lb[i].dgamma = GG(p.mod[i].ln_w); lb[i].dbeta = GG(p.mod[i].ln_b); }
      rc = mmda_ln_bwd_parts(lb, 3, WS(w.ln_parts), s);
    } else {
      rc = mmda_layernorm_bwd_multi(lb, 3, s);
    }
    void* ss = nullptr;
    if (!rc) rc = side_fork(m, s, &ss);
    for (int i = 0; i < 3; ++i) { lb[i].dgamma = GG(p.mod[i].ln_w); lb[i].dbeta = GG(p.mod[i].ln_b); if (!ln_split) lb[i].d_x = nullptr; }
    if (!rc && dg_on_side) rc = mmda_convert_bf16(dgj, 3, ss);
    if (!rc) rc = ln_split ? mmda_ln_parts_finish(lb, 3, WS(w.ln_parts), ss) : mmda_layernorm_param_grads(lb, 3, ss);
    if (!rc && !deferred.empty()) rc = mmda_gemm_grouped(deferred.data(), (int)deferred.size(), ss);
    const bool l2_early = !bside.empty();
    if (!rc && l2_early) { rc = mmda_gemm_bf16_grouped(bside.data(), (int)bside.size(), ss); bside.clear(); }
    deferred.clear();
    if (rc) return;
    if (!m->ev_early && hipEventCreateWithFlags(&m->ev_early, hipEventDisableTiming) != hipSuccess) rc = MMDA_ELAUNCH;
    if (!rc && hipEventRecord(m->ev_early, (hipStream_t)ss) != hipSuccess) rc = MMDA_ELAUNCH;
    m->early_floats = (l2_early && !is_gru(m) && P.bfg) ? p.rnn1_begin : p.rnn2_begin;
    m->early_valid = 1;
    if (!rc && early && m->early_floats > 0 && m->M1 && m->V1) {
      rc = bucket_adam(m, 0, m->early_floats, nullptr, early->lr, early->clip, early->grad_scale, early->step, kNoWait, ss);
      if (!rc) m->adam_early_done = m->early_floats;
    }
  } else {
    bwd_text_rows(t_ids, lengths);
  }
}

const unsigned* Pass::take_sorted() {
  if (!m->esort_valid) return nullptr;
  if (m->esort_valid == 2) {
    hipLaunchKernelGGL(flag_wait_kernel, dim3(1), dim3(64), 0, (hipStream_t)s, m->jflags + 3, m->esort_val, m->jflags + 2);
    if (hipGetLastError() != hipSuccess) rc = MMDA_ELAUNCH;
  }
  m->esort_valid = 0;
  return reinterpret_cast<const unsigned*>(WS(w.esort));
}

void Pass::bwd_text_rows(const int64_t* t_ids, const int32_t* lengths) {
  const float* dx = WS(w.mod[0].d_x);
  if (P.embed_update == EU_SPARSE || P.embed_deferred) {
    m->eu.take();
    if (!early) { m->eu.set(t_ids, lengths); return; }
  }
  if (P.embed_update == EU_FROZEN) return;
  const EmbedList list{t_ids, take_sorted(), R, c.d_t, dx, lengths, B};
  if (rc) return;
  if (P.embed_update == EU_SPARSE) {
// ... 251 lines not shown
```

### mmda_amd/csrc/rowlocal.h

```cpp
#pragma once
#include "common.h"

namespace {

__device__ __forceinline__ int64_t perm_row(int row, int S, int Bp) {
  if (S <= 0) return row;
  int s = row / Bp, b = row % Bp;
  return (int64_t)b * S + s;
}

template <int NQ>
__device__ __forceinline__ void ln_bwd_row(const mmda_ln_bwd_args& a, int row, int lane, float (&dg)[NQ], float (&db)[NQ]) {
  const int n = a.n;
  const float mean = a.mean[row], rstd = a.rstd[row];
  const int64_t drow = perm_row(row, a.permute_S, a.permute_B);
  float xh[NQ], gdy[NQ];
  float s1 = 0.f, s2 = 0.f;
#pragma unroll
  for (int q = 0; q < NQ; ++q) {
    int i = lane + 64 * q;
    xh[q] = 0.f; gdy[q] = 0.f;
    if (i < n) {
      int64_t idx = (int64_t)row * n + i;
      float x = act_fwd_p(a.act, a.x[idx], a.actp, (uint64_t)idx);
      if (a.res) x += a.res[idx] * drop_mul(a.drop_p, a.drop_seed, a.drop_site, (uint64_t)idx);
      float dy = a.dy[drow * n + i];
      xh[q] = (x - mean) * rstd;
      gdy[q] = dy * a.gamma[i];
      dg[q] += dy * xh[q];
      db[q] += dy;
      s1 += gdy[q];
      s2 += gdy[q] * xh[q];
    }
  }
  s1 = wave_sum(s1) / n;
  s2 = wave_sum(s2) / n;
  float dslope = 0.f;
#pragma unroll
  for (int q = 0; q < NQ; ++q) {
    int i = lane + 64 * q;
    if (i < n) {
      int64_t idx = (int64_t)row * n + i;
      float dxp = rstd * (gdy[q] - s1 - xh[q] * s2);
      if (a.d_x) {
        const float z = a.x[idx];
        float d = dxp * act_bwd_p(a.act, z, a.actp, (uint64_t)idx);
        a.d_x[idx] = a.accumulate_dx ? a.d_x[idx] + d : d;
        if (a.act == MMDA_ACT_PRELU && z <= 0.f) dslope += dxp * z;
      }
      if (a.d_res) a.d_res[idx] = dxp * drop_mul(a.drop_p, a.drop_seed, a.drop_site, (uint64_t)idx);
    }
  }
  if (a.act == MMDA_ACT_PRELU && a.d_x && a.actp.dslope) {
    dslope = wave_sum(dslope);
    if (lane == 0) atomicAdd(a.actp.dslope, dslope);
  }
}

template <int NQ>
__device__ __forceinline__ void ln_fwd_row(const mmda_ln_args& a, int row, int lane) {
  const int n = a.n;
  float v[NQ];
  float s = 0.f;
#pragma unroll
  for (int q = 0; q < NQ; ++q) {
    int i = lane + 64 * q;
    float x = 0.f;
    if (i < n) {
      int64_t idx = (int64_t)row * n + i;
      x = act_fwd_p(a.act, a.x[idx], a.actp, (uint64_t)idx);
      if (a.res) x += a.res[idx] * drop_mul(a.drop_p, a.drop_seed, a.drop_site, (uint64_t)idx);
    }
    v[q] = x;
    s += x;
  }
  const float mean = wave_sum(s) / n;
  float ss = 0.f;
#pragma unroll
  for (int q = 0; q < NQ; ++q) {
    int i = lane + 64 * q;
    float d = (i < n) ? v[q] - mean : 0.f;
    ss += d * d;
  }
  const float var = wave_sum(ss) / n;
  const float rstd = 1.0f / sqrtf(var + a.eps);
  if (lane == 0) {
    if (a.mean) a.mean[row] = mean;
    if (a.rstd) a.rstd[row] = rstd;
  }
  const int64_t orow = perm_row(row, a.permute_S, a.permute_B);
#pragma unroll
  for (int q = 0; q < NQ; ++q) {
    int i = lane + 64 * q;
    float y = 0.f;
    if (i < n) { y = (v[q] - mean) * rstd * a.gamma[i] + a.beta[i]; if (a.y) a.y[orow * n + i] = y; }
    if (a.y_bf16 && i < a.ld_bf16) reinterpret_cast<unsigned short*>(a.y_bf16)[orow * a.ld_bf16 + i] = f2bf(y);
  }
}

constexpr int S6K = 6;

__device__ __forceinline__ void attn_fwd_hd64_one(const float* __restrict__ qkv, int B, float* ctx, float* probs, float p, uint64_t seed,
                                                  int site, int nhead, int bh, int d) {
  constexpr int S = S6K, hd = 64;
  const int E = hd * nhead;
  const int b = bh / nhead, h = bh % nhead;
  float q[S], k[S], v[S];
#pragma unroll
  for (int s = 0; s < S; ++s) {
    const float* row = qkv + ((int64_t)s * B + b) * 3 * E + h * hd + d;
    q[s] = row[0]; k[s] = row[E]; v[s] = row[2 * E];
  }
  const float scale = 1.0f / sqrtf((float)hd);
  float pr[S][S];
#pragma unroll
  for (int i = 0; i < S; ++i)
#pragma unroll
    for (int j = 0; j < S; ++j) pr[i][j] = wave_sum(q[i] * k[j]) * scale;
#pragma unroll
  for (int i = 0; i < S; ++i) {
    float m = -INFINITY;
#pragma unroll
    for (int j = 0; j < S; ++j) m = fmaxf(m, pr[i][j]);
    float sum = 0.f;
#pragma unroll
    for (int j = 0; j < S; ++j) { pr[i][j] = expf(pr[i][j] - m); sum += pr[i][j]; }
    const float inv = 1.0f / sum;
#pragma unroll
    for (int j = 0; j < S; ++j) {
      const float pv = pr[i][j] * inv;
      const int64_t pi = ((int64_t)bh * S + i) * S + j;
      if (d == 0) probs[pi] = pv;
      pr[i][j] = pv * drop_mul(p, seed, site, (uint64_t)pi);
    }
  }
#pragma unroll
  for (int s = 0; s < S; ++s) {
    float acc = 0.f;
#pragma unroll
    for (int j = 0; j < S; ++j) acc += pr[s][j] * v[j];
    ctx[((int64_t)s * B + b) * E + h * hd + d] = acc;
  }
}


__device__ __forceinline__ void attn_bwd_hd64_one(const float* __restrict__ qkv, const float* __restrict__ probs, const float* __restrict__ dctx,
                                                  int B, float* dqkv, float p, uint64_t seed, int site, int nhead, int bh, int d) {
  constexpr int S = S6K, hd = 64;
  const int E = hd * nhead;
  const int b = bh / nhead, h = bh % nhead;
  float q[S], k[S], v[S], dc[S];
#pragma unroll
  for (int s = 0; s < S; ++s) {
    const float* row = qkv + ((int64_t)s * B + b) * 3 * E + h * hd + d;
    q[s] = row[0]; k[s] = row[E]; v[s] = row[2 * E];
    dc[s] = dctx[((int64_t)s * B + b) * E + h * hd + d];
  }
  float P[S][S], Pd[S][S], dS[S][S];
#pragma unroll
  for (int i = 0; i < S; ++i)
#pragma unroll
    for (int j = 0; j < S; ++j) {
      const int64_t pi = (int64_t)bh * S * S + i * S + j;
      const float mul = drop_mul(p, seed, site, (uint64_t)pi);
      P[i][j] = probs[pi];
      Pd[i][j] = P[i][j] * mul;
      dS[i][j] = wave_sum(dc[i] * v[j]) * mul;
    }
#pragma unroll
  for (int i = 0; i < S; ++i) {
    float dot = 0.f;
#pragma unroll
    for (int j = 0; j < S; ++j) dot += dS[i][j] * P[i][j];
#pragma unroll
    for (int j = 0; j < S; ++j) dS[i][j] = P[i][j] * (dS[i][j] - dot);
  }
  const float scale = 1.0f / sqrtf((float)hd);
#pragma unroll
  for (int s = 0; s < S; ++s) {
    float dq = 0.f, dk = 0.f, dv = 0.f;
#pragma unroll
    for (int j = 0; j < S; ++j) {
      dq += dS[s][j] * k[j];
      dk += dS[j][s] * q[j];
      dv += Pd[j][s] * dc[j];
    }
    float* row = dqkv + ((int64_t)s * B + b) * 3 * E + h * hd + d;
    row[0] = dq * scale; row[E] = dk * scale; row[2 * E] = dv;
  }
}

}
```

Baseline: 55170 samples/s.

## Split fused attention forward across heads and defer backward flag wait

Adds a fused forward kernel that launches one workgroup per (batch, head) plus a set of reconstruction workgroups. This replaces per-batch-row blocks and spreads the QKV projection, attention and output projection over more CUs. Per-head output-projection partials are combined by the last-arriving block through an atomic ticket before the LN1 forward. The backward kernel also gains a late-wait variant: the ln1 dx goes to a separate buffer so the flag wait can happen after the weight MACs, overlapping them with the side-stream join. The cost is extra partial-buffer traffic, atomics, and more synchronization complexity.

```diff
diff --git a/mmda_amd/csrc/fused_heads.hip b/mmda_amd/csrc/fused_heads.hip
--- /dev/null
+++ b/mmda_amd/csrc/fused_heads.hip
@@ -0,0 +1,179 @@
+#include "common.h"
+#include "internal.h"
+#include "rowlocal.h"
+#include "fused_rows.h"
+#include "fused_rows_dev.h"
+
+namespace {
+
+__device__ __forceinline__ void fwd_a_recon_rows(const FusedFwdA& P, int b0, int nb, float* lds_a, float* lds_w) {
+  const int B = P.B, hs = P.hs;
+  const int lane = threadIdx.x & 63, wave = threadIdx.x >> 6;
+  const int r16 = lane & 15, g = lane >> 4;
+  const int nmod = 3 * nb;
+  const bool mok = r16 < nmod;
+  const int mi = mok ? r16 / nb : 0;
+  const int col = wave * 16 + r16;
+  for (int e = threadIdx.x; e < nmod * (hs / 4); e += FR_THREADS) {
+    const int r = e / (hs / 4), c = e % (hs / 4);
+    const f4 a = *reinterpret_cast<const f4*>(lds_a + r * (hs + 4) + 4 * c), b2 = *reinterpret_cast<const f4*>(lds_a + (nmod + r) * (hs + 4) + 4 * c);
+    *reinterpret_cast<f4*>(lds_a + (12 + r) * (hs + 4) + 4 * c) = a + b2;
+  }
+  __syncthreads();
+  {
+    f32x4 acc = {0.f, 0.f, 0.f, 0.f};
+    const float* srow = mok ? lds_a + (12 + r16) * (hs + 4) : nullptr;
+    const float* const ar[3] = {(mok && mi == 0) ? srow : nullptr, (mok && mi == 1) ? srow : nullptr, (mok && mi == 2) ? srow : nullptr};
+    const float* rw = P.rec_w + (int64_t)wave * 16 * hs;
+    const float* const bb[3] = {rw, rw + (int64_t)hs * hs, rw + (int64_t)2 * hs * hs};
+    const int ld[3] = {hs, hs, hs};
+    tile_mac_chain<3>(acc, ar, bb, ld, lane, lds_w + wave * 16 * WL_LD);
+#pragma unroll
+    for (int i = 0; i < 4; ++i) {
+      const int r = 4 * g + i;
+      if (r < nmod) {
+        const int64_t o = ((int64_t)(r / nb) * B + b0 + (r % nb)) * hs + col;
+        const float rv = acc[i] + P.rec_b[(r / nb) * hs + col];
+        P.recon[o] = rv;
+        if (P.d_recon) {
+          const float gr = recon_seed(rv - P.orig[o], P.recon_inv_n, P.recon_scale);
+          P.d_recon[o] = gr;
+          P.d_orig[o] = 0.f - gr;
+        }
+      }
+    }
+  }
+}
+
+template <int NC>
+__device__ __forceinline__ void mac_lds(f32x4& acc, const float* arow , const float* wl, int lane) {
+  const int r16 = lane & 15, g = lane >> 4;
+  const f4 z = {0.f, 0.f, 0.f, 0.f};
+  f4 a[NC], b[NC];
+#pragma unroll
+  for (int c = 0; c < NC; ++c) {
+    a[c] = arow ? *reinterpret_cast<const f4*>(arow + 16 * c + 4 * g) : z;
+    b[c] = *reinterpret_cast<const f4*>(wl + r16 * WL_LD + 16 * c + 4 * g);
+  }
+#pragma unroll
+  for (int c = 0; c < NC; ++c)
+#pragma unroll
+    for (int s = 0; s < 4; ++s) acc = __builtin_amdgcn_mfma_f32_16x16x4f32(a[c][s], b[c][s], acc, 0, 0, 0);
+}
+struct WHalf { f4 g[4]; };
+__device__ __forceinline__ void whalf_load(WHalf& W, const float* __restrict__ bblk, int ldb, int lane) {
+#pragma unroll
+  for (int j = 0; j < 4; ++j) W.g[j] = *reinterpret_cast<const f4*>(bblk + (int64_t)(4 * j + (lane >> 4)) * ldb + 4 * (lane & 15));
+}
+__device__ __forceinline__ void whalf_to_lds(const WHalf& W, float* wl, int lane) {
+#pragma unroll
+  for (int j = 0; j < 4; ++j) *reinterpret_cast<f4*>(wl + (4 * j + (lane >> 4)) * WL_LD + 4 * (lane & 15)) = W.g[j];
+}
+
+__device__ __forceinline__ void part_store(float* p, float v) {
+  __hip_atomic_store(reinterpret_cast<unsigned*>(p), __float_as_uint(v), __ATOMIC_RELAXED, __HIP_MEMORY_SCOPE_AGENT);
+}
+__device__ __forceinline__ float part_load(const float* p) {
+  return __uint_as_float(__hip_atomic_load(reinterpret_cast<const unsigned*>(p), __ATOMIC_RELAXED, __HIP_MEMORY_SCOPE_AGENT));
+}
+__device__ __forceinline__ bool ticket_last(unsigned* ticket, unsigned n, unsigned* word) {
+  asm volatile("s_waitcnt vmcnt(0)" ::: "memory");
+  __syncthreads();
+  if (threadIdx.x == 0) {
+    const unsigned t = __hip_atomic_fetch_add(ticket, 1u, __ATOMIC_RELAXED, __HIP_MEMORY_SCOPE_AGENT);
+    const bool last = t == n - 1u;
+    if (last) __hip_atomic_store(ticket, 0u, __ATOMIC_RELAXED, __HIP_MEMORY_SCOPE_AGENT);
+    *word = last ? 1u : 0u;
+  }
+  __syncthreads();
+  return __builtin_amdgcn_readfirstlane((int)*word) != 0;
+}
+
+__global__ __launch_bounds__(FR_THREADS) void fused_fwd_a_heads_kernel(FusedFwdA P) {
+  __shared__ __attribute__((aligned(16))) float lds_a[LDS_A_FLOATS];
+  __shared__ __attribute__((aligned(16))) float lds_w[8 * 16 * WL_LD];
+  const int B = P.B, hs = P.hs;
+  const int lane = threadIdx.x & 63, wave = threadIdx.x >> 6;
+  const int r16 = lane & 15, g = lane >> 4;
+  constexpr int NH = 2, HD = 64;
+  if ((int)blockIdx.x >= NH * B) {
+    const int rb = (int)blockIdx.x - NH * B;
+    stage_rows(lds_a, S6K, hs, [&](int r) { return P.x6 + ((int64_t)r * B + rb) * hs; });
+    fwd_a_recon_rows(P, rb, 1, lds_a, lds_w);
+    return;
+  }
+  const int b = (int)blockIdx.x / NH, h = (int)blockIdx.x % NH;
+  float* wl = lds_w + wave * 16 * WL_LD;
+  float* lds_q = lds_a + 8 * (hs + 4);
+  float* lds_c = lds_q + S6K * 3 * HD;
+  auto tile_n0 = [&](int t) { return (t >> 2) * hs + h * HD + (t & 3) * 16; };
+  const bool two = wave < 4;
+  WRows W0, W1;
+  WHalf Wo;
+  wrows_load(W0, P.in_w + (int64_t)tile_n0(wave) * hs, hs, lane);
+  if (two) wrows_load(W1, P.in_w + (int64_t)tile_n0(8 + wave) * hs, hs, lane);
+  whalf_load(Wo, P.out_w + (int64_t)wave * 16 * hs + h * HD, hs, lane);
+  stage_rows(lds_a, S6K, hs, [&](int r) { return P.x6 + ((int64_t)r * B + b) * hs; });
+  const float* xrow = r16 < S6K ? lds_a + r16 * (hs + 4) : nullptr;
+  auto qkv_tile = [&](int t) {
+    f32x4 acc = {0.f, 0.f, 0.f, 0.f};
+    mac_lds<8>(acc, xrow, wl, lane);
+    const int n = tile_n0(t) + r16;
+    const float bias = P.in_b[n];
+#pragma unroll
+    for (int i = 0; i < 4; ++i) {
+      const int r = 4 * g + i;
+      if (r < S6K) {
+        const float v = acc[i] + bias;
+        lds_q[r * 3 * HD + (t >> 2) * HD + (t & 3) * 16 + r16] = v;
+        P.qkv[((int64_t)r * B + b) * 3 * hs + n] = v;
+      }
+    }
+  };
+  wrows_to_lds(W0, wl, lane);
+  qkv_tile(wave);
+  if (two) {
+    wrows_to_lds(W1, wl, lane);
+    qkv_tile(8 + wave);
+  }
+  whalf_to_lds(Wo, wl, lane);
+  __syncthreads();
+  if (wave < S6K) {
+    float k[S6K], v[S6K];
+#pragma unroll
+    for (int s = 0; s < S6K; ++s) { k[s] = lds_q[s * 3 * HD + HD + lane]; v[s] = lds_q[s * 3 * HD + 2 * HD + lane]; }
+    const float c = attn_fwd_hd64_row(lds_q[wave * 3 * HD + lane], k, v, P.probs, P.p_tf, P.seed, P.site_attn, b * NH + h, wave, lane);
+    lds_c[wave * (HD + 4) + lane] = c;
+    P.ctx[((int64_t)wave * B + b) * hs + h * HD + lane] = c;
+  }
+  __syncthreads();
+  {
+    f32x4 acc = {0.f, 0.f, 0.f, 0.f};
+    mac_lds<4>(acc, r16 < S6K ? lds_c + r16 * (HD + 4) : nullptr, wl, lane);
+    float* part = P.head_parts + ((int64_t)h * B + b) * S6K * hs;
+#pragma unroll
+    for (int i = 0; i < 4; ++i) {
+      const int r = 4 * g + i;
+      if (r < S6K) part_store(part + r * hs + wave * 16 + r16, acc[i]);
+    }
+  }
+  if (!ticket_last(P.head_tickets + b, NH, reinterpret_cast<unsigned*>(lds_a))) return;
+  for (int e = threadIdx.x; e < S6K * hs; e += FR_THREADS) {
+    const int r = e / hs, c = e % hs;
+    const float p0 = part_load(P.head_parts + ((int64_t)b * S6K + r) * hs + c);
+    const float p1 = part_load(P.head_parts + (((int64_t)B + b) * S6K + r) * hs + c);
+    P.attn_out[((int64_t)r * B + b) * hs + c] = (p0 + p1) + P.out_b[c];
+  }
+  stage_sync();
+  for (int i = wave; i < S6K; i += FR_THREADS / 64) ln_fwd_row<2>(P.ln1, i * B + b, lane);
+}
+
+}
+
+int mmda_fused_fwd_a_heads(const FusedFwdA* a, void* stream) {
+  if (!a || a->B <= 0 || a->B > FUSED_HEADS_MAX_B || a->nb != 1 || a->hs != 128 || a->nhead != 2 || a->ln1.n != 128) return MMDA_EINVAL;
+  if (!a->head_parts || !a->head_tickets || (a->d_recon && (!a->orig || !a->d_orig))) return MMDA_EINVAL;
+  hipLaunchKernelGGL(fused_fwd_a_heads_kernel, dim3(3 * a->B), dim3(FR_THREADS), 0, (hipStream_t)stream, *a);
+  MMDA_CHECK_LAUNCH("mmda_fused_fwd_a_heads");
+  return MMDA_OK;
+}
diff --git a/mmda_amd/csrc/fused_rows.h b/mmda_amd/csrc/fused_rows.h
--- a/mmda_amd/csrc/fused_rows.h
+++ b/mmda_amd/csrc/fused_rows.h
@@ -33,6 +33,7 @@
   float* pg_parts;
   unsigned long long* dbg;
   const unsigned* wait_flag; unsigned wait_value; unsigned* wait_err;
+  float* ln1_dx;
 };
 
 struct FusedFwdA {
@@ -45,7 +46,9 @@
   mmda_ln_args ln1;
   const float* orig; float* d_recon; float* d_orig; float recon_inv_n, recon_scale;
   int split_recon;
+  float* head_parts; unsigned* head_tickets;
 };
+constexpr int FUSED_HEADS_MAX_B = 64;
 struct FusedFwdC {
   int B, hs, ncls, nb;
   mmda_ln_args ln2;
@@ -73,6 +76,7 @@
 int mmda_fused_ffn_fwd(const FusedFfnFwd* a, void* stream);
 int mmda_fused_ffn_bwd(const FusedFfnBwd* a, void* stream);
 int mmda_fused_fwd_a(const FusedFwdA* a, void* stream);
+int mmda_fused_fwd_a_heads(const FusedFwdA* a, void* stream);
 int mmda_fused_fwd_c(const FusedFwdC* a, void* stream);
 int mmda_fused_bwd_c(const FusedBwdC* a, void* stream);
 int mmda_fused_bwd_a(const FusedBwdA* a, void* stream);
diff --git a/mmda_amd/csrc/fused_rows.hip b/mmda_amd/csrc/fused_rows.hip
--- a/mmda_amd/csrc/fused_rows.hip
+++ b/mmda_amd/csrc/fused_rows.hip
@@ -2,109 +2,9 @@
 #include "internal.h"
 #include "rowlocal.h"
 #include "fused_rows.h"
+#include "fused_rows_dev.h"
 
 namespace {
-
-typedef __attribute__((ext_vector_type(4))) float f4;
-constexpr int FR_THREADS = 512;
-
-struct MacRound { f4 a[8], b[8]; };
-constexpr int WL_LD = 128 + 4;
-struct WRows { f4 g[8]; };
-__device__ __forceinline__ void wrows_load(WRows& W, const float* __restrict__ bblk, int ldb, int lane) {
-#pragma unroll
-  for (int j = 0; j < 8; ++j) W.g[j] = *reinterpret_cast<const f4*>(bblk + (int64_t)(2 * j + (lane >> 5)) * ldb + 4 * (lane & 31));
-}
-__device__ __forceinline__ void wrows_to_lds(const WRows& W, float* wl, int lane) {
-#pragma unroll
-  for (int j = 0; j < 8; ++j) *reinterpret_cast<f4*>(wl + (2 * j + (lane >> 5)) * WL_LD + 4 * (lane & 31)) = W.g[j];
-}
-__device__ __forceinline__ void mac_frags(MacRound& R, const float* arow , const float* wl, int lane) {
-  const int r16 = lane & 15, g = lane >> 4;
-  const f4 z = {0.f, 0.f, 0.f, 0.f};
-#pragma unroll
-  for (int c = 0; c < 8; ++c) {
-    R.a[c] = arow ? *reinterpret_cast<const f4*>(arow + 16 * c + 4 * g) : z;
-    R.b[c] = *reinterpret_cast<const f4*>(wl + r16 * WL_LD + 16 * c + 4 * g);
-  }
-}
-__device__ __forceinline__ void mac_run(f32x4& acc, const MacRound& R) {
-#pragma unroll
-  for (int c = 0; c < 8; ++c)
-#pragma unroll
-    for (int s = 0; s < 4; ++s) acc = __builtin_amdgcn_mfma_f32_16x16x4f32(R.a[c][s], R.b[c][s], acc, 0, 0, 0);
-}
-template <int NR>
-__device__ __forceinline__ void tile_mac_chain(f32x4& acc, const float* const (&ar)[NR], const float* const (&bblk)[NR], const int (&ldb)[NR],
-                                               int lane, float* wl ) {
-  WRows W;
-  MacRound R;
-  wrows_load(W, bblk[0], ldb[0], lane);
-#pragma unroll
-  for (int r = 0; r < NR; ++r) {
-    wrows_to_lds(W, wl, lane);
-    if (r + 1 < NR) wrows_load(W, bblk[r + 1], ldb[r + 1], lane);
-    mac_frags(R, ar[r], wl, lane);
-    mac_run(acc, R);
-  }
-}
-
-__device__ __forceinline__ float sum_parts(const float* __restrict__ p, int n, int64_t stride) {
-  float acc = 0.f;
-  int q = 0;
-  for (; q + 16 <= n; q += 16) {
-    float v[16];
-#pragma unroll
-    for (int u = 0; u < 16; ++u) v[u] = p[(q + u) * stride];
-#pragma unroll
-    for (int u = 0; u < 16; ++u) acc += v[u];
-  }
-  for (; q < n; ++q) acc += p[q * stride];
-  return acc;
-}
-
-template <typename RowOff, typename Finish>
-__device__ __forceinline__ void sum_parts_rows(const float* __restrict__ parts, int n, int64_t stride, int groups, RowOff row_off, f4* lds,
-                                               Finish finish) {
-  const int n0 = (n + 1) >> 1;
-  for (int it = threadIdx.x; it < 2 * groups; it += FR_THREADS) {
-    const int gi = it % groups, half = it / groups;
-    const float* p = parts + row_off(gi) + (int64_t)(half ? n0 : 0) * stride;
-    const int cnt = half ? n - n0 : n0;
-    f4 acc = {0.f, 0.f, 0.f, 0.f};
-    int q = 0;
-    for (; q + 16 <= cnt; q += 16) {
-      f4 v[16];
-#pragma unroll
-      for (int u = 0; u < 16; ++u) v[u] = *reinterpret_cast<const f4*>(p + (q + u) * stride);
-#pragma unroll
-      for (int u = 0; u < 16; ++u) acc += v[u];
-    }
-    for (; q < cnt; ++q) acc += *reinterpret_cast<const f4*>(p + q * stride);
-    lds[half * groups + gi] = acc;
-  }
-  __syncthreads();
-  for (int gi = threadIdx.x; gi < groups; gi += FR_THREADS) finish(gi, lds[gi] + lds[groups + gi]);
-  __syncthreads();
-}
-
-__device__ __forceinline__ void stage_sync() {
-  __threadfence_block();
-  __syncthreads();
-}
-
-constexpr int LDS_A_FLOATS = 12 * (384 + 4) + 18 * (128 + 4);
-template <typename SrcOf>
-__device__ __forceinline__ void stage_rows(float* lds, int nrows, int K, SrcOf src_of) {
-  const int per_row = K >> 2;
-  for (int e = threadIdx.x; e < nrows * per_row; e += FR_THREADS) {
-    const int r = e / per_row, c = e % per_row;
-    const float* src = src_of(r);
-    const f4 z = {0.f, 0.f, 0.f, 0.f};
-    *reinterpret_cast<f4*>(lds + r * (K + 4) + 4 * c) = src ? *reinterpret_cast<const f4*>(src + 4 * c) : z;
-  }
-  __syncthreads();
-}
 
 template <typename RowOf>
 __device__ __forceinline__ void ln_bwd_rows(const mmda_ln_bwd_args& a, int nrows, RowOf row_of, float* red ,
@@ -184,6 +84,7 @@
   pg_zero_rest(P.pg_parts, b0, nb, 0);
 }
 
+template <bool LATE_WAIT>
 __global__ __launch_bounds__(FR_THREADS) void fused_bwd_a_kernel(FusedBwdA P) {
   __shared__ float red[2 * 8 * 128];
   __shared__ __attribute__((aligned(16))) float lds_a[LDS_A_FLOATS];
@@ -197,7 +98,7 @@
   int stamp_i = 0;
   auto stamp = [&]() { if (P.dbg && blockIdx.x == 0 && threadIdx.x == 0) P.dbg[stamp_i] = __builtin_readcyclecounter(); ++stamp_i; };
   stamp();
-  flag_wait(P.wait_flag, P.wait_value, P.wait_err);
+  if constexpr (!LATE_WAIT) flag_wait(P.wait_flag, P.wait_value, P.wait_err);
   if (P.ffn_parts) {
     const int64_t MH = (int64_t)S6K * B * hs;
     auto off = [&](int gi) { const int i = gi / (hs / 4); return ((int64_t)(i / nb) * B + b0 + (i % nb)) * hs + 4 * (gi % (hs / 4)); };
@@ -255,6 +156,7 @@
       const int ld[6] = {3 * hs, 3 * hs, 3 * hs, hs, hs, hs};
       tile_mac_chain<6>(acc, ar, bb, ld, lane, lds_w + wave * 16 * WL_LD);
     }
+    if constexpr (LATE_WAIT) flag_wait(P.wait_flag, P.wait_value, P.wait_err);
 #pragma unroll
     for (int i = 0; i < 4; ++i) {
       const int r = 4 * g + i;
@@ -263,7 +165,8 @@
         const float s = P.x6[o];
         float t = acc[i];
         if (P.rec_part) t += P.rec_part[((int64_t)((r / nb) % 3) * B + b0 + (r % nb)) * hs + col];
-        P.d_x6[o] = (P.d_x6[o] + t) * (s * (1.f - s));
+        if constexpr (LATE_WAIT) P.d_x6[o] = ((P.d_x6[o] + P.ln1_dx[o]) + t) * (s * (1.f - s));
+        else P.d_x6[o] = (P.d_x6[o] + t) * (s * (1.f - s));
       }
     }
   }
@@ -578,6 +481,7 @@
 int mmda_fused_fwd_a(const FusedFwdA* a, void* stream) {
   if (!a || a->B <= 0 || a->nb <= 0 || a->nb > 2 || a->hs != 128 || a->nhead != 2 || a->ln1.n != 128) return MMDA_EINVAL;
   if (a->d_recon && (!a->orig || !a->d_orig)) return MMDA_EINVAL;
+  if (a->head_parts || a->head_tickets) return mmda_fused_fwd_a_heads(a, stream);
   static const int split_on = mmda_env_int("MMDA_FUSED_SPLIT", 1);
   FusedFwdA f = *a;
   const int nblk = ceil_div(a->B, a->nb);
@@ -652,9 +556,10 @@
 int mmda_fused_bwd_a(const FusedBwdA* a, void* stream) {
   if (!a || a->B <= 0 || a->nb <= 0 || a->nb > 2 || a->hs != 128 || a->nhead != 2) return MMDA_EINVAL;
   if ((a->ln1.dgamma || a->ln1.dbeta || a->lnp[0].dgamma || a->lnp[0].dbeta) && !a->pg_parts) return MMDA_EINVAL;
+  if (a->ln1_dx && (a->ln1.d_x != a->ln1_dx || a->ln1.accumulate_dx)) return MMDA_EINVAL;
   FusedBwdA P = *a;
   P.dbg = g_fr_dbg;
-  hipLaunchKernelGGL(fused_bwd_a_kernel, dim3(ceil_div(a->B, a->nb)), dim3(FR_THREADS), 0, (hipStream_t)stream, P);
+  hipLaunchKernelGGL(a->ln1_dx ? fused_bwd_a_kernel<true> : fused_bwd_a_kernel<false>, dim3(ceil_div(a->B, a->nb)), dim3(FR_THREADS), 0, (hipStream_t)stream, P);
   MMDA_CHECK_LAUNCH("mmda_fused_bwd_a");
   return MMDA_OK;
 }
diff --git a/mmda_amd/csrc/fused_rows_dev.h b/mmda_amd/csrc/fused_rows_dev.h
--- /dev/null
+++ b/mmda_amd/csrc/fused_rows_dev.h
@@ -0,0 +1,107 @@
+#pragma once
+#include "common.h"
+
+namespace {
+
+typedef __attribute__((ext_vector_type(4))) float f4;
+constexpr int FR_THREADS = 512;
+
+struct MacRound { f4 a[8], b[8]; };
+constexpr int WL_LD = 128 + 4;
+struct WRows { f4 g[8]; };
+__device__ __forceinline__ void wrows_load(WRows& W, const float* __restrict__ bblk, int ldb, int lane) {
+#pragma unroll
+  for (int j = 0; j < 8; ++j) W.g[j] = *reinterpret_cast<const f4*>(bblk + (int64_t)(2 * j + (lane >> 5)) * ldb + 4 * (lane & 31));
+}
+__device__ __forceinline__ void wrows_to_lds(const WRows& W, float* wl, int lane) {
+#pragma unroll
+  for (int j = 0; j < 8; ++j) *reinterpret_cast<f4*>(wl + (2 * j + (lane >> 5)) * WL_LD + 4 * (lane & 31)) = W.g[j];
+}
+__device__ __forceinline__ void mac_frags(MacRound& R, const float* arow , const float* wl, int lane) {
+  const int r16 = lane & 15, g = lane >> 4;
+  const f4 z = {0.f, 0.f, 0.f, 0.f};
+#pragma unroll
+  for (int c = 0; c < 8; ++c) {
+    R.a[c] = arow ? *reinterpret_cast<const f4*>(arow + 16 * c + 4 * g) : z;
+    R.b[c] = *reinterpret_cast<const f4*>(wl + r16 * WL_LD + 16 * c + 4 * g);
+  }
+}
+__device__ __forceinline__ void mac_run(f32x4& acc, const MacRound& R) {
+#pragma unroll
+  for (int c = 0; c < 8; ++c)
+#pragma unroll
+    for (int s = 0; s < 4; ++s) acc = __builtin_amdgcn_mfma_f32_16x16x4f32(R.a[c][s], R.b[c][s], acc, 0, 0, 0);
+}
+template <int NR>
+__device__ __forceinline__ void tile_mac_chain(f32x4& acc, const float* const (&ar)[NR], const float* const (&bblk)[NR], const int (&ldb)[NR],
+                                               int lane, float* wl ) {
+  WRows W;
+  MacRound R;
+  wrows_load(W, bblk[0], ldb[0], lane);
+#pragma unroll
+  for (int r = 0; r < NR; ++r) {
+    wrows_to_lds(W, wl, lane);
+    if (r + 1 < NR) wrows_load(W, bblk[r + 1], ldb[r + 1], lane);
+    mac_frags(R, ar[r], wl, lane);
+    mac_run(acc, R);
+  }
+}
+
+__device__ __forceinline__ float sum_parts(const float* __restrict__ p, int n, int64_t stride) {
+  float acc = 0.f;
+  int q = 0;
+  for (; q + 16 <= n; q += 16) {
+    float v[16];
+#pragma unroll
+    for (int u = 0; u < 16; ++u) v[u] = p[(q + u) * stride];
+#pragma unroll
+    for (int u = 0; u < 16; ++u) acc += v[u];
+  }
+  for (; q < n; ++q) acc += p[q * stride];
+  return acc;
+}
+
+template <typename RowOff, typename Finish>
+__device__ __forceinline__ void sum_parts_rows(const float* __restrict__ parts, int n, int64_t stride, int groups, RowOff row_off, f4* lds,
+                                               Finish finish) {
+  const int n0 = (n + 1) >> 1;
+  for (int it = threadIdx.x; it < 2 * groups; it += FR_THREADS) {
+    const int gi = it % groups, half = it / groups;
+    const float* p = parts + row_off(gi) + (int64_t)(half ? n0 : 0) * stride;
+    const int cnt = half ? n - n0 : n0;
+    f4 acc = {0.f, 0.f, 0.f, 0.f};
+    int q = 0;
+    for (; q + 16 <= cnt; q += 16) {
+      f4 v[16];
+#pragma unroll
+      for (int u = 0; u < 16; ++u) v[u] = *reinterpret_cast<const f4*>(p + (q + u) * stride);
+#pragma unroll
+      for (int u = 0; u < 16; ++u) acc += v[u];
+    }
+    for (; q < cnt; ++q) acc += *reinterpret_cast<const f4*>(p + q * stride);
+    lds[half * groups + gi] = acc;
+  }
+  __syncthreads();
+  for (int gi = threadIdx.x; gi < groups; gi += FR_THREADS) finish(gi, lds[gi] + lds[groups + gi]);
+  __syncthreads();
+}
+
+__device__ __forceinline__ void stage_sync() {
+  __threadfence_block();
+  __syncthreads();
+}
+
+constexpr int LDS_A_FLOATS = 12 * (384 + 4) + 18 * (128 + 4);
+template <typename SrcOf>
+__device__ __forceinline__ void stage_rows(float* lds, int nrows, int K, SrcOf src_of) {
+  const int per_row = K >> 2;
+  for (int e = threadIdx.x; e < nrows * per_row; e += FR_THREADS) {
+    const int r = e / per_row, c = e % per_row;
+    const float* src = src_of(r);
+    const f4 z = {0.f, 0.f, 0.f, 0.f};
+    *reinterpret_cast<f4*>(lds + r * (K + 4) + 4 * c) = src ? *reinterpret_cast<const f4*>(src + 4 * c) : z;
+  }
+  __syncthreads();
+}
+
+}
diff --git a/mmda_amd/csrc/misa.hip b/mmda_amd/csrc/misa.hip
--- a/mmda_amd/csrc/misa.hip
+++ b/mmda_amd/csrc/misa.hip
@@ -85,6 +85,8 @@
   bool fj_on = false, fj_fwd = false, fj_device = false;
   bool zg_here = false;
   bool rec_hoisted = false;
+  bool head_slices = false;
+  bool late_join = false;
   bool sort_early = false;
   int embed_update = 0;
   bool embed_deferred = false;
@@ -311,7 +313,8 @@
     TENSOR("d_dom", d_dom), TENSOR("pub_begin", pub_begin), TENSOR("pub_end", pub_end), TENSOR("zero_begin", zero_begin),
     TENSOR("zero_end", zero_end), TENSOR("hseq1_t", mod[0].hseq[0]), TENSOR("hseq1_v", mod[1].hseq[0]), TENSOR("hseq1_a", mod[2].hseq[0]),
     TENSOR("d_x_t", mod[0].d_x),
-    TENSOR("xchg_t", mod[0].xchg), TENSOR("xchg_v", mod[1].xchg), TENSOR("xchg_a", mod[2].xchg)};
+    TENSOR("xchg_t", mod[0].xchg), TENSOR("xchg_v", mod[1].xchg), TENSOR("xchg_a", mod[2].xchg),
+    TENSOR("attn_out", attn_out)};
 #undef TENSOR
 
 }
@@ -353,6 +356,7 @@
   int bg_on = -1, bg_wgs = 0;
   const OptStep* bg_step = nullptr;
   int bg_pending = 0, bg_active = 0;
+  float* head_buf = nullptr;
   unsigned* jflags = nullptr;
   mmda_run* runs_dev = nullptr; int runs_dev_cap = 0; int runs_dirty = 1;
   std::vector<hipEvent_t> ev;
@@ -708,6 +712,9 @@
   return MMDA_OK;
 }
 
+constexpr size_t kHeadTicketBytes = 256;
+constexpr int kHeadSlicesMaxB = 64;
+static_assert(kHeadSlicesMaxB <= FUSED_HEADS_MAX_B, "the handle's partials are sized by FUSED_HEADS_MAX_B");
 constexpr int FJ_DEVICE_MAX_B = 64;
 constexpr int kEmbedBgDefault = 1, kEmbedBgWorkgroups = 32, kEmbedBgLds = 1024, kEmbedBgMaxB = 32;
 
@@ -720,6 +727,7 @@
   static const int flag_join_on = mmda_env_int("MMDA_FLAG_JOIN", 1);
   static const int zg_side = mmda_env_int("MMDA_ZERO_GRAD_SIDE", -1);
   static const int fsplit = mmda_env_int("MMDA_FUSED_SPLIT", 1);
+  static const int fheads = mmda_env_int("MMDA_FUSED_HEADS", 1);
   static const int sort_early = mmda_env_int("MMDA_SORT_EARLY", 1);
   static const int bg_on = mmda_env_int("MMDA_EMBED_BG", kEmbedBgDefault);
   static const int bg_wgs = mmda_env_int("MMDA_EMBED_BG_WGS", 0);
@@ -758,6 +766,8 @@
   P.fj_device = P.fj_fwd && B <= FJ_DEVICE_MAX_B;
   P.zg_here = zg_side >= 0 ? zg_side != 0 : P.fj_device;
   P.rec_hoisted = fsplit && m->lay.rec_part >= 0 && B <= 64;
+  P.head_slices = P.row_fuse && fsplit && fheads && B <= kHeadSlicesMaxB;
+  P.late_join = P.head_slices && P.fj_device;
   P.embed_update = m->embed_update;
   P.embed_deferred = m->embed_update == EU_DENSE && m->df_row_step != nullptr;
   P.sort_early = sort_early && T > 0 && m->lay.esort >= 0 && mmda_embed_scatter_sorts(T * B) && P.embed_update != EU_FROZEN && !P.enc_cut;
@@ -796,6 +806,7 @@
   if (m->row_stamp) (void)hipFree(m->row_stamp);
   if (m->side) (void)hipStreamDestroy(m->side);
   if (m->jflags) (void)hipFree(m->jflags);
+  if (m->head_buf) (void)hipFree(m->head_buf);
   if (m->runs_dev) (void)hipFree(m->runs_dev);
   for (hipEvent_t e : m->ev) (void)hipEventDestroy(e);
   delete m;
@@ -1340,7 +1351,16 @@
         f.orig = WS(w.orig); f.d_recon = WS(w.d_recon); f.d_orig = WS(w.d_orig);
         f.recon_inv_n = 1.0f / (float)(3 * BH); f.recon_scale = c.recon_weight;
       }
-      rc = mmda_fused_fwd_a(&f, s);
+      if (P.head_slices) {
+        constexpr size_t kBytes = kHeadTicketBytes + (size_t)(NHEAD + 1) * FUSED_HEADS_MAX_B * S6 * 128 * sizeof(float);
+        if (!m->head_buf) {
+          if (hipMalloc(reinterpret_cast<void**>(&m->head_buf), kBytes) != hipSuccess) { m->head_buf = nullptr; rc = MMDA_ELAUNCH; }
+          else if (hipMemsetAsync(m->head_buf, 0, kBytes, (hipStream_t)s) != hipSuccess) { (void)hipFree(m->head_buf); m->head_buf = nullptr; rc = MMDA_ELAUNCH; }
+        }
+        f.head_tickets = reinterpret_cast<unsigned*>(m->head_buf);
+        f.head_parts = m->head_buf + kHeadTicketBytes / sizeof(float);
+      }
+      if (!rc) rc = mmda_fused_fwd_a(&f, s);
     }
   } else {
     int n = 0;
@@ -1622,6 +1642,10 @@
   f.pg_parts = WS(w.pg_parts);
   if (m->fj1) {
     if (P.fj_device) { f.wait_flag = m->jflags; f.wait_value = m->jval[0]; f.wait_err = m->jflags + 2; }
+    if (P.late_join && m->head_buf) {
+      f.ln1_dx = m->head_buf + kHeadTicketBytes / sizeof(float) + (size_t)NHEAD * FUSED_HEADS_MAX_B * S6 * 128;
+      f.ln1.d_x = f.ln1_dx; f.ln1.accumulate_dx = 0;
+    }
     else rc = flag_join_fallback(m, s);
     m->fj1 = 0;
   }
diff --git a/mmda_amd/csrc/rowlocal.h b/mmda_amd/csrc/rowlocal.h
--- a/mmda_amd/csrc/rowlocal.h
+++ b/mmda_amd/csrc/rowlocal.h
@@ -144,6 +144,34 @@
 }
 
 
+__device__ __forceinline__ float attn_fwd_hd64_row(float qi, const float (&k)[6], const float (&v)[6], float* probs, float p, uint64_t seed,
+                                                   int site, int bh, int i, int d) {
+  constexpr int S = 6, hd = 64;
+  const float scale = 1.0f / sqrtf((float)hd);
+  float pr[S];
+#pragma unroll
+  for (int j = 0; j < S; ++j) pr[j] = wave_sum(qi * k[j]) * scale;
+  float m = -INFINITY;
+#pragma unroll
+  for (int j = 0; j < S; ++j) m = fmaxf(m, pr[j]);
+  float sum = 0.f;
+#pragma unroll
+  for (int j = 0; j < S; ++j) { pr[j] = expf(pr[j] - m); sum += pr[j]; }
+  const float inv = 1.0f / sum;
+#pragma unroll
+  for (int j = 0; j < S; ++j) {
+    const float pv = pr[j] * inv;
+    const int64_t pi = ((int64_t)bh * S + i) * S + j;
+    if (d == 0) probs[pi] = pv;
+    pr[j] = pv * drop_mul(p, seed, site, (uint64_t)pi);
+  }
+  float acc = 0.f;
+#pragma unroll
+  for (int j = 0; j < S; ++j) acc += pr[j] * v[j];
+  return acc;
+}
+
+
 __device__ __forceinline__ void attn_bwd_hd64_one(const float* __restrict__ qkv, const float* __restrict__ probs, const float* __restrict__ dctx,
                                                   int B, float* dqkv, float p, uint64_t seed, int site, int nhead, int bh, int d) {
   constexpr int S = S6K, hd = 64;
```

Measured after the change: 55690 samples/s, median of 6. About the same (+0.9%).
